# skylinemusiccds/Llama.github.io

Hardware: AMD Instinct MI355X
Metric: GBM train rows/sec (100 trees, depth 6) on HIGGS-11M at 1/2/4/8 MI355X (higher is better)
Workload: dtype fp32; 1 GPU; global_batch=11000000, parallelism=dp1 (row-sharded, hist all-reduce), rows=11000000, rows_per_rank=11000000, features=28, comm_bytes_per_tree=0

## Files before the change

llama_github_io_amd/csrc/tree_kernels.hip:

```cpp
#include <hip/hip_runtime.h>
#include <stdint.h>
#include <stdlib.h>
#include <string.h>

#include "abi.h"

#define NBIN 256
#define AMAX_SHARDS 64
#define NA_BIN 255
#define FTILE 32
#define BLK 1024
#define NW (BLK / 64)
#define TILE 2048
#define LEAFQ_STRIPES 16
#define LPR 8
#define RPI (BLK / LPR)

struct Node {
  int start, len, build, parent, sib ,
      dir , pad1, pad2;
};

#define NBW 32
#define GROUP_CAT 2
struct Dec {
  int feat;
  int bin;
  int na_left;
  int is_cat;
  unsigned bits[NBW];
  double gain;
  double wl, wr;
  float predl, predr;
};

#define TP_MAXL_DEV 64

struct Cand {
  double expl;
  double gain;
  double wl, wr;
  float predl, predr;
  int bin, na_left, valid, is_cat;
  unsigned bits[NBW];
};

struct SplitParams {
  double min_w;
  double min_split_improvement;
  double lambda, alpha, gamma;
  int mode;
  int random_split;
  unsigned long long seed;
  int hist_type;
  int fcut;
  const float* vrange;
  const double* hprev;
  const Dec* pdec;
  const Node* rnodes;
  const int* fgroup;
  const float* edges_all;
  int range_on, pad_r;
  const int* gcat;
  const double* rootw;
};

enum { HT_QUANTILES = 0, HT_UNIFORM = 1, HT_RANDOM = 2, HT_ROBUST = 3, HT_ROUND_ROBIN = 4 };

__device__ __forceinline__ unsigned long long splitmix64(unsigned long long x) {
  x += 0x9E3779B97F4A7C15ull;
  x = (x ^ (x >> 30)) * 0xBF58476D1CE4E5B9ull;
  x = (x ^ (x >> 27)) * 0x94D049BB133111EBull;
  return x ^ (x >> 31);
}

__device__ __forceinline__ bool dec_go_left(const Dec* d, int b) {
  if (b == NA_BIN) return d->na_left != 0;
  if (d->is_cat) return (d->bits[b >> 5] >> (b & 31)) & 1u;
  return b < d->bin;
}

__device__ __forceinline__ int group_level(unsigned word, unsigned pack) {
  if ((word & 0xFFu) == NA_BIN) return -1;
#pragma unroll
  for (int k = 0; k < 4; ++k) {
    const unsigned ek = (pack >> (8 * k)) & 0xFFu, b = (word >> (8 * k)) & 0xFFu;
    if (ek != 0u && b != ek) return 254 * k + (int)b;
  }
  return -1;
}

template <bool GRP = true>
__device__ __forceinline__ bool dec_go_left_key(const Dec* d, unsigned v) {
  if (GRP && d->is_cat == GROUP_CAT) {
    const int l = group_level(v, (unsigned)d->bin);
    return l < 0 ? d->na_left != 0 : ((d->bits[l >> 5] >> (l & 31)) & 1u) != 0u;
  }
  return dec_go_left(d, (int)v);
}

__device__ __forceinline__ int find_node(const int* __restrict__ tp, int n, int t) {
  int lo = 0, hi = n - 1;
  while (lo < hi) {
    int mid = (lo + hi + 1) >> 1;
    if (tp[mid] <= t) lo = mid; else hi = mid - 1;
  }
  return lo;
}

__device__ __forceinline__ double wave_sum_d(double v) {
  for (int o = 32; o > 0; o >>= 1) v += __shfl_xor(v, o, 64);
  return v;
}
__device__ __forceinline__ int wave_sum_i(int v) {
  for (int o = 32; o > 0; o >>= 1) v += __shfl_xor(v, o, 64);
  return v;
}

__device__ void block_sum4(double v[4], double* scratch ) {
  const int lane = threadIdx.x & 63, wid = threadIdx.x >> 6, nw = blockDim.x >> 6;
  for (int k = 0; k < 4; ++k) v[k] = wave_sum_d(v[k]);
  __syncthreads();
  if (lane == 0) for (int k = 0; k < 4; ++k) scratch[k * 16 + wid] = v[k];
  __syncthreads();
  if (threadIdx.x == 0) {
    for (int k = 0; k < 4; ++k) { double s = 0; for (int w = 0; w < nw; ++w) s += scratch[k * 16 + w]; v[k] = s; }
  }
  __syncthreads();
}

#define HPLANE (NBIN * FTILE + 16)
#define HIST_LDS_BYTES (2 * HPLANE * 8 + FTILE * 4)
#define WQCAP 192
#define HIST_LDS_TAIL (64 * 8 + (BLK / 64) * WQCAP * 4)
__device__ __forceinline__ int fslot(int fl) { return (fl & 16) | ((fl + ((fl >> 4) << 1)) & 15); }

__device__ __forceinline__ void lds_zero64(long long* h, int n) {
  for (int i = threadIdx.x; i < n; i += blockDim.x) h[i] = 0ll;
}

__device__ __forceinline__ long long q64(float v, float scale) {
  return (long long)(v * scale);
}

#define PACK_SHIFT 48
#define PACK_MAX 63488
__device__ __forceinline__ long long qpack(float w, float b, float scale_p, float sw, float shf) {
  if (shf < 40.f) return ((long long)__float2uint_rn(w * sw) << 32) + (long long)__float2int_rn(b * scale_p);
  return ((long long)__float2int_rz(w) << PACK_SHIFT) + (long long)__float2int_rz(b * scale_p);
}
__device__ __forceinline__ void unpack(long long v, long long& cnt, long long& val, int shift = PACK_SHIFT) {
  cnt = (long long)(((unsigned long long)v + (1ull << (shift - 1))) >> shift);
  val = (long long)((unsigned long long)v - ((unsigned long long)cnt << shift));
}

template <typename P>
__device__ __forceinline__ void put_partial(P* q, double d, bool acc) {
  *q = acc ? (P)((double)*q + d) : (P)d;
}
__device__ void flush_partial(const long long* h, const float* nayy, double node_wyy, int ftile, int F,
                              double* __restrict__ part, const double* __restrict__ qs, bool packed, bool acc,
                              bool f32, const int* srep, const int* snb, const int* sfine) {
  const int f0 = ftile * FTILE;
  const int nf = min(FTILE, F - f0);
  const double inv_a = qs[2], inv_b = qs[3], inv_p = qs[5];
  if (packed) {
    const int pshift = (int)qs[12];
    const double inv_w = qs[11];
    const int dbin = (int)blockDim.x / nf, drem = (int)blockDim.x - dbin * nf;
    int bin = (int)threadIdx.x / nf, fl = (int)threadIdx.x - bin * nf;
    for (int i = threadIdx.x; i < nf * NBIN; i += blockDim.x, bin += dbin, fl += drem) {
      if (fl >= nf) { fl -= nf; ++bin; }
      const int reps = srep[fl], nb = snb[fl];
      long long q = 0;
      if (sfine[fl]) {
        const int m = fl & ~3, k = fl & 3;
#pragma unroll
        for (int l = 0; l < 4; ++l) {
          const int bb = l <= k ? bin : bin - 1;
          if (bb >= 0) q += h[bb * FTILE + fslot(m + l)];
        }
      } else if (reps == 1) {
        q = h[bin * FTILE + fslot(fl)];
      } else if (bin < nb) {
        for (int c = 0; c < reps; ++c) q += h[(bin + c * nb) * FTILE + fslot(fl)];
      }
      long long c, v;
      unpack(q, c, v, pshift);
      const double dc = (double)c * inv_w, dv = (double)v * inv_p;
      const size_t e2 = (size_t)bin * 2 * F + 2 * (f0 + fl);
      if (f32) {
        float2* p2 = (float2*)((float*)part + e2);
        float2 o = make_float2((float)dc, (float)dv);
        if (acc) { const float2 a = *p2; o = make_float2((float)((double)a.x + dc), (float)((double)a.y + dv)); }
        *p2 = o;
      } else {
        double2* p2 = (double2*)(part + e2);
        double2 o = make_double2(dc, dv);
        if (acc) { const double2 a = *p2; o.x += a.x; o.y += a.y; }
        *p2 = o;
      }
    }
  } else {
  const int row2 = 2 * nf, dbin = (int)blockDim.x / row2, drem = (int)blockDim.x - dbin * row2;
  int bin = (int)threadIdx.x / row2, rem = (int)threadIdx.x - bin * row2;
  for (int i = threadIdx.x; i < nf * 2 * NBIN; i += blockDim.x, bin += dbin, rem += drem) {
    if (rem >= row2) { rem -= row2; ++bin; }
    const int fl = rem >> 1, r = rem & 1;
    const int reps = srep[fl], nb = snb[fl];
    long long q = 0;
    if (sfine[fl]) {
      const int m = fl & ~3, k = fl & 3;
      const int pl = r * HPLANE;
#pragma unroll
      for (int l = 0; l < 4; ++l) {
        const int bb = l <= k ? bin : bin - 1;
        if (bb >= 0) q += h[pl + bb * FTILE + fslot(m + l)];
      }
    } else if (reps == 1 || bin < nb) {
      for (int c = 0; c < reps; ++c) q += h[r * HPLANE + (bin + c * nb) * FTILE + fslot(fl)];
    }
    const double d = (double)q * (r ? inv_b : inv_a);
    const size_t e2 = (size_t)bin * 2 * F + 2 * (f0 + fl) + r;
    if (f32) put_partial((float*)part + e2, d, acc);
    else put_partial(part + e2, d, acc);
  }
  }
  for (int i = threadIdx.x; i < nf; i += blockDim.x) {
    const size_t e2 = (size_t)F * 2 * NBIN + f0 + i;
    if (f32) put_partial((float*)part + e2, (double)nayy[i], acc);
    else put_partial(part + e2, (double)nayy[i], acc);
  }
  if (threadIdx.x == 0 && ftile == 0) {
    const size_t e2 = (size_t)F * 2 * NBIN + F;
    if (f32) put_partial((float*)part + e2, node_wyy, acc);
    else put_partial(part + e2, node_wyy, acc);
  }
}

__device__ __forceinline__ float row_yy(float a, float b) {
  return a > 0.f ? b * b * __builtin_amdgcn_rcpf(a) : 0.f;
}

__device__ __forceinline__ size_t bin_off(long long row, int f, int stride, long long N, int planar) {
  return planar ? ((size_t)(f >> 5) * (size_t)N + (size_t)row) * 32 + (f & 31) : (size_t)row * stride + f;
}

struct RowFilter {
  const Dec* pd;
  const uint8_t* fptr;
  int fstride;
  int feat;
  int jw;
  int dir;
  int bin, na_left, is_cat;
  bool count;
  __device__ __forceinline__ bool left(unsigned v) const {
    if (is_cat == GROUP_CAT) {
      const int l = group_level(v, (unsigned)bin);
      return l < 0 ? na_left != 0 : ((pd->bits[l >> 5] >> (l & 31)) & 1u) != 0u;
    }
    const int b = (int)v;
    if (b == NA_BIN) return na_left != 0;
    if (is_cat) return (pd->bits[b >> 5] >> (b & 31)) & 1u;
    return b < bin;
  }
};


__device__ __forceinline__ void wave_sync_lds() {
  __builtin_amdgcn_fence(__ATOMIC_RELEASE, "wavefront");
  __builtin_amdgcn_wave_barrier();
  __builtin_amdgcn_fence(__ATOMIC_ACQUIRE, "wavefront");
}

#define FNP (TILE / BLK)
#define WROWS (TILE / NW)
__device__ __forceinline__ void filt_load(const RowFilter& flt, int r0, int r1, unsigned (&byt)[FNP]) {
  const int lane = threadIdx.x & 63, wv = threadIdx.x >> 6;
  if (flt.is_cat == GROUP_CAT) {
#pragma unroll
    for (int p = 0; p < FNP; ++p) {
      const int row = min(r0 + wv * WROWS + p * 64 + lane, r1 - 1);
      byt[p] = *reinterpret_cast<const unsigned*>(flt.fptr + (size_t)row * (size_t)flt.fstride);
    }
    return;
  }
#pragma unroll
  for (int p = 0; p < FNP; ++p) {
    const int row = min(r0 + wv * WROWS + p * 64 + lane, r1 - 1);
    byt[p] = flt.fptr[(size_t)row * (size_t)flt.fstride];
  }
}

__device__ __forceinline__ int filt_append(const RowFilter& flt, int r0, int r1, int* wq, int qn, int& lcnt,
                                           const unsigned (&byt)[FNP]) {
  const int lane = threadIdx.x & 63, wv = threadIdx.x >> 6;
  const unsigned long long below = (1ull << lane) - 1ull;
#pragma unroll
  for (int p = 0; p < FNP; ++p) {
    const int row = r0 + wv * WROWS + p * 64 + lane;
    bool sl = false;
    if (row < r1) {
      const bool gl = flt.left(byt[p]);
      if (flt.count) lcnt += gl ? 1 : 0;
      sl = (gl ? 0 : 1) == flt.dir;
    }
    const unsigned long long m = __ballot(sl);
    if (sl) wq[qn + __popcll(m & below)] = row;
    qn += __popcll(m);
  }
  return qn;
}

#ifndef H2O_UNR
#define H2O_UNR 8
#endif

struct HistSrc {
  const unsigned* bins32;
  const float* aw;
  const float* ay;
  __amdgpu_buffer_rsrc_t rb, ra, rw;
  int lgw;
};

__device__ __forceinline__ HistSrc make_src(const unsigned* bins32, const float* aw, const float* ay, long long N, int W,
                                            int lgw) {
  return HistSrc{bins32, aw, ay,
                 __builtin_amdgcn_make_buffer_rsrc((void*)bins32, 0, (int)(unsigned)((unsigned long long)N * W * 4),
                                                   0x00020000),
                 __builtin_amdgcn_make_buffer_rsrc((void*)ay, 0, (int)(unsigned)(N * 4), 0x00020000),
                 __builtin_amdgcn_make_buffer_rsrc((void*)(aw ? aw : ay), 0, (int)(unsigned)(N * 4), 0x00020000),
                 lgw};
}

template <bool FILT, bool PACKED, bool UNIT, bool NONA, bool BUF, bool FINE, int GR = RPI, int UNR = H2O_UNR>
__device__ __forceinline__ void hist_rows(long long* h, float* nayy, const HistSrc& src, int W, int wabs,
                                          int F, bool lead, int r0, int r1, int g, int j, float& wyy, float sa,
                                          float sb, float sp, const int* lst, const int* srep, const int* snb,
                                          const int* sfine) {
  const int rot = g & 1;
  unsigned offb[4], sh[4];
  unsigned vmask = 0u;
#pragma unroll
  for (int k = 0; k < 4; ++k) {
    const int kk = (k + rot) & 3;
    const int fl = j * 4 + kk;
    const int c = (g >> 1) & (srep[fl] - 1);
    offb[k] = (unsigned)fslot(fl) * 8u + ((unsigned)(c * snb[fl]) << 8);
    sh[k] = 8u * kk;
    if (wabs < W && wabs * 4 + kk < F) vmask |= 0xFFu << (8 * kk);
  }
  const bool live = vmask != 0u;
  const bool fine = FINE && live && sfine[j * 4] != 0;
  unsigned fsl[4];
#pragma unroll
  for (int l = 0; l < 4; ++l) fsl[l] = (unsigned)fslot(j * 4 + l) * 8u;
  const int wc = min(wabs, W - 1);
  const bool weighted = !UNIT && src.aw != nullptr;
  char* Hb = (char*)h;
  static_assert(FTILE * 8 == 256, "bin row of the LDS histogram is 256 bytes");
  auto ent = [&](unsigned w, int k) -> unsigned long long* {
    return (unsigned long long*)(Hb + ((__builtin_amdgcn_ubfe(w, sh[k], 8) << 8) + offb[k]));
  };
  for (int base = r0; base < r1; base += GR * UNR) {
    unsigned wd[UNR];
    float2 ab[UNR];
    const bool whole = base + GR * UNR <= r1;
    if (BUF && !FILT && whole) {
      const unsigned row0 = (unsigned)(base + g);
      const unsigned vb = (row0 << src.lgw) + (unsigned)wc * 4u, va = row0 * 4u;
#pragma unroll
      for (int u = 0; u < UNR; ++u) {
        wd[u] = __builtin_amdgcn_raw_buffer_load_b32(src.rb, vb, (unsigned)(u * GR) << src.lgw, 0);
        const float y = __uint_as_float(__builtin_amdgcn_raw_buffer_load_b32(src.ra, va, u * GR * 4, 0));
        const float w = weighted ? __uint_as_float(__builtin_amdgcn_raw_buffer_load_b32(src.rw, va, u * GR * 4, 0))
                                 : 1.f;
        ab[u] = make_float2(w, y);
      }
    } else {
#pragma unroll
      for (int u = 0; u < UNR; ++u) {
        const int idx = whole ? base + g + u * GR : min(base + g + u * GR, r1 - 1);
        const int row = FILT ? lst[idx] : idx;
        if (BUF) {
          const unsigned ro = (unsigned)row;
          wd[u] = __builtin_amdgcn_raw_buffer_load_b32(src.rb, (ro << src.lgw) + (unsigned)wc * 4u, 0, 0);
          const float y = __uint_as_float(__builtin_amdgcn_raw_buffer_load_b32(src.ra, ro * 4u, 0, 0));
          const float w = weighted ? __uint_as_float(__builtin_amdgcn_raw_buffer_load_b32(src.rw, ro * 4u, 0, 0)) : 1.f;
          ab[u] = make_float2(w, y);
        } else {
          ab[u] = make_float2(weighted ? src.aw[row] : 1.f, src.ay[row]);
          wd[u] = src.bins32[(size_t)row * W + wc];
        }
      }
    }
    auto row = [&](int u) {
      if (lead) wyy += UNIT ? ab[u].y * ab[u].y : row_yy(ab[u].x, ab[u].y);
      const long long qa = UNIT ? (1ll << PACK_SHIFT) + (long long)(int)(ab[u].y * sp)
                                : PACKED ? qpack(ab[u].x, ab[u].y, sp, sa, sb) : q64(ab[u].x, sa);
      const long long qb = PACKED ? 0ll : q64(ab[u].y, sb);
      const unsigned w = wd[u];
      if (FINE && fine) {
        const unsigned t = __builtin_amdgcn_sad_u8(w, 0u, 0u);
        const unsigned l = t & 3u;
        const unsigned so = (l & 2u) ? ((l & 1u) ? fsl[3] : fsl[2]) : ((l & 1u) ? fsl[1] : fsl[0]);
        unsigned long long* p = (unsigned long long*)(Hb + (((t >> 2) << 8) + so));
        atomicAdd(p, (unsigned long long)qa);
        if (!PACKED) atomicAdd(p + HPLANE, (unsigned long long)qb);
      } else if (live) {
#pragma unroll
        for (int k = 0; k < 4; ++k) {
          unsigned long long* p = ent(w, k);
          atomicAdd(p, (unsigned long long)qa);
          if (!PACKED) atomicAdd(p + HPLANE, (unsigned long long)qb);
        }
      }
      if (!NONA) {
        const unsigned x = ~w | ~vmask;
        if (((x - 0x01010101u) & ~x & 0x80808080u) != 0u) {
          const float yy = UNIT ? ab[u].y * ab[u].y : row_yy(ab[u].x, ab[u].y);
#pragma unroll
          for (int k = 0; k < 4; ++k)
            if (((vmask >> sh[k]) & 1u) && __builtin_amdgcn_ubfe(w, sh[k], 8) == NA_BIN)
              atomicAdd(nayy + j * 4 + (sh[k] >> 3), yy);
        }
      }
    };
    if (whole) {
#pragma unroll
      for (int u = 0; u < UNR; ++u) row(u);
    } else {
#pragma unroll
      for (int u = 0; u < UNR; ++u)
        if (base + g + u * GR < r1) row(u);
    }
  }
}

template <bool PACKED, bool UNIT, bool NONA, bool BUF, bool FINE>
__device__ __forceinline__ void hist_span(long long* h, float* nayy, const HistSrc& src, int W, int wabs, int F,
                                          bool lead, int r0, int r1, int g, int j, float& wyy, float sa, float sb,
                                          float sp, const int* srep, const int* snb, const int* sfine,
                                          bool no_atoms = false) {
  constexpr int GR = RPI, UNR = H2O_UNR;
  const int rot = g & 1;
  unsigned offb[4], sh[4];
  unsigned vmask = 0u;
#pragma unroll
  for (int k = 0; k < 4; ++k) {
    const int kk = (k + rot) & 3;
    const int fl = j * 4 + kk;
    const int c = (g >> 1) & (srep[fl] - 1);
    offb[k] = (unsigned)fslot(fl) * 8u + ((unsigned)(c * snb[fl]) << 8);
    sh[k] = 8u * kk;
    if (wabs < W && wabs * 4 + kk < F) vmask |= 0xFFu << (8 * kk);
  }
  const bool live = vmask != 0u && !no_atoms;
  const bool fine = FINE && live && sfine[j * 4] != 0;
  unsigned fsl[4];
#pragma unroll
  for (int l = 0; l < 4; ++l) fsl[l] = (unsigned)fslot(j * 4 + l) * 8u;
  const int wc = min(wabs, W - 1);
  const bool weighted = !UNIT && src.aw != nullptr;
  char* Hb = (char*)h;
  auto load = [&](int base, unsigned (&wd)[UNR], float2 (&ab)[UNR]) {
    if (BUF && base + GR * UNR <= r1) {
      const unsigned row0 = (unsigned)(base + g);
      const unsigned vb = (row0 << src.lgw) + (unsigned)wc * 4u, va = row0 * 4u;
#pragma unroll
      for (int u = 0; u < UNR; ++u) {
        wd[u] = __builtin_amdgcn_raw_buffer_load_b32(src.rb, vb, (unsigned)(u * GR) << src.lgw, 0);
        const float y = __uint_as_float(__builtin_amdgcn_raw_buffer_load_b32(src.ra, va, u * GR * 4, 0));
        const float w = weighted ? __uint_as_float(__builtin_amdgcn_raw_buffer_load_b32(src.rw, va, u * GR * 4, 0))
                                 : 1.f;
        ab[u] = make_float2(w, y);
      }
    } else {
#pragma unroll
      for (int u = 0; u < UNR; ++u) {
        const int row = min(base + g + u * GR, r1 - 1);
        if (BUF) {
          const unsigned ro = (unsigned)row;
          wd[u] = __builtin_amdgcn_raw_buffer_load_b32(src.rb, (ro << src.lgw) + (unsigned)wc * 4u, 0, 0);
          const float y = __uint_as_float(__builtin_amdgcn_raw_buffer_load_b32(src.ra, ro * 4u, 0, 0));
          const float w = weighted ? __uint_as_float(__builtin_amdgcn_raw_buffer_load_b32(src.rw, ro * 4u, 0, 0)) : 1.f;
          ab[u] = make_float2(w, y);
        } else {
          ab[u] = make_float2(weighted ? src.aw[row] : 1.f, src.ay[row]);
          wd[u] = src.bins32[(size_t)row * W + wc];
        }
      }
    }
  };
  unsigned wdn[UNR];
  float2 abn[UNR];
  if (r0 < r1) load(r0, wdn, abn);
  for (int base = r0; base < r1; base += GR * UNR) {
    unsigned wd[UNR];
    float2 ab[UNR];
#pragma unroll
    for (int u = 0; u < UNR; ++u) { wd[u] = wdn[u]; ab[u] = abn[u]; }
    if (base + GR * UNR < r1) load(base + GR * UNR, wdn, abn);
    auto atoms = [&](int u) {
      const long long qa = UNIT ? (1ll << PACK_SHIFT) + (long long)(int)(ab[u].y * sp)
                                : PACKED ? qpack(ab[u].x, ab[u].y, sp, sa, sb) : q64(ab[u].x, sa);
      const long long qb = PACKED ? 0ll : q64(ab[u].y, sb);
      const unsigned w = wd[u];
      if (FINE && fine) {
        const unsigned t = __builtin_amdgcn_sad_u8(w, 0u, 0u);
        const unsigned l = t & 3u;
        const unsigned so = (l & 2u) ? ((l & 1u) ? fsl[3] : fsl[2]) : ((l & 1u) ? fsl[1] : fsl[0]);
        unsigned long long* p = (unsigned long long*)(Hb + (((t >> 2) << 8) + so));
        atomicAdd(p, (unsigned long long)qa);
        if (!PACKED) atomicAdd(p + HPLANE, (unsigned long long)qb);
      } else {
#pragma unroll
        for (int k = 0; k < 4; ++k) {
          unsigned long long* p = (unsigned long long*)(Hb + ((__builtin_amdgcn_ubfe(w, sh[k], 8) << 8) + offb[k]));
          atomicAdd(p, (unsigned long long)qa);
          if (!PACKED) atomicAdd(p + HPLANE, (unsigned long long)qb);
        }
      }
    };
    auto row = [&](int u) {
      if (lead) wyy += UNIT ? ab[u].y * ab[u].y : row_yy(ab[u].x, ab[u].y);
      if (FINE && live) atoms(u);
      if (!NONA) {
        const unsigned w = wd[u];
        const unsigned x = ~w | ~vmask;
        if (((x - 0x01010101u) & ~x & 0x80808080u) != 0u) {
          const float yy = UNIT ? ab[u].y * ab[u].y : row_yy(ab[u].x, ab[u].y);
#pragma unroll
          for (int k = 0; k < 4; ++k)
            if (((vmask >> sh[k]) & 1u) && __builtin_amdgcn_ubfe(w, sh[k], 8) == NA_BIN)
              atomicAdd(nayy + j * 4 + (sh[k] >> 3), yy);
        }
      }
    };
    if (base + GR * UNR <= r1) {
#pragma unroll
      for (int u = 0; u < UNR; ++u) row(u);
      if (!FINE && live) {
#pragma unroll
        for (int u = 0; u < UNR; ++u) atoms(u);
      }
    } else {
#pragma unroll
      for (int u = 0; u < UNR; ++u)
        if (base + g + u * GR < r1) row(u);
      if (!FINE && live) {
#pragma unroll
        for (int u = 0; u < UNR; ++u)
          if (base + g + u * GR < r1) atoms(u);
      }
    }
  }
}

struct FiltLane {
  unsigned offb[4];
  unsigned vmask;
  int wc, rot;
  bool live, fine, weighted, lead;
};

template <bool PACKED, bool UNIT, bool FINE>
__device__ __forceinline__ FiltLane filt_lane(const HistSrc& src, int W, int wabs, int F, int g8, int j, bool lead,
                                              const int* srep, const int* snb, const int* sfine) {
  FiltLane L;
  L.rot = g8 & 1;
  L.vmask = 0u;
#pragma unroll
  for (int k = 0; k < 4; ++k) {
    const int kk = (k + L.rot) & 3;
    const int fl = j * 4 + kk;
    const int c = (g8 >> 1) & (srep[fl] - 1);
    L.offb[k] = (unsigned)fslot(fl) * 8u + ((unsigned)(c * snb[fl]) << 8);
    if (wabs < W && wabs * 4 + kk < F) L.vmask |= 0xFFu << (8 * kk);
  }
  L.live = L.vmask != 0u;
  L.fine = FINE && L.live && sfine[j * 4] != 0;
  L.wc = min(wabs, W - 1);
  L.weighted = !UNIT && src.aw != nullptr;
  L.lead = lead;
  return L;
}

template <bool UNIT, bool BUF>
__device__ __forceinline__ void filt_gather(const FiltLane& L, const HistSrc& src, int W, const int* wq, int n, int g8,
                                            unsigned (&wd)[8], float (&yv)[8], float (&wv)[8]) {
#pragma unroll
  for (int u = 0; u < 8; ++u) {
    const int row = wq[min(g8 + 8 * u, n - 1)];
    if (BUF) {
      const unsigned ro = (unsigned)row;
      wd[u] = __builtin_amdgcn_raw_buffer_load_b32(src.rb, (ro << src.lgw) + (unsigned)L.wc * 4u, 0, 0);
      yv[u] = __uint_as_float(__builtin_amdgcn_raw_buffer_load_b32(src.ra, ro * 4u, 0, 0));
      if (!UNIT) wv[u] = L.weighted ? __uint_as_float(__builtin_amdgcn_raw_buffer_load_b32(src.rw, ro * 4u, 0, 0)) : 1.f;
    } else {
      yv[u] = src.ay[row];
      if (!UNIT) wv[u] = L.weighted ? src.aw[row] : 1.f;
      wd[u] = src.bins32[(size_t)row * W + L.wc];
    }
  }
}

template <bool PACKED, bool UNIT, bool NONA, bool FINE>
__device__ __forceinline__ void filt_atoms(const FiltLane& L, long long* h, float* nayy, int n, int g8, int j,
                                           const unsigned (&wd)[8], const float (&yv)[8], const float (&wv)[8],
                                           float& wyy, float sa, float sb, float sp) {
  char* Hb = (char*)h;
#pragma unroll
  for (int u = 0; u < 8; ++u) {
    if (g8 + 8 * u >= n) continue;
    const float x = UNIT ? 1.f : wv[u];
    if (L.lead) wyy += UNIT ? yv[u] * yv[u] : row_yy(x, yv[u]);
    const long long qa = UNIT ? (1ll << PACK_SHIFT) + (long long)(int)(yv[u] * sp)
                              : PACKED ? qpack(x, yv[u], sp, sa, sb) : q64(x, sa);
    const long long qb = PACKED ? 0ll : q64(yv[u], sb);
    const unsigned w = wd[u];
    if (FINE && L.fine) {
      const unsigned t = __builtin_amdgcn_sad_u8(w, 0u, 0u);
      const unsigned l = t & 3u;
      unsigned long long* p = (unsigned long long*)(Hb + (((t >> 2) << 8) + (unsigned)fslot(j * 4 + (int)l) * 8u));
      atomicAdd(p, (unsigned long long)qa);
      if (!PACKED) atomicAdd(p + HPLANE, (unsigned long long)qb);
    } else if (L.live) {
      const unsigned wr = __builtin_amdgcn_alignbyte(w, w, L.rot);
#pragma unroll
      for (int k = 0; k < 4; ++k) {
        unsigned long long* p = (unsigned long long*)(Hb + ((__builtin_amdgcn_ubfe(wr, 8 * k, 8) << 8) + L.offb[k]));
        atomicAdd(p, (unsigned long long)qa);
        if (!PACKED) atomicAdd(p + HPLANE, (unsigned long long)qb);
      }
    }
    if (!NONA) {
      const unsigned xx = ~w | ~L.vmask;
      if (((xx - 0x01010101u) & ~xx & 0x80808080u) != 0u) {
        const float yy = UNIT ? yv[u] * yv[u] : row_yy(x, yv[u]);
#pragma unroll
        for (int k = 0; k < 4; ++k)
          if (((L.vmask >> (8 * k)) & 1u) && __builtin_amdgcn_ubfe(w, 8 * k, 8) == NA_BIN) atomicAdd(nayy + j * 4 + k, yy);
      }
    }
  }
}

template <bool FILT, bool PACKED, bool UNIT, bool NONA, bool BUF, bool FINE>
__global__ __launch_bounds__(BLK) void k_hist_build(
    const uint8_t* __restrict__ bins, int stride ,
    const float* __restrict__ aw , const float* __restrict__ ay ,
    const Node* __restrict__ nodes, const int* __restrict__ tile_prefix,
    const int* __restrict__ meta , int F, double* __restrict__ partials,
    int slot_doubles, const double* __restrict__ qs ,
    const Dec* __restrict__ pdec, int* __restrict__ nl_out, int f32, long long N, int planar, int lgw,
    const int* __restrict__ nbins_f ,
    const int* __restrict__ fine_f ,
    const uint8_t* __restrict__ fdir ,
    int dbg ) {
  constexpr bool packed = PACKED;
  extern __shared__ __attribute__((aligned(16))) long long smem64[];
  long long* h = smem64;
  float* nayy = (float*)(smem64 + (PACKED ? 1 : 2) * HPLANE);
  double* red = (double*)(nayy + FTILE);
  const int lane = threadIdx.x & 63;
  int* wq = (int*)(red + 64) + (threadIdx.x >> 6) * WQCAP;

  const int n_nodes = meta[0], n_tiles = meta[2];
  if (n_nodes <= 0 || n_tiles <= 0) return;
  const int per = (n_tiles + gridDim.x - 1) / gridDim.x;
  const int t0 = blockIdx.x * per, t1 = min(n_tiles, t0 + per);
  if (t0 >= t1) return;
  const int ftile = blockIdx.y;
  planar &= 1;
  const int W = planar ? LPR : stride >> 2;
  const int g = threadIdx.x / LPR, j = threadIdx.x % LPR;
  const int wabs = planar ? j : ftile * LPR + j;
  const int Fl = planar ? F - ftile * FTILE : F;
  const unsigned* bins32 = (const unsigned*)(planar ? bins + (size_t)ftile * (size_t)N * 32 : bins);
  const float sa = (float)qs[PACKED ? 10 : 0], sb = (float)qs[PACKED ? 12 : 1], sp = (float)qs[4];
  const HistSrc src = make_src(bins32, aw, ay, N, W, lgw);
  __shared__ int srep[FTILE], snb[FTILE], sfine[FTILE];
  if (threadIdx.x < FTILE) {
    const int fg = ftile * FTILE + threadIdx.x;
    const int fi = (fine_f && fg < F) ? fine_f[fg] : 0;
    const int nb = (NONA && nbins_f && fg < F && !fi) ? nbins_f[fg] : 0;
    srep[threadIdx.x] = (nb > 0 && nb * 4 <= NA_BIN) ? 4 : (nb > 0 && nb * 2 <= NA_BIN) ? 2 : 1;
    snb[threadIdx.x] = nb;
    sfine[threadIdx.x] = fi;
  }
  __syncthreads();

  __shared__ Dec spd;
  RowFilter flt{&spd, bins, stride, 0, -1, 0, 0, 0, 0, false};
  int lcnt = 0;
  int cur = -1, since = 0, cur_parent = -1;
  unsigned pre[FNP], pre2[FNP];
  int pre_t = -1, pre2_t = -1;
  int qn = 0;
  bool acc = false;
  double wyy = 0.0;
  const FiltLane FL = filt_lane<PACKED, UNIT, FINE>(src, W, wabs, Fl, lane >> 3, j, j == 0 && ftile == 0, srep, snb,
                                                    sfine);
  unsigned wdP[8];
  float yP[8], wP[8];
  int np = 0;
  auto drain = [&]() {
    if (!FILT) return;
    float wf2 = 0.f;
    if (qn > 0) {
      unsigned wdN[8];
      float yN[8], wN[8];
      wave_sync_lds();
      filt_gather<UNIT, BUF>(FL, src, W, wq, qn, lane >> 3, wdN, yN, wN);
      if (np > 0) filt_atoms<PACKED, UNIT, NONA, FINE>(FL, h, nayy, np, lane >> 3, j, wdP, yP, wP, wf2, sa, sb, sp);
      filt_atoms<PACKED, UNIT, NONA, FINE>(FL, h, nayy, qn, lane >> 3, j, wdN, yN, wN, wf2, sa, sb, sp);
      qn = 0;
      wave_sync_lds();
    } else if (np > 0) {
      filt_atoms<PACKED, UNIT, NONA, FINE>(FL, h, nayy, np, lane >> 3, j, wdP, yP, wP, wf2, sa, sb, sp);
    }
    np = 0;
    wyy += (double)wf2;
  };
  auto flush = [&]() {
    drain();
    if (dbg & 1) return;
    double v[4] = {wyy, (double)lcnt, 0, 0};
    block_sum4(v, red);
    __syncthreads();
    const size_t so = (size_t)(blockIdx.x + cur) * slot_doubles;
    flush_partial(h, nayy, v[0], ftile, F, f32 ? (double*)((float*)partials + so) : partials + so, qs, packed, acc,
                  f32 != 0, srep, snb, sfine);
    if (FILT && threadIdx.x == 0 && v[1] != 0.0) atomicAdd(nl_out + cur_parent, (int)v[1]);
    __syncthreads();
  };
  if (!FILT) {
    int t = t0;
    while (t < t1) {
      const int node = find_node(tile_prefix, n_nodes, t);
      const Node nd = nodes[node];
      const int tn0 = tile_prefix[node];
      const int te = max(t + 1, min(t1, tile_prefix[node + 1]));
      int rs = nd.start + (t - tn0) * TILE;
      const int re = min(nd.start + nd.len, nd.start + (te - tn0) * TILE);
      t = te;
      if (!nd.build) continue;
      while (rs < re) {
        if (node != cur || (packed && since >= PACK_MAX)) {
          if (cur >= 0) flush();
          acc = node == cur;
          lds_zero64(h, packed ? HPLANE : 2 * HPLANE);
          for (int i = threadIdx.x; i < FTILE; i += blockDim.x) nayy[i] = 0.f;
          wyy = 0.0;
          lcnt = 0;
          since = 0;
          cur = node;
          cur_parent = nd.parent;
          __syncthreads();
        }
        const int we = packed ? min(re, rs + (PACK_MAX - since)) : re;
        float wf = 0.f;
        hist_span<PACKED, UNIT, NONA, BUF, FINE>(h, nayy, src, W, wabs, Fl, j == 0 && ftile == 0, rs, we, g, j, wf, sa,
                                                 sb, sp, srep, snb, sfine, (dbg & 2) != 0);
        wyy += (double)wf;
        since += we - rs;
        rs = we;
      }
    }
  }
  for (int t = FILT ? t0 : t1; t < t1; ++t) {
    const int node = find_node(tile_prefix, n_nodes, t);
    const Node nd = nodes[node];
    if (!nd.build) continue;
    const int r0 = nd.start + (t - tile_prefix[node]) * TILE;
    const int r1 = min(r0 + TILE, nd.start + nd.len);
    if (node != cur || (packed && since + (r1 - r0) > PACK_MAX)) {
      if (cur >= 0) flush();
      acc = node == cur;
      lds_zero64(h, packed ? HPLANE : 2 * HPLANE);
      for (int i = threadIdx.x; i < FTILE; i += blockDim.x) nayy[i] = 0.f;
      if (FILT && threadIdx.x < (int)(sizeof(Dec) / 4))
        ((int*)&spd)[threadIdx.x] = ((const int*)(pdec + nd.parent))[threadIdx.x];
      wyy = 0.0;
      lcnt = 0;
      since = 0;
      cur = node;
      cur_parent = nd.parent;
      __syncthreads();
      if (FILT) {
        flt.feat = spd.feat;
        flt.fptr = bins + bin_off(0, spd.feat, stride, N, planar);
        flt.fstride = planar ? 32 : stride;
        if (fdir) { flt.fptr = fdir; flt.fstride = 1; }
        const int jw = (spd.feat >> 2) - ftile * LPR;
        flt.jw = (jw >= 0 && jw < LPR) ? jw : -1;
        flt.dir = nd.dir;
        flt.bin = spd.bin; flt.na_left = spd.na_left; flt.is_cat = spd.is_cat;
        if (fdir) { flt.bin = 1; flt.na_left = 0; flt.is_cat = 0; }
        flt.count = ftile == 0;
      }
    }
    since += r1 - r0;
    float wf = 0.f;
    if (FILT) {
      if (pre_t != t) filt_load(flt, r0, r1, pre);
      unsigned curb[FNP];
#pragma unroll
      for (int k = 0; k < FNP; ++k) curb[k] = pre[k];
      const int nend = nd.start + nd.len;
      const int rn1 = r0 + TILE, rn2 = r0 + 2 * TILE;
      if (pre2_t == t + 1) {
#pragma unroll
        for (int k = 0; k < FNP; ++k) pre[k] = pre2[k];
        pre_t = t + 1;
      } else if (t + 1 < t1 && rn1 < nend) {
        filt_load(flt, rn1, min(rn1 + TILE, nend), pre);
        pre_t = t + 1;
      } else {
        pre_t = -1;
      }
      if (t + 2 < t1 && rn2 < nend) {
        filt_load(flt, rn2, min(rn2 + TILE, nend), pre2);
        pre2_t = t + 2;
      } else {
        pre2_t = -1;
      }
      qn = filt_append(flt, r0, r1, wq, qn, lcnt, curb);
      while (qn >= 64) {
        unsigned wdN[8];
        float yN[8], wN[8];
        wave_sync_lds();
        filt_gather<UNIT, BUF>(FL, src, W, wq, 64, lane >> 3, wdN, yN, wN);
        const int rest = qn - 64;
        wave_sync_lds();
        const int v0 = lane < rest ? wq[64 + lane] : 0, v1 = lane + 64 < rest ? wq[128 + lane] : 0;
        if (lane < rest) wq[lane] = v0;
        if (lane + 64 < rest) wq[64 + lane] = v1;
        qn = rest;
        if (np > 0) filt_atoms<PACKED, UNIT, NONA, FINE>(FL, h, nayy, np, lane >> 3, j, wdP, yP, wP, wf, sa, sb, sp);
#pragma unroll
        for (int u = 0; u < 8; ++u) { wdP[u] = wdN[u]; yP[u] = yN[u]; wP[u] = wN[u]; }
        np = 64;
      }
    }
    wyy += (double)wf;
  }
  if (cur >= 0) flush();
}

#define RW 8
template <typename P, typename TO, bool COLS>
__global__ __launch_bounds__(RW * 64) void k_hist_reduce(
    const P* __restrict__ partials, int slot_doubles, int used, const Node* __restrict__ nodes,
    const int* __restrict__ bp, const int* __restrict__ meta, int G, TO* __restrict__ out, int ostride,
    double* __restrict__ hist_next, const double* __restrict__ hist_cur, int lo_F) {
  const int node = blockIdx.y;
  if (node >= meta[0]) return;
  const Node nd = nodes[node];
  if (!nd.build) return;
  __shared__ double red[RW][64];
  const int n_tiles = meta[2];
  const int per = n_tiles > 0 ? (n_tiles + G - 1) / G : 1;
  const int t0 = bp[node], t1 = bp[node + 1];
  const int b0 = t0 / per, b1 = t1 > t0 ? (t1 - 1) / per : b0 - 1;
  const int oslot = nd.parent >= 0 ? nd.parent : 0;
  const int lane = threadIdx.x & 63, w = threadIdx.x >> 6;
  int i = (COLS ? blockIdx.x * RW + w : blockIdx.x) * 64 + lane;
  if (lo_F > 0) {
    const int F = (used - 1) / (2 * NBIN + 1), lo2 = 2 * lo_F;
    const int vb = NBIN * lo2;
    if (i >= vb + F + 1) i = used;
    else i = i < vb ? (i / lo2) * 2 * F + i % lo2 : NBIN * 2 * F + (i - vb);
  }
  const int ic = min(i, used - 1);
  double a[8] = {0.0, 0.0, 0.0, 0.0, 0.0, 0.0, 0.0, 0.0};
  constexpr int ST = COLS ? 1 : RW;
  int b = b0 + (COLS ? 0 : w);
  for (; b + 7 * ST <= b1; b += 8 * ST) {
#pragma unroll
    for (int k = 0; k < 8; ++k) a[k] += (double)partials[(size_t)(b + k * ST + node) * slot_doubles + ic];
  }
  for (; b <= b1; b += ST) a[0] += (double)partials[(size_t)(b + node) * slot_doubles + ic];
  double acc = ((a[0] + a[1]) + (a[2] + a[3])) + ((a[4] + a[5]) + (a[6] + a[7]));
  if (!COLS) {
    red[w][lane] = acc;
    __syncthreads();
    if (w != 0) return;
    acc = red[0][lane];
#pragma unroll
    for (int k = 1; k < RW; ++k) acc += red[k][lane];
  }
  if (i >= used) return;
  if (out) out[(size_t)oslot * ostride + i] = (TO)acc;
  if (hist_next) {
    hist_next[(size_t)node * slot_doubles + i] = acc;
    if (nd.sib >= 0)
      hist_next[(size_t)nd.sib * slot_doubles + i] = hist_cur[(size_t)nd.parent * slot_doubles + i] - acc;
  }
}

struct Derive {
  const void* recv;
  int f32, E;
  const double* prev;
  const Node* nodes;
};

__device__ __forceinline__ double add_mul_rn(double a, double x, double y) {
#pragma clang fp contract(off)
  return a + x * y;
}

struct HistRead {
  const double* slot;
  const void* recv;
  const double* pv;
  size_t rb;
  int f32, build, derive;
  __device__ __forceinline__ double operator()(size_t i) const {
    if (!derive) return slot[i];
    const double r = f32 ? (double)((const float*)recv)[rb + i] : ((const double*)recv)[rb + i];
    return build ? r : pv[i] - r;
  }
};
#define GBINS 1024
__device__ void split_find_group(const HistRead& hv, int node, int f, int gg, int hs, int FL,
                                 const int* __restrict__ nbins_f, const int* __restrict__ mono_f, const SplitParams& p,
                                 int level, int f0, Cand* __restrict__ cand) {
  __shared__ double gk[GBINS], gw[GBINS], gy[GBINS];
  __shared__ int gi[GBINS];
  __shared__ double gwt[8];
  __shared__ double gbe[4];
  __shared__ int gbc[4];
  __shared__ unsigned gbits[NBW];
  __shared__ int s_lo, s_hi;
  const int t = threadIdx.x;
  int L = 0;
  for (int k = 0; k < gg; ++k) L = 254 * k + (nbins_f[f + k] - 1);
  for (int i = t; i < GBINS; i += 256) {
    const int k = i / 254, b = i - 254 * k;
    double w = 0.0, y = 0.0;
    bool in = false;
    if (k < gg && b < nbins_f[f + k] - 1) {
      in = true;
      w = hv((size_t)b * hs + 2 * (f + k));
      y = hv((size_t)b * hs + 2 * (f + k) + 1);
    }
    gw[i] = w; gy[i] = y;
    gk[i] = in ? (w > 0 ? y / w : -1.0e308) : 1.0e308;
    gi[i] = i;
  }
  if (t < NBW) gbits[t] = 0u;
  __syncthreads();
  for (int k = 2; k <= GBINS; k <<= 1) {
    for (int j = k >> 1; j > 0; j >>= 1) {
      for (int i = t; i < GBINS; i += 256) {
        const int ixj = i ^ j;
        if (ixj > i) {
          const bool up = (i & k) == 0;
          const double a = gk[i], b = gk[ixj];
          const int ia = gi[i], ib = gi[ixj];
          const bool gt = (a > b) || (a == b && ia > ib);
          if (gt == up) { gk[i] = b; gk[ixj] = a; gi[i] = ib; gi[ixj] = ia; }
        }
      }
      __syncthreads();
    }
  }
  double a[4], b[4];
#pragma unroll
  for (int j = 0; j < 4; ++j) { a[j] = gw[gi[4 * t + j]]; b[j] = gy[gi[4 * t + j]]; }
#pragma unroll
  for (int j = 1; j < 4; ++j) { a[j] += a[j - 1]; b[j] += b[j - 1]; }
  {
    const int lane = t & 63, wv = t >> 6;
    double sa = a[3], sb = b[3];
#pragma unroll
    for (int o = 1; o < 64; o <<= 1) {
      const double a2 = __shfl_up(sa, o, 64), b2 = __shfl_up(sb, o, 64);
      if (lane >= o) { sa += a2; sb += b2; }
    }
    if (lane == 63) { gwt[wv] = sa; gwt[4 + wv] = sb; }
    __syncthreads();
// ... 719 lines not shown
        next[li] = Node{nd.start, nd.len, 1, i, -1, 0, 0, 0};
      } else if (ri >= 0) {
        next[ri] = Node{nd.start, nd.len, 1, i, -1, 1, 0, 0};
      }
    }
  }
  const int nn = min(act_total, cap_next);
  if (i == 0) counters[0] = min(leaf_base0 + n_leaves_new, leaf_cap);
  if (odd) {
    if (i == 0) { next_meta[0] = nn; next_meta[1] = 0; next_meta[2] = 0; }
    return;
  }
  const int kt = (nd.len + TILE - 1) / TILE;
  const bool lb = li >= 0 && (ri < 0 || d.wl <= d.wr);
  const bool rb = ri >= 0 && !(li >= 0 && d.wl <= d.wr);
  int tot, totb;
  int off = wave_excl_scan((li >= 0 ? kt : 0) + (ri >= 0 ? kt : 0), &tot);
  int offb = wave_excl_scan((lb ? kt : 0) + (rb ? kt : 0), &totb);
  if (li >= 0) { next_tile_prefix[li] = off; next_build_prefix[li] = offb; off += kt; offb += lb ? kt : 0; }
  if (ri >= 0) { next_tile_prefix[ri] = off; next_build_prefix[ri] = offb; }
  if (i == 0) {
    next_tile_prefix[nn] = tot; next_build_prefix[nn] = totb;
    next_meta[0] = nn; next_meta[1] = tot; next_meta[2] = totb;
  }
}

__device__ void plan_body(
    const Node* __restrict__ nodes, const int* __restrict__ meta, Dec* __restrict__ dec,
    int* __restrict__ node_nl, const int* __restrict__ prev_nl, int4* __restrict__ curs,
    int* __restrict__ child_l, int* __restrict__ child_r,
    Node* __restrict__ next, int* __restrict__ next_tile_prefix, int* __restrict__ next_meta,
    int* __restrict__ next_build_prefix,
    int* __restrict__ counters, int* __restrict__ scratch ,
    int depth, int max_depth, double min_w, int cap_next, int leaf_cap, PlanReduce pr) {
  __shared__ int sh[17];
  const int n = meta[0];
  const int T = blockDim.x, tid = threadIdx.x;
  if (pr.cand) {
    for (int node = tid >> 6; node < n; node += T >> 6)
      reduce_node(pr.cand, node, pr.F, pr.feat_ok, pr.k_cols, pr.seed, depth, dec, pr.node_ok, pr.fgroup, tid & 63,
                  pr.cfs, pr.ccap);
    __syncthreads();
  }
  if (n <= 64 && !pr.no_wave) {
    if (tid < 64)
      plan_wave(nodes, n, dec, node_nl, prev_nl, curs, child_l, child_r, next, next_tile_prefix, next_meta,
                next_build_prefix, counters, depth, max_depth, min_w, cap_next, leaf_cap);
    return;
  }
  const bool odd = depth & 1;
  int total;
  const int perN = (n + T - 1) / T;
  const int na = min(n, tid * perN), nb2 = min(n, na + perN);
  for (int i = na; i < nb2; ++i) {
    const Node nd = nodes[i];
    if (!odd) {
      node_nl[i] = 0;
    } else {
      const int nl = nd.parent >= 0 ? prev_nl[nd.parent] : 0;
      const int cs = nd.start + (nd.dir ? nl : 0);
      const int ce = nd.dir ? nd.start + nd.len : nd.start + nl;
      curs[i] = make_int4(cs, ce, cs, ce);
    }
  }
  int act_cnt = 0;
  for (int i = na; i < nb2; ++i) {
    const DecLite d = dec_lite(dec + i);
    int a = 0;
    if (d.feat >= 0 && depth + 1 < max_depth) {
      a += (d.wl >= 2.0 * min_w) ? 1 : 0;
      a += (d.wr >= 2.0 * min_w) ? 1 : 0;
    }
    act_cnt += a;
  }
  int act_off = block_excl_scan(act_cnt, sh, &total);
  int leaf_cnt = 0;
  {
    int ao = act_off;
    for (int i = na; i < nb2; ++i) {
      const DecLite d = dec_lite(dec + i);
      int flags = 0, lv = 0;
      if (d.feat < 0) { lv = 1; }
      else {
        const bool la = depth + 1 < max_depth && d.wl >= 2.0 * min_w;
        const bool ra = depth + 1 < max_depth && d.wr >= 2.0 * min_w;
        if (la) { if (ao < cap_next) flags |= 1; ++ao; }
        if (ra) { if (ao < cap_next) flags |= 2; ++ao; }
        lv = 2 - ((flags & 1) + ((flags >> 1) & 1));
      }
      scratch[i] = flags;
      leaf_cnt += lv;
    }
  }
  const int leaf_base0 = counters[0];
  __syncthreads();
  int leaf_off = block_excl_scan(leaf_cnt, sh, &total);
  const int n_leaves_new = total;
  int ao = act_off;
  int lo = leaf_base0 + leaf_off;
  for (int i = na; i < nb2; ++i) {
    const DecLite d = dec_lite(dec + i);
    const Node nd = nodes[i];
    const int flags = scratch[i];
    if (d.feat < 0) {
      const int lid = min(lo++, leaf_cap - 1);
      child_l[i] = -1 - lid; child_r[i] = -1 - lid;
      continue;
    }
    const bool la = depth + 1 < max_depth && d.wl >= 2.0 * min_w;
    const bool ra = depth + 1 < max_depth && d.wr >= 2.0 * min_w;
    int li = -1, ri = -1;
    if (la) { if (flags & 1) li = ao; ++ao; }
    if (ra) { if (flags & 2) ri = ao; ++ao; }
    child_l[i] = (li >= 0) ? li : -1 - min(lo++, leaf_cap - 1);
    child_r[i] = (ri >= 0) ? ri : -1 - min(lo++, leaf_cap - 1);
    if (li >= 0 && ri >= 0) {
      const bool build_left = d.wl <= d.wr;
      next[li] = Node{nd.start, nd.len, build_left ? 1 : 0, i, ri, 0, 0, 0};
      next[ri] = Node{nd.start, nd.len, build_left ? 0 : 1, i, li, 1, 0, 0};
    } else if (li >= 0) {
      next[li] = Node{nd.start, nd.len, 1, i, -1, 0, 0, 0};
    } else if (ri >= 0) {
      next[ri] = Node{nd.start, nd.len, 1, i, -1, 1, 0, 0};
    }
  }
  __syncthreads();
  __shared__ int s_nnext;
  if (tid == T - 1) s_nnext = min(act_off + act_cnt, cap_next);
  __syncthreads();
  const int nn = s_nnext;
  if (tid == 0) counters[0] = min(leaf_base0 + n_leaves_new, leaf_cap);
  if (!odd) {
    level_tile_prefix(next, nn, next_tile_prefix, next_build_prefix, next_meta, sh);
  } else if (tid == 0) {
    next_meta[0] = nn; next_meta[1] = 0; next_meta[2] = 0;
  }
}

__global__ __launch_bounds__(1024) void k_plan(
    const Node* __restrict__ nodes, const int* __restrict__ meta, Dec* __restrict__ dec,
    int* __restrict__ node_nl, const int* __restrict__ prev_nl, int4* __restrict__ curs,
    int* __restrict__ child_l, int* __restrict__ child_r,
    Node* __restrict__ next, int* __restrict__ next_tile_prefix, int* __restrict__ next_meta,
    int* __restrict__ next_build_prefix, int* __restrict__ counters, int* __restrict__ scratch,
    int depth, int max_depth, double min_w, int cap_next, int leaf_cap, PlanReduce pr) {
  plan_body(nodes, meta, dec, node_nl, prev_nl, curs, child_l, child_r, next, next_tile_prefix, next_meta,
            next_build_prefix, counters, scratch, depth, max_depth, min_w, cap_next, leaf_cap, pr);
}

template <bool GRP>
__global__ __launch_bounds__(256) void k_split_find(
    double* __restrict__ hist, int slot_doubles, const int* __restrict__ meta, int F,
    const int* __restrict__ nbins_f, const int* __restrict__ iscat_f, const int* __restrict__ mono_f,
    SplitParams p, int level, Cand* __restrict__ cand, double* __restrict__ root_w,
    const float* __restrict__ edges, int adapt_nb, int f0, int FL, Derive dv) {
  split_find_body<GRP>(hist, slot_doubles, meta, F, nbins_f, iscat_f, mono_f, p, level, cand, root_w, edges, adapt_nb,
                       f0, FL, dv);
}

struct PlanArgs {
  const Node* nodes;
  const int* meta;
  Dec* dec;
  int* node_nl;
  const int* prev_nl;
  int4* curs;
  int* child_l;
  int* child_r;
  Node* next;
  int* next_tp;
  int* next_meta;
  int* next_bp;
  int* counters;
  int* scratch;
  int depth, max_depth, cap_next, leaf_cap;
  double min_w;
  PlanReduce pr;
  int* done;
};

__global__ __launch_bounds__(256) void k_split_find_plan(
    double* __restrict__ hist, int slot_doubles, const int* __restrict__ meta, int F,
    const int* __restrict__ nbins_f, const int* __restrict__ iscat_f, const int* __restrict__ mono_f,
    SplitParams p, int level, Cand* __restrict__ cand, double* __restrict__ root_w,
    const float* __restrict__ edges, int adapt_nb, int f0, int FL, Derive dv, PlanArgs pa) {
  split_find_body<false>(hist, slot_doubles, meta, F, nbins_f, iscat_f, mono_f, p, level, cand, root_w, edges,
                         adapt_nb, f0, FL, dv);
  __shared__ int s_last;
  __syncthreads();
  if (threadIdx.x == 0) {
    const int total = (int)(gridDim.x * gridDim.y);
    s_last = __hip_atomic_fetch_add(pa.done, 1, __ATOMIC_RELEASE, __HIP_MEMORY_SCOPE_AGENT) == total - 1;
  }
  __syncthreads();
  if (!s_last) return;
  __builtin_amdgcn_fence(__ATOMIC_ACQUIRE, "agent");
  plan_body(pa.nodes, pa.meta, pa.dec, pa.node_nl, pa.prev_nl, pa.curs, pa.child_l, pa.child_r, pa.next, pa.next_tp,
            pa.next_meta, pa.next_bp, pa.counters, pa.scratch, pa.depth, pa.max_depth, pa.min_w, pa.cap_next,
            pa.leaf_cap, pa.pr);
  if (threadIdx.x == 0) __hip_atomic_store(pa.done, 0, __ATOMIC_RELAXED, __HIP_MEMORY_SCOPE_AGENT);
}

__global__ __launch_bounds__(64) void k_ic_next(const Node* __restrict__ next, const int* __restrict__ next_meta,
                                                const Dec* __restrict__ dec, const unsigned char* __restrict__ ok_cur,
                                                const unsigned char* __restrict__ ic_map, int F,
                                                unsigned char* __restrict__ ok_next) {
  const int c = blockIdx.x;
  if (c >= next_meta[0]) return;
  const int par = next[c].parent;
  const int sf = dec[par].feat;
  for (int f = threadIdx.x; f < F; f += 64)
    ok_next[(size_t)c * F + f] = (sf >= 0 && ok_cur[(size_t)par * F + f] && ic_map[(size_t)sf * F + f]) ? 1 : 0;
}

__global__ __launch_bounds__(1024) void k_ranges(Node* __restrict__ next, const int4* __restrict__ curs,
                                                 int* __restrict__ tp, int* __restrict__ bp, int* __restrict__ meta) {
  __shared__ int sh[17];
  const int nn = meta[0];
  for (int i = threadIdx.x; i < nn; i += blockDim.x) {
    Node nd = next[i];
    const int4 c = curs[nd.parent];
    if (nd.dir == 0) { nd.start = c.z; nd.len = c.x - c.z; }
    else { nd.start = c.y; nd.len = c.w - c.y; }
    next[i] = nd;
  }
  __syncthreads();
  level_tile_prefix(next, nn, tp, bp, meta, sh);
}

__global__ void k_zero_hist(double* __restrict__ hbuild, const Node* __restrict__ next,
                            const int* __restrict__ meta, int slot_doubles) {
  const int node = blockIdx.y;
  if (node >= meta[0] || !next[node].build) return;
  double* s = hbuild + (size_t)next[node].parent * slot_doubles;
  for (int i = blockIdx.x * blockDim.x + threadIdx.x; i < slot_doubles; i += gridDim.x * blockDim.x) s[i] = 0.0;
}

template <typename TO>
__global__ void k_hist_pack(const double* __restrict__ src, int slot, int F, int Fs, int W, int n,
                            TO* __restrict__ dst) {
  const long long E = (long long)Fs * 2 * NBIN + Fs + 1;
  const long long total = (long long)W * n * E;
  for (long long i = blockIdx.x * (long long)blockDim.x + threadIdx.x; i < total;
       i += (long long)gridDim.x * blockDim.x) {
    const long long e = i % E;
    const long long rn = i / E;
    const int node = (int)(rn % n), r = (int)(rn / n);
    const double* sl = src + (size_t)node * slot;
    double v;
    if (e < (long long)Fs * 2 * NBIN) {
      const int bin = (int)(e / (2 * Fs)), rem = (int)(e % (2 * Fs));
      const int f = r * Fs + (rem >> 1);
      v = f < F ? sl[(size_t)bin * 2 * F + 2 * f + (rem & 1)] : 0.0;
    } else if (e < (long long)Fs * 2 * NBIN + Fs) {
      const int f = r * Fs + (int)(e - (long long)Fs * 2 * NBIN);
      v = f < F ? sl[(size_t)F * 2 * NBIN + f] : 0.0;
    } else {
      v = sl[(size_t)F * 2 * NBIN + F];
    }
    dst[i] = (TO)v;
  }
}

#define LW 8
#define LROWS (TILE / LW)
#define LU (LROWS / 64)
#define LMAXW 16

__device__ __forceinline__ unsigned pick_word(uint4 v, int wi) {
  unsigned r = v.x;
  r = wi == 1 ? v.y : r;
  r = wi == 2 ? v.z : r;
  r = wi == 3 ? v.w : r;
  return r;
}
__device__ __forceinline__ int row_byte(uint4 v0, uint4 v1, int f) {
  const int wi = f >> 2;
  const unsigned w = wi < 4 ? pick_word(v0, wi) : pick_word(v1, wi - 4);
  return (w >> (8 * (f & 3))) & 0xFF;
}
__device__ __forceinline__ int row_byte4(uint4 v0, uint4 v1, uint4 v2, uint4 v3, int f) {
  return f < 32 ? row_byte(v0, v1, f) : row_byte(v2, v3, f - 32);
}
__device__ __forceinline__ unsigned row_word(uint4 v0, uint4 v1, int f) {
  const int wi = f >> 2;
  return wi < 4 ? pick_word(v0, wi) : pick_word(v1, wi - 4);
}
__device__ __forceinline__ unsigned row_word4(uint4 v0, uint4 v1, uint4 v2, uint4 v3, int f) {
  return f < 32 ? row_word(v0, v1, f) : row_word(v2, v3, f - 32);
}
template <int NV, bool GRP>
__device__ __forceinline__ unsigned split_key(bool grp, int f, uint4 v0, uint4 v1, uint4 v2, uint4 v3,
                                              const uint8_t* __restrict__ bins, long long row, int stride, long long N,
                                              int planar) {
  if (GRP && grp) {
    if (NV > 0 && f < NV * 16) return NV > 2 ? row_word4(v0, v1, v2, v3, f) : row_word(v0, v1, f);
    return *reinterpret_cast<const unsigned*>(bins + bin_off(row, f, stride, N, planar));
  }
  return (NV > 0 && f >= NV * 16) ? bins[bin_off(row, f, stride, N, planar)]
         : NV > 2 ? (unsigned)row_byte4(v0, v1, v2, v3, f) : NV > 0 ? (unsigned)row_byte(v0, v1, f)
                  : bins[bin_off(row, f, stride, N, planar)];
}

template <int NV, bool GRP>
__device__ __forceinline__ void route_tile(
    const uint8_t* __restrict__ sbins, const float* __restrict__ say, const float* __restrict__ saw,
    uint8_t* __restrict__ dbins, float* __restrict__ day, float* __restrict__ daw, int stride,
    const Node* __restrict__ nodesA, const int* __restrict__ tpA, const int* __restrict__ metaA,
    const Dec* __restrict__ decA, const int* __restrict__ clA, const int* __restrict__ crA,
    const Dec* __restrict__ decB, const int* __restrict__ clB, const int* __restrict__ crB,
    int4* __restrict__ curs, long long N, int planar, uint8_t* __restrict__ lvl2,
    const uint8_t* __restrict__ fdir, int t) {
  const int n_nodes = metaA[0];
  __shared__ Dec sA, sB[2];
  __shared__ int sC[2], sG[4], sBase[4], sL[4];
  __shared__ int sCnt[LW][4];
  const int node = find_node(tpA, n_nodes, t);
  const Node nd = nodesA[node];
  const int tin = t - tpA[node];
  const int r0 = nd.start + tin * TILE;
  const int r1 = min(r0 + TILE, nd.start + nd.len);
  constexpr int NI = (int)(sizeof(Dec) / 4);
  if (threadIdx.x < NI) ((int*)&sA)[threadIdx.x] = ((const int*)(decA + node))[threadIdx.x];
  if (threadIdx.x < 2) sC[threadIdx.x] = threadIdx.x == 0 ? clA[node] : crA[node];
  __syncthreads();
  if (threadIdx.x < 4) {
    const int q = threadIdx.x, c = sC[q >> 1];
    sG[q] = c < 0 ? -1 : ((q & 1) ? crB[c] : clB[c]);
    const int g = c < 0 ? c : sG[q];
    sL[q] = g >= 0 ? g : 128 + (-1 - g);
  }
  for (int k = 0; k < 2; ++k) {
    const int c = sC[k];
    if (c >= 0 && threadIdx.x < NI) ((int*)&sB[k])[threadIdx.x] = ((const int*)(decB + c))[threadIdx.x];
  }
  __syncthreads();
  const int lane = threadIdx.x & 63, wid = threadIdx.x >> 6;
  const int featA = sA.feat;
  const bool grpA = sA.is_cat == GROUP_CAT;
  const int fB0 = sC[0] >= 0 ? sB[0].feat : -1, fB1 = sC[1] >= 0 ? sB[1].feat : -1;
  const bool grpB0 = sC[0] >= 0 && sB[0].is_cat == GROUP_CAT, grpB1 = sC[1] >= 0 && sB[1].is_cat == GROUP_CAT;
  const int wbase = r0 + wid * LROWS;
  const unsigned long long below = (lane == 0) ? 0ull : (~0ull >> (64 - lane));
  int q[LU], rank[LU];
  bool mv[LU];
  int cnt[4] = {0, 0, 0, 0};
  uint4 rv0[LU], rv1[LU], rv2[LU], rv3[LU];
  float ry[LU], rw[LU];
#pragma unroll
  for (int u = 0; u < LU; ++u) {
    const int row = min(wbase + u * 64 + lane, r1 - 1);
    if (NV > 0) {
      const uint4* s4 = (const uint4*)(sbins + (planar ? (size_t)row * 32 : (size_t)row * stride));
      const uint4* s4b = planar ? (const uint4*)(sbins + ((size_t)N + row) * 32) : s4 + 2;
      rv0[u] = s4[0];
      rv1[u] = NV > 1 ? s4[1] : make_uint4(0u, 0u, 0u, 0u);
      rv2[u] = NV > 2 ? s4b[0] : make_uint4(0u, 0u, 0u, 0u);
      rv3[u] = NV > 3 ? s4b[1] : make_uint4(0u, 0u, 0u, 0u);
    }
    ry[u] = say[row];
    rw[u] = saw ? saw[row] : 1.f;
  }
#pragma unroll
  for (int u = 0; u < LU; ++u) {
    const int row = wbase + u * 64 + lane;
    const bool valid = row < r1;
    int dA = 0, dB = 0;
    if (fdir) {
      dA = valid && featA >= 0 ? fdir[row] : 0;
    } else if (valid && featA >= 0)
      dA = dec_go_left_key<GRP>(&sA, split_key<NV, GRP>(grpA, featA, rv0[u], rv1[u], rv2[u], rv3[u], sbins, row, stride,
                                                        N, planar)) ? 0 : 1;
    if (valid && sC[dA] >= 0) {
      const Dec* b = &sB[dA];
      const int fb = dA ? fB1 : fB0;
      if (fb >= 0)
        dB = dec_go_left_key<GRP>(b, split_key<NV, GRP>(dA ? grpB1 : grpB0, fb, rv0[u], rv1[u], rv2[u], rv3[u], sbins,
                                                        row, stride, N, planar)) ? 0 : 1;
    }
    q[u] = 2 * dA + dB;
    mv[u] = valid && sG[q[u]] >= 0;
    if (lvl2 && valid) lvl2[row] = (uint8_t)sL[q[u]];
    rank[u] = 0;
#pragma unroll
    for (int k = 0; k < 4; ++k) {
      const bool mine = mv[u] && q[u] == k;
      const unsigned long long bm = __ballot(mine);
      if (mine) rank[u] = cnt[k] + __popcll(bm & below);
      cnt[k] += __popcll(bm);
    }
  }
  if (lane == 0) for (int k = 0; k < 4; ++k) sCnt[wid][k] = cnt[k];
  __syncthreads();
  if (threadIdx.x < 4) {
    const int k = threadIdx.x;
    int tot = 0;
    for (int w = 0; w < LW; ++w) tot += sCnt[w][k];
    int base = 0;
    if (tot > 0) {
      int4* cu = curs + sC[k >> 1];
      base = (k & 1) ? atomicSub(&cu->y, tot) - tot : atomicAdd(&cu->x, tot);
    }
    sBase[k] = base;
  }
  __syncthreads();
  int off[4];
#pragma unroll
  for (int k = 0; k < 4; ++k) {
    off[k] = sBase[k];
    for (int w = 0; w < wid; ++w) off[k] += sCnt[w][k];
  }
  const int W = stride >> 2;
  const unsigned* sb32 = (const unsigned*)sbins;
  unsigned* db32 = (unsigned*)dbins;
#pragma unroll
  for (int u = 0; u < LU; ++u) {
    if (!mv[u]) continue;
    const int row = wbase + u * 64 + lane;
    int pos = rank[u];
#pragma unroll
    for (int k = 0; k < 4; ++k) if (q[u] == k) pos += off[k];
    unsigned* dst = db32 + (size_t)pos * (planar ? 8 : W);
    if (NV > 0) {
      uint4* d4 = (uint4*)dst;
      uint4* d4b = planar ? (uint4*)(db32 + ((size_t)N + pos) * 8) : d4 + 2;
      d4[0] = rv0[u];
      if (NV > 1) d4[1] = rv1[u];
      if (NV > 2) d4b[0] = rv2[u];
      if (NV > 3) d4b[1] = rv3[u];
    } else if (planar) {
      for (int pl = 0; pl < (W >> 3); ++pl) {
        const unsigned* src = sb32 + ((size_t)pl * N + row) * 8;
        unsigned* d = db32 + ((size_t)pl * N + pos) * 8;
#pragma unroll
        for (int k = 0; k < 8; ++k) d[k] = src[k];
      }
    } else {
      const unsigned* src = sb32 + (size_t)row * W;
      if (W <= LMAXW) {
        unsigned v[LMAXW];
#pragma unroll
        for (int k = 0; k < LMAXW; ++k) if (k < W) v[k] = src[k];
#pragma unroll
        for (int k = 0; k < LMAXW; ++k) if (k < W) dst[k] = v[k];
      } else {
        for (int k = 0; k < W; ++k) dst[k] = src[k];
      }
    }
    day[pos] = ry[u];
    if (daw) daw[pos] = rw[u];
  }
}

struct RangesOut {
  Node* next;
  int* tp;
  int* bp;
  int* meta;
  int* done;
};
template <int NV, bool GRP>
__global__ __launch_bounds__(LW * 64) void k_route(
    const uint8_t* __restrict__ sbins, const float* __restrict__ say, const float* __restrict__ saw,
    uint8_t* __restrict__ dbins, float* __restrict__ day, float* __restrict__ daw, int stride,
    const Node* __restrict__ nodesA, const int* __restrict__ tpA, const int* __restrict__ metaA,
    const Dec* __restrict__ decA, const int* __restrict__ clA, const int* __restrict__ crA,
    const Dec* __restrict__ decB, const int* __restrict__ clB, const int* __restrict__ crB,
    int4* __restrict__ curs, long long N, int planar, uint8_t* __restrict__ lvl2,
    const uint8_t* __restrict__ fdir ,
    RangesOut ro) {
  const int t = blockIdx.x;
  if (t < metaA[1])
    route_tile<NV, GRP>(sbins, say, saw, dbins, day, daw, stride, nodesA, tpA, metaA, decA, clA, crA, decB, clB, crB,
                        curs, N, planar, lvl2, fdir, t);
  if (!ro.done) return;
  __shared__ int s_last;
  __shared__ int sh[17];
  __syncthreads();
  if (threadIdx.x == 0) s_last = atomicAdd(ro.done, 1) == (int)gridDim.x - 1;
  __syncthreads();
  if (!s_last) return;
  const int nn = ro.meta[0];
  for (int i = threadIdx.x; i < nn; i += blockDim.x) {
    Node nd = ro.next[i];
    int* cp = (int*)(curs + nd.parent);
    if (nd.dir == 0) {
      const int z = __hip_atomic_load(cp + 2, __ATOMIC_RELAXED, __HIP_MEMORY_SCOPE_AGENT);
      nd.start = z;
      nd.len = __hip_atomic_load(cp + 0, __ATOMIC_RELAXED, __HIP_MEMORY_SCOPE_AGENT) - z;
    } else {
      const int y = __hip_atomic_load(cp + 1, __ATOMIC_RELAXED, __HIP_MEMORY_SCOPE_AGENT);
      nd.start = y;
      nd.len = __hip_atomic_load(cp + 3, __ATOMIC_RELAXED, __HIP_MEMORY_SCOPE_AGENT) - y;
    }
    ro.next[i] = nd;
  }
  __syncthreads();
  level_tile_prefix(ro.next, nn, ro.tp, ro.bp, ro.meta, sh);
  if (threadIdx.x == 0) atomicExch(ro.done, 0);
}

__global__ __launch_bounds__(256) void k_row_dir(const uint8_t* __restrict__ bins, int stride, long long N, int planar,
                                                 const Dec* __restrict__ dec, uint8_t* __restrict__ out) {
  __shared__ Dec sd;
  if (threadIdx.x < (int)(sizeof(Dec) / 4)) ((int*)&sd)[threadIdx.x] = ((const int*)dec)[threadIdx.x];
  __syncthreads();
  const int f = sd.feat;
  for (long long row = (long long)blockIdx.x * blockDim.x + threadIdx.x; row < N; row += (long long)gridDim.x * blockDim.x)
    out[row] = (f >= 0 && !dec_go_left_key(&sd, sd.is_cat == GROUP_CAT
                                                   ? *reinterpret_cast<const unsigned*>(bins + bin_off(row, f, stride, N, planar))
                                                   : (unsigned)bins[bin_off(row, f, stride, N, planar)])) ? 1 : 0;
}

#define LEAF_LDS_MAX 2048
#define LEAF_TREE_MAX 2048
struct LevelPtrs { const Dec* dec; const int* cl; const int* cr; long long cap; };

template <int NV, bool GRP>
__device__ __forceinline__ void leaf_assign_body(
    const uint8_t* __restrict__ bins, int stride, long long N, const LevelPtrs* __restrict__ lv, int D,
    const float* __restrict__ an, const float* __restrict__ ad, const double* __restrict__ qs,
    int* __restrict__ leaf_of_row, unsigned long long* __restrict__ leafq, int leaf_cap, int n_nodes, int planar,
    const uint8_t* __restrict__ lvl2 ) {
  extern __shared__ __align__(16) unsigned char la_smem[];
  __shared__ int sbase[TP_MAXL_DEV + 1];
  const bool lds = leaf_cap <= LEAF_LDS_MAX;
  const bool tl = n_nodes <= LEAF_TREE_MAX;
  unsigned long long* sq = (unsigned long long*)la_smem;
  int4* st = (int4*)(la_smem + (lds ? (size_t)16 * leaf_cap : 0));
  if (threadIdx.x == 0) {
    int b = 0;
    for (int d = 0; d < D; ++d) { sbase[d] = b; b += (int)lv[d].cap; }
    sbase[D] = b;
  }
  if (lds)
    for (int i = threadIdx.x; i < 2 * leaf_cap; i += blockDim.x) sq[i] = 0ull;
  __syncthreads();
  if (tl) {
    for (int d = 0; d < D; ++d) {
      const int c = (int)lv[d].cap, b = sbase[d];
      for (int i = threadIdx.x; i < c; i += blockDim.x) {
        const Dec* dc = lv[d].dec + i;
        st[b + i] = make_int4(dc->feat, (dc->bin & 0xFFFF) | ((dc->na_left != 0) << 16) | ((dc->is_cat != 0) << 17) |
                                            ((dc->is_cat == GROUP_CAT) << 18),
                              lv[d].cl[i], lv[d].cr[i]);
      }
    }
  }
  __syncthreads();
  const float sn = (float)qs[6], sd = (float)qs[7];
  for (long long row = (long long)blockIdx.x * blockDim.x + threadIdx.x; row < N;
       row += (long long)gridDim.x * blockDim.x) {
    uint4 v0 = make_uint4(0u, 0u, 0u, 0u), v1 = v0, v2 = v0, v3 = v0;
    if (NV > 0) {
      const uint4* s4 = (const uint4*)(bins + (planar ? (size_t)row * 32 : (size_t)row * stride));
      const uint4* s4b = planar ? (const uint4*)(bins + ((size_t)N + row) * 32) : s4 + 2;
      v0 = s4[0];
      if (NV > 1) v1 = s4[1];
      if (NV > 2) v2 = s4b[0];
      if (NV > 3) v3 = s4b[1];
    }
    const float a_n = an[row], a_d = ad[row];
    int i = 0, leaf = 0, d0 = 0;
    if (lvl2) {
      const int code = lvl2[row];
      d0 = (code & 128) ? D : 2;
      if (code & 128) leaf = code & 127; else i = code;
    }
    for (int d = d0; d < D; ++d) {
      int c;
      if (tl) {
        const int4 e = st[sbase[d] + i];
        if (e.x < 0) {
          c = e.z;
        } else if (GRP && ((e.y >> 18) & 1)) {
          const Dec* dc = lv[d].dec + i;
          c = dec_go_left_key<GRP>(dc, split_key<NV, GRP>(true, e.x, v0, v1, v2, v3, bins, row, stride, N, planar))
                  ? e.z : e.w;
        } else {
          const int b = (NV > 0 && e.x >= NV * 16) ? bins[bin_off(row, e.x, stride, N, planar)]
                        : NV > 2 ? row_byte4(v0, v1, v2, v3, e.x) : NV > 0 ? row_byte(v0, v1, e.x)
                                 : bins[bin_off(row, e.x, stride, N, planar)];
          bool gl;
          if (b == NA_BIN) gl = (e.y >> 16) & 1;
          else if ((e.y >> 17) & 1) gl = (lv[d].dec[i].bits[b >> 5] >> (b & 31)) & 1u;
          else gl = b < (e.y & 0xFFFF);
          c = gl ? e.z : e.w;
        }
      } else {
        const Dec* dc = lv[d].dec + i;
        const int f = dc->feat;
        if (f < 0) {
          c = lv[d].cl[i];
        } else {
          c = dec_go_left_key<GRP>(dc, split_key<NV, GRP>(dc->is_cat == GROUP_CAT, f, v0, v1, v2, v3, bins, row, stride,
                                                          N, planar)) ? lv[d].cl[i] : lv[d].cr[i];
        }
      }
      if (c < 0) { leaf = -1 - c; break; }
      i = c;
    }
    leaf_of_row[row] = leaf;
    const long long qn = (long long)(a_n * sn), qd = (long long)(a_d * sd);
    if (lds) {
      if (qn) atomicAdd(sq + 2 * leaf, (unsigned long long)qn);
      if (qd) atomicAdd(sq + 2 * leaf + 1, (unsigned long long)qd);
    } else {
      unsigned long long* lq = leafq + (size_t)(blockIdx.x % LEAFQ_STRIPES) * 2 * leaf_cap;
      if (qn) atomicAdd(lq + 2 * leaf, (unsigned long long)qn);
      if (qd) atomicAdd(lq + 2 * leaf + 1, (unsigned long long)qd);
    }
  }
  if (lds) {
    __syncthreads();
    unsigned long long* lq = leafq + (size_t)(blockIdx.x % LEAFQ_STRIPES) * 2 * leaf_cap;
    for (int i = threadIdx.x; i < 2 * leaf_cap; i += blockDim.x)
      if (sq[i]) atomicAdd(lq + i, sq[i]);
  }
}

struct LeafVals {
  int log_link;
  double scale, kclamp, mx, lam, l1;
  float* out;
};

__device__ __forceinline__ float leaf_value(double num, double den, const LeafVals& v) {
  if (v.l1 > 0.0) num = num > v.l1 ? num - v.l1 : (num < -v.l1 ? num + v.l1 : 0.0);
  double g = den == 0.0 ? 0.0 : num / (den + v.lam);
  if (v.log_link) g = den == 0.0 ? 0.0 : log(fmax(g, 1e-300));
  double x = v.scale * g;
  if (x != x) x = 0.0;
  if (v.kclamp > 0.0) x = fmin(fmax(x, -v.kclamp), v.kclamp);
  if (isinf(x)) x = x > 0 ? 1e4 : -1e4;
  x = fmin(fmax(x, -v.mx), v.mx);
  return (float)x;
}

__device__ __forceinline__ void leafsum_one(unsigned long long* __restrict__ leafq, const double* __restrict__ qs,
                                            int n, double* __restrict__ leafsum, const LeafVals& lv, int i) {
  long long a = 0, b = 0;
  for (int k = 0; k < LEAFQ_STRIPES; ++k) {
    unsigned long long* q = leafq + (size_t)k * 2 * n;
    a += (long long)q[2 * i];
    b += (long long)q[2 * i + 1];
    q[2 * i] = 0ull;
    q[2 * i + 1] = 0ull;
  }
  leafsum[2 * i] = (double)a * qs[8];
  leafsum[2 * i + 1] = (double)b * qs[9];
  if (lv.out) lv.out[i] = leaf_value(leafsum[2 * i], leafsum[2 * i + 1], lv);
}

__global__ void k_leafsum_finish(unsigned long long* __restrict__ leafq, const double* __restrict__ qs, int n,
                                 double* __restrict__ leafsum, LeafVals lv) {
  const int i = blockIdx.x * blockDim.x + threadIdx.x;
  if (i < n) leafsum_one(leafq, qs, n, leafsum, lv, i);
}

template <int NV, bool FUSE, bool GRP>
__global__ __launch_bounds__(256) void k_leaf_assign(
    const uint8_t* __restrict__ bins, int stride, long long N, const LevelPtrs* __restrict__ lv, int D,
    const float* __restrict__ an, const float* __restrict__ ad, const double* __restrict__ qs,
    int* __restrict__ leaf_of_row, unsigned long long* __restrict__ leafq, int leaf_cap, int n_nodes, int planar,
    const uint8_t* __restrict__ lvl2, double* __restrict__ leafsum, LeafVals vals, int* __restrict__ done) {
  leaf_assign_body<NV, GRP>(bins, stride, N, lv, D, an, ad, qs, leaf_of_row, leafq, leaf_cap, n_nodes, planar, lvl2);
  if (!FUSE || !done) return;
  __shared__ int s_last;
  __syncthreads();
  if (threadIdx.x == 0)
    s_last = __hip_atomic_fetch_add(done, 1, __ATOMIC_RELEASE, __HIP_MEMORY_SCOPE_AGENT) == (int)gridDim.x - 1;
  __syncthreads();
  if (!s_last) return;
  __builtin_amdgcn_fence(__ATOMIC_ACQUIRE, "agent");
  for (int i = threadIdx.x; i < leaf_cap; i += blockDim.x) leafsum_one(leafq, qs, leaf_cap, leafsum, vals, i);
  if (threadIdx.x == 0) __hip_atomic_store(done, 0, __ATOMIC_RELAXED, __HIP_MEMORY_SCOPE_AGENT);
}

__global__ __launch_bounds__(256) void k_bin_assign(const float* __restrict__ X, long long N, int F, int stride,
                                                    const float* __restrict__ edges, int max_edges,
                                                    const int* __restrict__ nedges, const int* __restrict__ iscat,
                                                    uint8_t* __restrict__ bins, int planar,
                                                    const int* __restrict__ xmap ) {
  extern __shared__ float se[];
  __shared__ int sn[32], sc[32];
  const int f0 = blockIdx.y * 32;
  const int nf = min(32, stride - f0);
  const int nr = max(0, min(32, F - f0));
  for (int i = threadIdx.x; i < nr * max_edges; i += blockDim.x)
    se[i] = edges[(size_t)f0 * max_edges + i];
  if (threadIdx.x < 32) {
    sn[threadIdx.x] = threadIdx.x < nr ? nedges[f0 + threadIdx.x] : 0;
    sc[threadIdx.x] = threadIdx.x < nr ? iscat[f0 + threadIdx.x] : 0;
  }
  __syncthreads();
  for (long long row = (long long)blockIdx.x * blockDim.x + threadIdx.x; row < N;
       row += (long long)gridDim.x * blockDim.x) {
    uint32_t wd[8];
#pragma unroll
    for (int k = 0; k < 8; ++k) wd[k] = 0u;
#pragma unroll
    for (int fl = 0; fl < 32; ++fl) {
      if (fl < nr) {
        const int xr = xmap ? xmap[f0 + fl] : f0 + fl;
        const float x = X[(long long)xr * N + row];
        int b;
        if (x != x) b = NA_BIN;
        else if (sc[fl]) {
          const int code = (int)x;
          b = (code >= 0 && code <= sn[fl]) ? code : NA_BIN;
        } else {
          const float* e = se + fl * max_edges;
          int lo = 0, hi = sn[fl];
          while (lo < hi) { const int mid = (lo + hi) >> 1; if (e[mid] <= x) lo = mid + 1; else hi = mid; }
          b = lo;
        }
        wd[fl >> 2] |= (uint32_t)(b & 0xFF) << (8 * (fl & 3));
      }
    }
    if (planar) {
      uint4* dst = reinterpret_cast<uint4*>(bins + ((long long)blockIdx.y * N + row) * 32);
      dst[0] = make_uint4(wd[0], wd[1], wd[2], wd[3]);
      dst[1] = make_uint4(wd[4], wd[5], wd[6], wd[7]);
    } else {
      uint32_t* dst = reinterpret_cast<uint32_t*>(bins + row * stride + f0);
#pragma unroll
      for (int k = 0; k < 8; ++k)
        if (4 * k < nf) dst[k] = wd[k];
    }
  }
}

__global__ __launch_bounds__(256) void k_amax(const float* __restrict__ aux, long long N, unsigned* __restrict__ amax_bits) {
  float m[4] = {0.f, 0.f, 0.f, 0.f};
  for (long long i = (long long)blockIdx.x * blockDim.x + threadIdx.x; i < N; i += (long long)gridDim.x * blockDim.x) {
#pragma unroll
    for (int c = 0; c < 4; ++c) m[c] = fmaxf(m[c], fabsf(aux[(size_t)c * N + i]));
  }
#pragma unroll
  for (int c = 0; c < 4; ++c)
    for (int off = 32; off > 0; off >>= 1) m[c] = fmaxf(m[c], __shfl_xor(m[c], off, 64));
  __shared__ float sm[4][4];
  const int wv = threadIdx.x >> 6;
  if ((threadIdx.x & 63) == 0) for (int c = 0; c < 4; ++c) sm[c][wv] = m[c];
  __syncthreads();
  if (threadIdx.x < 4) {
    const int c = threadIdx.x;
    float v = sm[c][0];
    for (int k = 1; k < (int)(blockDim.x >> 6); ++k) v = fmaxf(v, sm[c][k]);
    atomicMax(amax_bits + 4 * (blockIdx.x & (AMAX_SHARDS - 1)) + c, __float_as_uint(v));
  }
}

__global__ __launch_bounds__(256) void k_qscale(unsigned* __restrict__ amax_bits, double* __restrict__ qs,
                                                int* __restrict__ counters, long long N, int fpack) {
  __shared__ unsigned sm[4];
  if (threadIdx.x < 4) {
    unsigned mbits = 0u;
    for (int k = 0; k < AMAX_SHARDS; ++k) mbits = max(mbits, amax_bits[4 * k + threadIdx.x]);
    sm[threadIdx.x] = mbits;
  }
  __syncthreads();
  if (threadIdx.x < 4) {
    const int c = threadIdx.x;
    const double m = (double)__uint_as_float(sm[c]);
    const bool ok = m > 0.0 && m == m && m < 1e300;
    if (c < 2) {
      const double sc = ok ? 1099511627776.0 / m : 1.0;
      qs[c] = sc;
      qs[2 + c] = 1.0 / sc;
      if (c == 1) {
        const double sp = !ok ? 1.0 : fpack ? 0.99 * 2147483648.0 / ((double)PACK_MAX * m) : 1073741824.0 / m;
        qs[4] = sp;
        qs[5] = 1.0 / sp;
      } else {
        const double sw = (fpack && ok) ? 0.99 * 4294967296.0 / ((double)PACK_MAX * m) : 1.0;
        qs[10] = sw;
        qs[11] = 1.0 / sw;
        qs[12] = fpack ? 32.0 : (double)PACK_SHIFT;
      }
    } else {
      int lb = 61;
      for (long long n = N; n > 0; n >>= 1) --lb;
      if (lb < 8) lb = 8;
      const double sc = ok ? ldexp(1.0, lb) / m : 1.0;
      qs[6 + (c - 2)] = sc;
      qs[8 + (c - 2)] = 1.0 / sc;
    }
  }
  for (int i = threadIdx.x; i < 4 * AMAX_SHARDS; i += blockDim.x) amax_bits[i] = 0u;
  if (counters && threadIdx.x < 4) counters[threadIdx.x] = 0;
}

__global__ void k_leaf_values(const double* __restrict__ leafsum, int n, int log_link, double scale, double kclamp,
                              double mx, double lam, double l1, float* __restrict__ out) {
  const int i = blockIdx.x * blockDim.x + threadIdx.x;
  if (i >= n) return;
  const LeafVals v{log_link, scale, kclamp, mx, lam, l1, out};
  out[i] = leaf_value(leafsum[2 * i], leafsum[2 * i + 1], v);
}

#define R16_NB 1024
#define R16_NA 1023
#define R16_FS 16
#define R16_LDS (R16_NB * R16_FS * 8 + R16_FS * 4 + 64 * 8)
template <bool UNIT>
__global__ __launch_bounds__(BLK) void k_hist_root16(
    const unsigned* __restrict__ fine32 , const float* __restrict__ aw,
    const float* __restrict__ ay, long long N, const int* __restrict__ meta, const int* __restrict__ fcol ,
    const int* __restrict__ fnc , int F,
    double* __restrict__ partials, int slot_doubles, const double* __restrict__ qs, int f32) {
  extern __shared__ __attribute__((aligned(16))) long long smem64[];
  long long* h = smem64;
  float* nayy = (float*)(smem64 + R16_NB * R16_FS);
  double* red = (double*)(nayy + R16_FS);
  const int n_tiles = meta[2];
  if (n_tiles <= 0) return;
  const int per = (n_tiles + gridDim.x - 1) / gridDim.x;
  const int t0 = blockIdx.x * per, t1 = min(n_tiles, t0 + per);
  if (t0 >= t1) return;
  const long long rb = (long long)t0 * TILE, re = min(N, (long long)t1 * TILE);
  const int ft = blockIdx.y;
  const unsigned* w32 = fine32 + (size_t)ft * (size_t)N * 8;
  const int g = threadIdx.x / LPR, j = threadIdx.x % LPR;
  const bool lead = j == 0 && ft == 0;
  const float sa = (float)qs[10], sb = (float)qs[12], sp = (float)qs[4];
  const int pshift = (int)qs[12];
  const double inv_w = qs[11], inv_p = qs[5];
  constexpr int UNR = 8;
  char* Hb = (char*)h;
  const unsigned slo = (unsigned)(2 * j) * 8u, shi = (unsigned)(2 * j + 1) * 8u;
  double wyy_blk = 0.0;
  bool acc = false;
  for (long long ws = rb; ws < re; ws += PACK_MAX) {
    const long long we = min(re, ws + PACK_MAX);
    for (int i = threadIdx.x; i < R16_NB * R16_FS; i += BLK) h[i] = 0ll;
    if (threadIdx.x < R16_FS) nayy[threadIdx.x] = 0.f;
    __syncthreads();
    float wyy = 0.f;
    for (long long base = ws; base < we; base += (long long)RPI * UNR) {
      unsigned wd[UNR];
      float yv[UNR], wv[UNR];
#pragma unroll
      for (int u = 0; u < UNR; ++u) {
        const long long row = min(base + g + (long long)u * RPI, we - 1);
        wd[u] = w32[(size_t)row * 8 + j];
        yv[u] = ay[row];
        wv[u] = UNIT ? 1.f : (aw ? aw[row] : 1.f);
      }
#pragma unroll
      for (int u = 0; u < UNR; ++u) {
        const long long row = base + g + (long long)u * RPI;
        if (row >= we) continue;
        const long long qa = UNIT ? (1ll << PACK_SHIFT) + (long long)(int)(yv[u] * sp) : qpack(wv[u], yv[u], sp, sa, sb);
        const unsigned w = wd[u];
        const unsigned tl = w & 0xFFFFu, th = w >> 16;
        const bool odd = (row & 1) != 0;
        const unsigned t_a = odd ? th : tl, t_b = odd ? tl : th;
        const unsigned s_a = odd ? shi : slo, s_b = odd ? slo : shi;
        atomicAdd((unsigned long long*)(Hb + ((t_a << 7) + s_a)), (unsigned long long)qa);
        atomicAdd((unsigned long long*)(Hb + ((t_b << 7) + s_b)), (unsigned long long)qa);
        const float yy = UNIT ? yv[u] * yv[u] : row_yy(wv[u], yv[u]);
        if (lead) wyy += yy;
        if (tl == R16_NA) atomicAdd(nayy + 2 * j, yy);
        if (th == R16_NA) atomicAdd(nayy + 2 * j + 1, yy);
      }
    }
    double v[4] = {(double)wyy, 0.0, 0.0, 0.0};
    block_sum4(v, red);
    __syncthreads();
    wyy_blk = v[0];
    double* part = partials + (size_t)blockIdx.x * slot_doubles;
    for (int i = threadIdx.x; i < R16_FS * 4 * NBIN; i += BLK) {
      const int bin = i >> 6, sl = (i >> 2) & 15, k = i & 3;
      const int slot = ft * R16_FS + sl;
      const int n = fnc[slot];
      if (k >= n) continue;
      const int col = fcol[slot * 4 + k];
      long long q = 0;
      if (bin == NA_BIN) {
        q = h[R16_NA * R16_FS + sl];
      } else {
        for (int m = 0; m < n; ++m) {
          const int t = n * bin + k - m;
          if (t >= 0 && t < R16_NA) q += h[t * R16_FS + sl];
        }
      }
      long long c, val;
      unpack(q, c, val, pshift);
      const double dc = (double)c * inv_w, dv = (double)val * inv_p;
      const size_t e2 = (size_t)bin * 2 * F + 2 * col;
      if (f32) {
        float2* p2 = (float2*)((float*)part + e2);
        float2 o = make_float2((float)dc, (float)dv);
        if (acc) { const float2 a = *p2; o = make_float2((float)((double)a.x + dc), (float)((double)a.y + dv)); }
        *p2 = o;
      } else {
        double2* p2 = (double2*)(part + e2);
        double2 o = make_double2(dc, dv);
        if (acc) { const double2 a = *p2; o.x += a.x; o.y += a.y; }
        *p2 = o;
      }
    }
    for (int i = threadIdx.x; i < R16_FS * 4; i += BLK) {
      const int sl = i >> 2, k = i & 3, slot = ft * R16_FS + sl;
      if (k >= fnc[slot]) continue;
      const size_t e2 = (size_t)F * 2 * NBIN + fcol[slot * 4 + k];
      if (f32) put_partial((float*)part + e2, (double)nayy[sl], acc);
      else put_partial(part + e2, (double)nayy[sl], acc);
    }
    if (threadIdx.x == 0 && ft == 0) {
      const size_t e2 = (size_t)F * 2 * NBIN + F;
      if (f32) put_partial((float*)part + e2, wyy_blk, acc);
      else put_partial(part + e2, wyy_blk, acc);
    }
    acc = true;
    __syncthreads();
  }
}

__global__ __launch_bounds__(256) void k_fine16_build(const uint8_t* __restrict__ master, int planes, long long N,
                                                      const int* __restrict__ cslot ,
                                                      int nslot, unsigned short* __restrict__ fine) {
  __shared__ unsigned short acc[64][256];
  const int tid = threadIdx.x;
  const long long row = (long long)blockIdx.x * 256 + tid;
  for (int k = 0; k < nslot; ++k) acc[k][tid] = 0;
  if (row >= N) return;
  for (int pl = 0; pl < planes; ++pl) {
    const uint4* src = (const uint4*)(master + ((size_t)pl * (size_t)N + (size_t)row) * 32);
    const uint4 v0 = src[0], v1 = src[1];
    const unsigned wd[8] = {v0.x, v0.y, v0.z, v0.w, v1.x, v1.y, v1.z, v1.w};
#pragma unroll
    for (int c = 0; c < 32; ++c) {
      const int sl = cslot[pl * 32 + c];
      if (sl < 0) continue;
      const unsigned b = (wd[c >> 2] >> (8 * (c & 3))) & 0xFFu;
      if (b == NA_BIN) acc[sl][tid] = 0x8000;
      else acc[sl][tid] = (unsigned short)(acc[sl][tid] + b);
    }
  }
  const int p16 = (nslot + 15) / 16;
  for (int q = 0; q < p16; ++q) {
    unsigned w[8];
#pragma unroll
    for (int i = 0; i < 8; ++i) {
      unsigned lo = 0, hi = 0;
      const int s0 = q * 16 + 2 * i, s1 = s0 + 1;
      if (s0 < nslot) { lo = acc[s0][tid]; lo = (lo & 0x8000u) ? 1023u : lo; }
      if (s1 < nslot) { hi = acc[s1][tid]; hi = (hi & 0x8000u) ? 1023u : hi; }
      w[i] = lo | (hi << 16);
    }
    uint4* dst = (uint4*)(fine + ((size_t)q * (size_t)N + (size_t)row) * 16);
    dst[0] = make_uint4(w[0], w[1], w[2], w[3]);
    dst[1] = make_uint4(w[4], w[5], w[6], w[7]);
  }
}

static int hist_dbg() {
  const char* e = getenv("H2O_HIST_DBG");
  return e ? atoi(e) : 0;
}

template <bool FILT, bool PACKED, bool UNIT, bool NONA, bool BUF>
static void launch_hist4(dim3 grid, size_t lds, hipStream_t s, const void* bins, int stride, const void* aw,
                         const void* ay, const void* nodes, const void* tile_prefix, const void* meta, int F,
                         void* partials, int slot_doubles, const void* qs, const void* pdec, void* nl_out, int f32,
                         long long N, int planar, int lgw, const void* nbins_f, const void* fine_f, const void* fdir) {
#define H2O_HB(FINE_)                                                                                              \
  hipLaunchKernelGGL((k_hist_build<FILT, PACKED, UNIT, NONA, BUF, FINE_>), grid, dim3(BLK), lds, s,               \
                     (const uint8_t*)bins, stride, (const float*)aw, (const float*)ay, (const Node*)nodes,         \
                     (const int*)tile_prefix, (const int*)meta, F, (double*)partials, slot_doubles, (const double*)qs, \
                     (const Dec*)pdec, (int*)nl_out, f32, N, planar, lgw, (const int*)nbins_f, (const int*)fine_f,  \
                     (const uint8_t*)fdir, hist_dbg())
  if (fine_f) H2O_HB(true); else H2O_HB(false);
#undef H2O_HB
}

template <bool PACKED, bool UNIT>
static void launch_hist(dim3 grid, size_t lds, hipStream_t s, const void* bins, int stride, const void* aw,
                        const void* ay, const void* nodes, const void* tile_prefix, const void* meta, int F,
                        void* partials, int slot_doubles, const void* qs, const void* pdec, void* nl_out, int f32,
                        long long N, int planar, const void* nbins_f, const void* fine_f, const void* fdir) {
  const bool nona = (planar >> 1) & 1;
  planar &= 1;
  const int rowb = planar ? 32 : stride;
  const unsigned long long bytes = (unsigned long long)N * (unsigned long long)rowb;
  int lgw = -1;
  for (int k = 0; k < 12; ++k) if (rowb == (1 << k)) lgw = k;
  const char* e_buf = getenv("H2O_HIST_BUF");
  const bool buf = lgw >= 0 && bytes < (1ull << 32) && (unsigned long long)N * 4ull < (1ull << 32) &&
                   !(e_buf && strcmp(e_buf, "0") == 0);
#define H2O_HIST_CASE(F_, N_, B_) \
  launch_hist4<F_, PACKED, UNIT, N_, B_>(grid, lds, s, bins, stride, aw, ay, nodes, tile_prefix, meta, F, partials, \
                                          slot_doubles, qs, pdec, nl_out, f32, N, planar, lgw, nbins_f, fine_f, fdir)
  const bool filt = pdec != nullptr;
  if (filt) {
    if (nona) { if (buf) H2O_HIST_CASE(true, true, true); else H2O_HIST_CASE(true, true, false); }
    else { if (buf) H2O_HIST_CASE(true, false, true); else H2O_HIST_CASE(true, false, false); }
  } else {
    if (nona) { if (buf) H2O_HIST_CASE(false, true, true); else H2O_HIST_CASE(false, true, false); }
    else { if (buf) H2O_HIST_CASE(false, false, true); else H2O_HIST_CASE(false, false, false); }
  }
#undef H2O_HIST_CASE
}

template <typename P, typename TO>
static void reduce_launch(const void* partials, int slot_doubles, int used, const void* nodes, const void* bp,
                          const void* meta, int cap, int grid, void* out, int ostride, void* hist_next,
                          const void* hist_cur, int lo_F, hipStream_t s) {
  const int F = (used - 1) / (2 * NBIN + 1);
  if (lo_F >= F) lo_F = 0;
  const int n = lo_F > 0 ? NBIN * 2 * lo_F + F + 1 : used;
  if (cap >= 16 && !getenv("H2O_REDUCE_SPLIT")) {
    const int gx = (n + 64 * RW - 1) / (64 * RW);
    hipLaunchKernelGGL((k_hist_reduce<P, TO, true>), dim3(gx, cap), dim3(RW * 64), 0, s, (const P*)partials,
                       slot_doubles, used, (const Node*)nodes, (const int*)bp, (const int*)meta, grid, (TO*)out,
                       ostride, (double*)hist_next, (const double*)hist_cur, lo_F);
    return;
  }
  const int gx = (n + 63) / 64;
  hipLaunchKernelGGL((k_hist_reduce<P, TO, false>), dim3(gx, cap), dim3(RW * 64), 0, s, (const P*)partials, slot_doubles,
                     used, (const Node*)nodes, (const int*)bp, (const int*)meta, grid, (TO*)out, ostride,
                     (double*)hist_next, (const double*)hist_cur, lo_F);
}

extern "C" {

int h2o_abi_version() { return H2O_ABI_VERSION; }

int h2o_tree_sizes(int* out) {
  out[7] = AMAX_SHARDS;
  out[8] = LEAFQ_STRIPES;
  out[0] = sizeof(Node); out[1] = sizeof(Dec); out[2] = sizeof(Cand); out[3] = TILE; out[4] = FTILE;
  out[5] = HIST_LDS_BYTES + HIST_LDS_TAIL;
  out[6] = BLK;
  return 0;
}

int h2o_hist_build(const void* bins, int stride, const void* aw, const void* ay, const void* nodes,
                   const void* tile_prefix, const void* meta, int F, void* partials, int slot_doubles, const void* qs,
                   int grid, int packed, const void* pdec, void* nl_out, int f32, long long N, int planar,
                   const void* nbins_f, const void* fine_f, int nft_lim, const void* fdir, hipStream_t s) {
  int nft = (F + FTILE - 1) / FTILE;
  if (nft_lim > 0 && nft_lim < nft) nft = nft_lim;
  const char* e_repl = getenv("H2O_HIST_REPL");
  const char* e_fine = getenv("H2O_HIST_FINE");
  const bool repl = !e_repl || strcmp(e_repl, "0") != 0;
  const bool fine = e_fine && strcmp(e_fine, "1") == 0;
  if (!repl) nbins_f = nullptr;
  if (!fine) fine_f = nullptr;
  const size_t lds = (packed ? HIST_LDS_BYTES - HPLANE * 8 : HIST_LDS_BYTES) + HIST_LDS_TAIL;
  const dim3 gr(grid, nft);
  if (packed && aw == nullptr)
    launch_hist<true, true>(gr, lds, s, bins, stride, aw, ay, nodes, tile_prefix, meta, F, partials, slot_doubles, qs, pdec, nl_out, f32, N, planar, nbins_f, fine_f, fdir);
  else if (packed) launch_hist<true, false>(gr, lds, s, bins, stride, aw, ay, nodes, tile_prefix, meta, F, partials, slot_doubles, qs, pdec, nl_out, f32, N, planar, nbins_f, fine_f, fdir);
  else launch_hist<false, false>(gr, lds, s, bins, stride, aw, ay, nodes, tile_prefix, meta, F, partials, slot_doubles, qs, pdec, nl_out, f32, N, planar, nbins_f, fine_f, fdir);
  return (int)hipGetLastError();
}


int h2o_fine16_build(const void* master, int planes, long long N, const void* cslot, int nslot, void* fine,
                     hipStream_t s) {
  if (nslot < 1 || nslot > 64 || planes < 1 || N <= 0) return (int)hipErrorInvalidValue;
  hipLaunchKernelGGL(k_fine16_build, dim3((unsigned)((N + 255) / 256)), dim3(256), 0, s, (const uint8_t*)master, planes,
                     N, (const int*)cslot, nslot, (unsigned short*)fine);
  return (int)hipGetLastError();
}

int h2o_hist_root16(const void* fine, int planes, const void* aw, const void* ay, long long N, const void* meta,
                    const void* fcol, const void* fnc, int F, void* partials, int slot_doubles, const void* qs, int grid,
                    int f32, hipStream_t s) {
  if (planes < 1 || grid < 1 || N <= 0) return (int)hipErrorInvalidValue;
  const dim3 gr(grid, planes);
  if (aw == nullptr)
    hipLaunchKernelGGL((k_hist_root16<true>), gr, dim3(BLK), R16_LDS, s, (const unsigned*)fine, (const float*)aw,
                       (const float*)ay, N, (const int*)meta, (const int*)fcol, (const int*)fnc, F, (double*)partials,
                       slot_doubles, (const double*)qs, f32);
  else
    hipLaunchKernelGGL((k_hist_root16<false>), gr, dim3(BLK), R16_LDS, s, (const unsigned*)fine, (const float*)aw,
                       (const float*)ay, N, (const int*)meta, (const int*)fcol, (const int*)fnc, F, (double*)partials,
                       slot_doubles, (const double*)qs, f32);
  return (int)hipGetLastError();
}

int h2o_hist_reduce(const void* partials, int slot_doubles, int used, const void* nodes, const void* bp,
                    const void* meta, int cap, int grid, void* out, void* hist_next, const void* hist_cur,
                    int f32, int out_f32, int ostride, int lo_F, hipStream_t s) {
  if (ostride <= 0) ostride = slot_doubles;
  if (f32 && out_f32)
    reduce_launch<float, float>(partials, slot_doubles, used, nodes, bp, meta, cap, grid, out, ostride, hist_next, hist_cur, lo_F, s);
  else if (f32)
    reduce_launch<float, double>(partials, slot_doubles, used, nodes, bp, meta, cap, grid, out, ostride, hist_next, hist_cur, lo_F, s);
  else if (out_f32)
    reduce_launch<double, float>(partials, slot_doubles, used, nodes, bp, meta, cap, grid, out, ostride, hist_next, hist_cur, lo_F, s);
  else
    reduce_launch<double, double>(partials, slot_doubles, used, nodes, bp, meta, cap, grid, out, ostride, hist_next, hist_cur, lo_F, s);
  return (int)hipGetLastError();
}

int h2o_leaf_values(const void* leafsum, int n, int log_link, double scale, double kclamp, double mx, double lam,
                    double l1, void* out,
                    hipStream_t s) {
  hipLaunchKernelGGL(k_leaf_values, dim3((n + 255) / 256), dim3(256), 0, s, (const double*)leafsum, n, log_link,
                     scale, kclamp, mx, lam, l1, (float*)out);
  return (int)hipGetLastError();
}

static int split_find_launch(void* hist, int slot_doubles, const void* meta, int cap, int F, const void* nbins_f,
                             const void* iscat_f, const void* mono_f, const SplitParams& p, int level, void* cand,
                             void* root_w, const void* edges, int adapt_nb, int f0, int FL, Derive dv, hipStream_t s) {
  if (F <= 0 || cap <= 0) return 0;
  if (FL < F) return (int)hipErrorInvalidValue;
  if (p.gcat)
    hipLaunchKernelGGL(k_split_find<true>, dim3(cap, F), dim3(256), 0, s, (double*)hist, slot_doubles,
                       (const int*)meta, F, (const int*)nbins_f, (const int*)iscat_f, (const int*)mono_f, p, level,
                       (Cand*)cand, (double*)root_w, (const float*)edges, adapt_nb, f0, FL, dv);
  else
    hipLaunchKernelGGL(k_split_find<false>, dim3(cap, F), dim3(256), 0, s, (double*)hist, slot_doubles,
                       (const int*)meta, F, (const int*)nbins_f, (const int*)iscat_f, (const int*)mono_f, p, level,
                       (Cand*)cand, (double*)root_w, (const float*)edges, adapt_nb, f0, FL, dv);
  return (int)hipGetLastError();
}

int h2o_split_find(const void* hist, int slot_doubles, const void* meta, int cap, int F, const void* nbins_f,
                   const void* iscat_f, const void* mono_f, double min_w, double msi, double lambda_, double alpha,
                   double gamma, int mode, int random_split, unsigned long long seed, int level, void* cand,
                   void* root_w, const void* edges, int adapt_nb, int hist_type, int f0, int FL, hipStream_t s) {
  SplitParams p;
  p.min_w = min_w; p.min_split_improvement = msi; p.lambda = lambda_; p.alpha = alpha; p.gamma = gamma;
  p.mode = mode; p.random_split = random_split; p.seed = seed; p.hist_type = hist_type; p.fcut = 0;
  p.vrange = nullptr; p.hprev = nullptr; p.pdec = nullptr; p.rnodes = nullptr; p.fgroup = nullptr; p.edges_all = nullptr;
  p.range_on = 0; p.pad_r = 0; p.gcat = nullptr; p.rootw = nullptr;
  return split_find_launch((void*)hist, slot_doubles, meta, cap, F, nbins_f, iscat_f, mono_f, p, level, cand, root_w,
                           edges, adapt_nb, f0, FL, Derive{nullptr, 0, 0, nullptr, nullptr}, s);
}

int h2o_split_reduce(const void* cand, const void* meta, int cap, int F, const void* feat_ok, int k_cols,
                     unsigned long long seed, int level, void* dec, const void* node_ok, const void* fgroup,
                     int cfs, hipStream_t s) {
  hipLaunchKernelGGL(k_split_reduce, dim3(cap), dim3(64), 0, s, (const Cand*)cand, (const int*)meta, F,
                     (const int*)feat_ok, k_cols, seed, level, (Dec*)dec, (const unsigned char*)node_ok,
                     (const int*)fgroup, cfs, cap);
  return (int)hipGetLastError();
}

int h2o_ic_next(const void* next, const void* next_meta, const void* dec, const void* ok_cur, const void* ic_map, int F,
                void* ok_next, int cap_next, hipStream_t s) {
  if (cap_next <= 0) return 0;
  hipLaunchKernelGGL(k_ic_next, dim3(cap_next), dim3(64), 0, s, (const Node*)next, (const int*)next_meta,
                     (const Dec*)dec, (const unsigned char*)ok_cur, (const unsigned char*)ic_map, F,
                     (unsigned char*)ok_next);
  return (int)hipGetLastError();
}

static int plan_wave_off() {
  static int v = -1;
  if (v < 0) { const char* e = getenv("H2O_PLAN_WAVE"); v = (e && e[0] == '0') ? 1 : 0; }
  return v;
}

static int plan_launch(const void* nodes, const void* meta, void* dec, void* node_nl, const void* prev_nl, void* curs,
                       void* child_l, void* child_r, void* next, void* next_tile_prefix, void* next_meta,
                       void* next_build_prefix, void* counters, void* scratch, int depth, int max_depth, double min_w,
                       int cap_next, int leaf_cap, PlanReduce pr, hipStream_t s) {
  pr.no_wave = plan_wave_off();
  hipLaunchKernelGGL(k_plan, dim3(1), dim3(1024), 0, s, (const Node*)nodes, (const int*)meta, (Dec*)dec,
                     (int*)node_nl, (const int*)prev_nl, (int4*)curs, (int*)child_l, (int*)child_r, (Node*)next,
                     (int*)next_tile_prefix, (int*)next_meta, (int*)next_build_prefix, (int*)counters, (int*)scratch,
                     depth, max_depth, min_w, cap_next, leaf_cap, pr);
  return (int)hipGetLastError();
}

int h2o_plan(const void* nodes, const void* meta, const void* dec, void* node_nl, const void* prev_nl, void* curs,
             void* child_l, void* child_r, void* next, void* next_tile_prefix, void* next_meta, void* next_build_prefix,
             void* counters, void* scratch, int depth, int max_depth, double min_w, int cap_next, int leaf_cap,
             hipStream_t s) {
  PlanReduce pr{nullptr, 0, nullptr, 0, 0ull, nullptr, nullptr, 0, 0};
  return plan_launch(nodes, meta, (void*)dec, node_nl, prev_nl, curs, child_l, child_r, next, next_tile_prefix,
                     next_meta, next_build_prefix, counters, scratch, depth, max_depth, min_w, cap_next, leaf_cap, pr, s);
}

int h2o_ranges(void* next, const void* curs, void* tp, void* bp, void* meta, hipStream_t s) {
  hipLaunchKernelGGL(k_ranges, dim3(1), dim3(1024), 0, s, (Node*)next, (const int4*)curs, (int*)tp, (int*)bp,
                     (int*)meta);
  return (int)hipGetLastError();
}

int h2o_zero_hist(void* hist, const void* next, const void* meta, int cap, int slot_doubles, hipStream_t s) {
  const int gx = (slot_doubles + 1023) / 1024;
  hipLaunchKernelGGL(k_zero_hist, dim3(gx < 64 ? gx : 64, cap), dim3(256), 0, s, (double*)hist,
                     (const Node*)next, (const int*)meta, slot_doubles);
  return (int)hipGetLastError();
}


int h2o_hist_pack(const void* src, int slot, int F, int Fs, int W, int n, void* dst, int out_f32, hipStream_t s) {
  if (n <= 0) return 0;
  const long long total = (long long)W * n * ((long long)Fs * 2 * NBIN + Fs + 1);
  long long g = (total + 255) / 256;
  const dim3 gr((unsigned)(g < 4096 ? g : 4096));
  if (out_f32)
    hipLaunchKernelGGL(k_hist_pack<float>, gr, dim3(256), 0, s, (const double*)src, slot, F, Fs, W, n, (float*)dst);
  else
    hipLaunchKernelGGL(k_hist_pack<double>, gr, dim3(256), 0, s, (const double*)src, slot, F, Fs, W, n, (double*)dst);
  return (int)hipGetLastError();
}

static bool route_generic() {
  static int v = -1;
  if (v < 0) { const char* e = getenv("H2O_ROUTE_GENERIC"); v = (e && e[0] == '1') ? 1 : 0; }
  return v == 1;
}

static int nv_of(int stride) {
  if (route_generic()) return 0;
  return stride == 64 ? 4 : stride == 48 ? 3 : stride == 32 ? 2 : stride == 16 ? 1 : 0;
}

static int route_launch(const void* sbins, const void* say, const void* saw, void* dbins, void* day, void* daw,
                        int stride, const void* nodesA, const void* tpA, const void* metaA, const void* decA,
                        const void* clA, const void* crA, const void* decB, const void* clB, const void* crB,
                        void* curs, int tiles_cap, long long N, int planar, int lp, void* lvl2, const void* fdir,
                        RangesOut ro, hipStream_t s, int grp = 0) {
  if (planar && (stride % 32 != 0 || stride < 64)) return (int)hipErrorInvalidValue;
  if (lp < 0 || lp > 2 || (lp > 0 && !planar)) return (int)hipErrorInvalidValue;
#define ROUTE_LAUNCH(NV) do { if (grp) ROUTE_LAUNCH2(NV, true); else ROUTE_LAUNCH2(NV, false); } while (0)
#define ROUTE_LAUNCH2(NV, G)                                                                                   \
  hipLaunchKernelGGL((k_route<NV, G>), dim3(tiles_cap), dim3(LW * 64), 0, s, (const uint8_t*)sbins,           \
                     (const float*)say, (const float*)saw, (uint8_t*)dbins, (float*)day, (float*)daw, stride,  \
                     (const Node*)nodesA, (const int*)tpA, (const int*)metaA, (const Dec*)decA, (const int*)clA, \
                     (const int*)crA, (const Dec*)decB, (const int*)clB, (const int*)crB, (int4*)curs, N, planar, \
                     (uint8_t*)lvl2, (const uint8_t*)fdir, ro)
  switch (lp == 1 ? 2 : lp == 2 ? 4 : nv_of(stride)) {
    case 4: ROUTE_LAUNCH(4); break;
    case 3: ROUTE_LAUNCH(3); break;
    case 2: ROUTE_LAUNCH(2); break;
    case 1: ROUTE_LAUNCH(1); break;
    default: ROUTE_LAUNCH(0);
  }
#undef ROUTE_LAUNCH
#undef ROUTE_LAUNCH2
  return (int)hipGetLastError();
}

int h2o_route(const void* sbins, const void* say, const void* saw, void* dbins, void* day, void* daw, int stride,
              const void* nodesA, const void* tpA, const void* metaA, const void* decA, const void* clA,
              const void* crA, const void* decB, const void* clB, const void* crB, void* curs, int tiles_cap,
              long long N, int planar, int lp, void* lvl2, const void* fdir, hipStream_t s) {
  return route_launch(sbins, say, saw, dbins, day, daw, stride, nodesA, tpA, metaA, decA, clA, crA, decB, clB, crB,
                      curs, tiles_cap, N, planar, lp, lvl2, fdir, RangesOut{nullptr, nullptr, nullptr, nullptr, nullptr},
                      s);
}

static int leaf_assign_launch(const void* master, int stride, long long N, const void* lvptrs, int D, const void* an,
                              const void* ad, const void* qs, void* leaf_of_row, void* leafq, int leaf_cap,
                              void* leafsum, int n_nodes, int planar, LeafVals lv, hipStream_t s,
                              const void* lvl2 = nullptr, int* done = nullptr, int grp = 0) {
  if (D > TP_MAXL_DEV) return (int)hipErrorInvalidValue;
  long long grid = (N + 255) / 256;
  if (grid > 2048) grid = 2048;
  if (grid < 1) grid = 1;
  const size_t lds = (leaf_cap <= LEAF_LDS_MAX ? (size_t)16 * leaf_cap : 0) +
                     (n_nodes <= LEAF_TREE_MAX ? (size_t)16 * n_nodes : 0);
#define LA(NV) do { if (done) { LA1(NV, true); } else { LA1(NV, false); } } while (0)
#define LA1(NV, FU) do { if (grp) { LA2(NV, FU, true); } else { LA2(NV, FU, false); } } while (0)
#define LA2(NV, FU, G) hipLaunchKernelGGL((k_leaf_assign<NV, FU, G>), dim3((unsigned)grid), dim3(256), lds, s, (const uint8_t*)master, \
                                  stride, N, (const LevelPtrs*)lvptrs, D, (const float*)an, (const float*)ad,          \
                                  (const double*)qs, (int*)leaf_of_row, (unsigned long long*)leafq, leaf_cap, n_nodes, planar, \
                                  (const uint8_t*)lvl2, (double*)leafsum, lv, done)
  switch ((planar && stride > 64 && !route_generic()) ? (lvl2 ? 2 : 4) : nv_of(stride)) {
    case 4: LA(4); break;
    case 3: LA(3); break;
    case 2: LA(2); break;
    case 1: LA(1); break;
    default: LA(0);
  }
#undef LA
#undef LA1
#undef LA2
  if (!done)
    hipLaunchKernelGGL(k_leafsum_finish, dim3((leaf_cap + 255) / 256), dim3(256), 0, s, (unsigned long long*)leafq,
                       (const double*)qs, leaf_cap, (double*)leafsum, lv);
  return (int)hipGetLastError();
}

int h2o_leaf_assign(const void* master, int stride, long long N, const void* lvptrs, int D, const void* an,
                    const void* ad, const void* qs, void* leaf_of_row, void* leafq, int leaf_cap, void* leafsum,
                    int n_nodes, int planar, hipStream_t s) {
  const LeafVals lv{0, 0.0, 0.0, 0.0, 0.0, 0.0, nullptr};
  return leaf_assign_launch(master, stride, N, lvptrs, D, an, ad, qs, leaf_of_row, leafq, leaf_cap, leafsum, n_nodes,
                            planar, lv, s);
}

int h2o_amax(const void* aux, long long N, void* amax_bits, hipStream_t s) {
  long long grid = (N + 255) / 256;
  if (grid > 2048) grid = 2048;
  if (grid < 1) grid = 1;
  hipLaunchKernelGGL(k_amax, dim3((unsigned)grid), dim3(256), 0, s, (const float*)aux, N, (unsigned*)amax_bits);
  return (int)hipGetLastError();
}

__global__ __launch_bounds__(256) void k_snap_copy(const uint4* __restrict__ src, uint4* __restrict__ dst, long long n16,
                                                   const unsigned char* __restrict__ srcb, unsigned char* __restrict__ dstb,
                                                   long long nbytes) {
  for (long long i = (long long)blockIdx.x * blockDim.x + threadIdx.x; i < n16; i += (long long)gridDim.x * blockDim.x)
    dst[i] = src[i];
  const long long t = n16 * 16 + (long long)blockIdx.x * blockDim.x + threadIdx.x;
  if (t < nbytes) dstb[t] = srcb[t];
}

int h2o_host_dev_ptr(void* host, unsigned long long* out) {
  void* d = nullptr;
  const hipError_t e = hipHostGetDevicePointer(&d, host, 0);
  *out = (unsigned long long)(uintptr_t)d;
  return (int)e;
}

int h2o_snap_copy(const void* src, void* dst, long long nbytes, hipStream_t s) {
  if (nbytes <= 0) return 0;
  if ((((uintptr_t)src) | ((uintptr_t)dst)) & 15) return (int)hipErrorInvalidValue;
  const long long n16 = nbytes / 16;
  long long grid = (n16 + 255) / 256;
  if (grid < 1) grid = 1;
  if (grid > 64) grid = 64;
  hipLaunchKernelGGL(k_snap_copy, dim3((unsigned)grid), dim3(256), 0, s, (const uint4*)src, (uint4*)dst, n16,
                     (const unsigned char*)src, (unsigned char*)dst, nbytes);
  return (int)hipGetLastError();
}

int h2o_qscale(void* amax_bits, void* qs, void* counters, long long N, int fpack, hipStream_t s) {
  hipLaunchKernelGGL(k_qscale, dim3(1), dim3(256), 0, s, (unsigned*)amax_bits, (double*)qs, (int*)counters, N, fpack);
  return (int)hipGetLastError();
}

int h2o_bin_assign(const void* X, long long N, int F, int stride, const void* edges, int max_edges,
                   const void* nedges, const void* iscat, void* bins, int planar, const void* xmap,
                   hipStream_t s) {
  if (planar && (stride % 32 != 0 || stride < 64)) return (int)hipErrorInvalidValue;
  if (stride % 4 != 0 || max_edges < 1 || (size_t)32 * max_edges * sizeof(float) > 96 * 1024)
    return (int)hipErrorInvalidValue;
  const int blk = 256;
  const int groups = (stride + 31) / 32;
  long long grid = (N + blk - 1) / blk;
  if (grid > 4096) grid = 4096;
  if (grid < 1) grid = 1;
  hipLaunchKernelGGL(k_bin_assign, dim3((unsigned)grid, (unsigned)groups), dim3(blk),
                     (size_t)32 * max_edges * sizeof(float), s, (const float*)X, N, F, stride,
                     (const float*)edges, max_edges, (const int*)nedges, (const int*)iscat, (uint8_t*)bins, planar,
                     (const int*)xmap);
  return (int)hipGetLastError();
}

#define TP_MAXL 65
struct TreePlan {
  long long N;
  int stride, F, D, slot, used, pf32, grid, leaf_cap, mode, random_split, unit;
  double min_w, msi, lam, alpha, gamma;
  void *master, *partials, *hist0, *hist1, *hbuild, *cand, *scratch, *nbins_f, *iscat_f, *mono_f;
  void *qs, *leafsum, *leaf_of_row, *counters, *rootw, *leafval, *leafq, *lvptrs;
  void *bb[2], *by[2], *bw[2];
  void *nodes[TP_MAXL], *meta[TP_MAXL], *tp[TP_MAXL], *bp[TP_MAXL], *dec[TP_MAXL], *cl[TP_MAXL], *cr[TP_MAXL],
      *nl[TP_MAXL], *cur[TP_MAXL];
  int caps[TP_MAXL], tiles_cap[TP_MAXL];
  void *aux, *amax_bits, *feat_ok;
  int compute_amax, k_cols, packed, leaf_native, log_link, hist_type;
  unsigned long long seed;
  double scale, kclamp, mx;
  int kc_level[TP_MAXL];
  int pad2;
  void* edges;
  int nb_level[TP_MAXL];
  int pad3;
  void* ic_map;
  void* ic[TP_MAXL];
  int sliced, fs0, fsn, sslot;
  void *cand_local, *hrecv;
  double leaf_lam, leaf_l1;
  int planar, no_na;
  void* fgroup;
  void* coll_fn;
  void* coll_ctx;
  int W, cf32;
  int cand_fs;
  int dist;
  void *hsend, *cand_all, *lsx;
  void* fine_f;
  int lo_F, lo_from, mid_F, mid_from;
  void* lvl2;
  void* fdir;
  int num_plane, pad4;
  void* fine16;
  void* f16col;
  void* f16n;
  int f16_planes, pad5;
  void* vrange;
  int range_on, pad6;
  void* gcat;
};

static inline void tp_node_range(const TreePlan* P, int d, const void* hprev, SplitParams& p) {
  p.range_on = (P->range_on && P->vrange && P->edges && P->nb_level[d] > 1) ? 1 : 0;
  p.vrange = (const float*)P->vrange;
  p.hprev = d > 0 ? (const double*)hprev : nullptr;
  p.pdec = d > 0 ? (const Dec*)P->dec[d - 1] : nullptr;
  p.rnodes = (const Node*)P->nodes[d];
  p.fgroup = (const int*)P->fgroup;
  p.edges_all = (const float*)P->edges;
  p.pad_r = 0;
  p.gcat = (const int*)P->gcat;
  p.rootw = d > 0 ? (const double*)P->rootw : nullptr;
}

enum { H2O_COLL_ALLREDUCE = 0, H2O_COLL_REDUCE_SCATTER = 1, H2O_COLL_ALLGATHER = 2 };
enum { H2O_DT_F32 = 0, H2O_DT_F64 = 1, H2O_DT_U8 = 2 };
typedef int (*h2o_coll_fn)(void* ctx, int op, const void* send, void* recv, long long count, int dtype,
                           hipStream_t s);

static inline const float* tp_aux(const TreePlan* P, int c) { return (const float*)P->aux + (size_t)c * P->N; }

static inline void tp_level_buf(const TreePlan* P, int e, const void*& b, const void*& y, const void*& w) {
  if (e == 0) { b = P->master; y = tp_aux(P, 1); w = P->unit ? nullptr : tp_aux(P, 0); return; }
  const int i = (e / 2 - 1) % 2;
  b = P->bb[i]; y = P->by[i]; w = P->unit ? nullptr : P->bw[i];
}

static inline int tp_fcut(const TreePlan* P, int d) {
  if (P->lo_F > 0 && d >= P->lo_from) return P->lo_F;
  if (P->mid_F > 0 && d >= P->mid_from) return P->mid_F;
  return 0;
}
static inline int tp_planes(int fc) { return fc > 0 ? (fc + FTILE - 1) / FTILE : 0; }
static inline void* tp_lvl2(const TreePlan* P) {
  return (P->lvl2 && P->planar && P->D > 2 && tp_fcut(P, 2) > 0 && tp_fcut(P, 2) <= FTILE) ? P->lvl2 : nullptr;
}

static bool route_fused_ranges() {
  static int v = -1;
  if (v < 0) { const char* e = getenv("H2O_ROUTE_RANGES"); v = (e && e[0] == '0') ? 0 : 1; }
  return v == 1;
}

static int tp_route(const TreePlan* P, int e, hipStream_t s, bool ranges) {
  const void *sb, *sy, *sw;
  tp_level_buf(P, e, sb, sy, sw);
  const int di = (e / 2) % 2;
  const int np = tp_planes(tp_fcut(P, e + 2));
  const int lp = (P->planar && np <= 2) ? np : 0;
  const RangesOut ro = ranges ? RangesOut{(Node*)P->nodes[e + 2], (int*)P->tp[e + 2], (int*)P->bp[e + 2],
                                          (int*)P->meta[e + 2], (int*)P->counters + 1}
                              : RangesOut{nullptr, nullptr, nullptr, nullptr, nullptr};
  return route_launch(sb, sy, sw, P->bb[di], P->by[di], P->unit ? nullptr : P->bw[di], P->stride, P->nodes[e], P->tp[e],
                      P->meta[e], P->dec[e], P->cl[e], P->cr[e], P->dec[e + 1], P->cl[e + 1], P->cr[e + 1],
                      P->cur[e + 1], P->tiles_cap[e], P->N, P->planar, lp, e == 0 ? tp_lvl2(P) : nullptr,
                      (e == 0 && tp_lvl2(P) && P->fdir) ? P->fdir : nullptr, ro, s, P->gcat != nullptr);
}

#define TP_CHECK(x) do { int rc_ = (x); if (rc_) return rc_; } while (0)

int h2o_tree_plan_size() { return (int)sizeof(TreePlan); }

int h2o_tree_root(const TreePlan* P, hipStream_t s) {
  if (P->D >= TP_MAXL - 1) return (int)hipErrorInvalidValue;
  if (P->compute_amax) TP_CHECK(h2o_amax(P->aux, P->N, P->amax_bits, s));
  TP_CHECK(h2o_qscale(P->amax_bits, P->qs, P->counters, P->N, P->packed == 2, s));
  const int g0 = P->tiles_cap[0] < P->grid ? P->tiles_cap[0] : P->grid;
  if (P->fine16 && P->packed && !P->sliced && tp_fcut(P, 0) == 0)
    TP_CHECK(h2o_hist_root16(P->fine16, P->f16_planes, P->unit ? nullptr : tp_aux(P, 0), tp_aux(P, 1), P->N, P->meta[0],
                             P->f16col, P->f16n, P->F, P->partials, P->slot, P->qs, g0, P->pf32, s));
  else
  TP_CHECK(h2o_hist_build(P->master, P->stride, P->unit ? nullptr : tp_aux(P, 0), tp_aux(P, 1), P->nodes[0], P->bp[0],
                          P->meta[0], P->F, P->partials, P->slot, P->qs, g0, P->packed, nullptr, nullptr, P->pf32, P->N,
                          P->planar | (P->no_na << 1), P->nbins_f, P->fine_f, tp_planes(tp_fcut(P, 0)), nullptr, s));
  if (P->dist && !P->sliced)
    return h2o_hist_reduce(P->partials, P->slot, P->used, P->nodes[0], P->bp[0], P->meta[0], 1, g0, P->hrecv, nullptr,
                           nullptr, P->pf32, P->cf32, P->sslot, tp_fcut(P, 0), s);
  return h2o_hist_reduce(P->partials, P->slot, P->used, P->nodes[0], P->bp[0], P->meta[0], 1, g0,
                         P->sliced ? P->hbuild : P->hist0, nullptr, nullptr, P->pf32, 0, 0,
                         tp_fcut(P, 0), s);
}

int h2o_tree_find(const TreePlan* P, int d, hipStream_t s) {
  void* hc = (d % 2) ? P->hist1 : P->hist0;
  const void* hp = (d % 2) ? P->hist0 : P->hist1;
  SplitParams p;
  p.min_w = P->min_w; p.min_split_improvement = P->msi; p.lambda = P->lam; p.alpha = P->alpha; p.gamma = P->gamma;
  p.mode = P->mode; p.random_split = P->random_split; p.seed = P->seed; p.hist_type = P->hist_type;
  p.fcut = tp_fcut(P, d);
  tp_node_range(P, d, hp, p);
  const int hs = P->sliced ? P->sslot : P->slot;
  const Derive dv = P->dist ? Derive{P->hrecv, P->cf32, P->sslot, (const double*)hp, (const Node*)P->nodes[d]}
                            : Derive{nullptr, 0, 0, nullptr, nullptr};
  if (!P->sliced)
    return split_find_launch(hc, hs, P->meta[d], P->caps[d], P->F, P->nbins_f, P->iscat_f, P->mono_f, p, d, P->cand,
                             d == 0 ? P->rootw : nullptr, P->edges, P->nb_level[d], 0, P->F, dv, s);
  const int f0 = P->fs0;
  return split_find_launch(hc, hs, P->meta[d], P->caps[d], P->fsn, (const int*)P->nbins_f + f0,
                           (const int*)P->iscat_f + f0, P->mono_f ? (const int*)P->mono_f + f0 : nullptr, p, d,
                           P->cand_local, d == 0 ? P->rootw : nullptr,
                           P->edges ? (const float*)P->edges + (size_t)f0 * 255 : nullptr, P->nb_level[d], f0,
                           (P->sslot - 1) / (2 * NBIN + 1), dv, s);
}

static int tree_grow(const TreePlan* P, int d, int dist, hipStream_t s, bool plan_done);
int h2o_tree_grow(const TreePlan* P, int d, int dist, hipStream_t s) { return tree_grow(P, d, dist, s, false); }

static bool plan_fused() {
  static int v = -1;
  if (v < 0) { const char* e = getenv("H2O_PLAN_FUSED"); v = (e && e[0] == '1') ? 1 : 0; }
  return v == 1;
}

static int tree_find_plan(const TreePlan* P, int d, hipStream_t s) {
  void* hc = (d % 2) ? P->hist1 : P->hist0;
  SplitParams p;
  p.min_w = P->min_w; p.min_split_improvement = P->msi; p.lambda = P->lam; p.alpha = P->alpha; p.gamma = P->gamma;
  p.mode = P->mode; p.random_split = P->random_split; p.seed = P->seed; p.hist_type = P->hist_type;
  p.fcut = tp_fcut(P, d);
  tp_node_range(P, d, (d % 2) ? P->hist0 : P->hist1, p);
  const int cap = P->caps[d];
  const int kc = P->kc_level[d] > 0 ? P->kc_level[d] : P->k_cols;
  const PlanReduce pr{(const Cand*)P->cand, P->F, (const int*)P->feat_ok, kc, P->seed,
                      P->ic_map ? (const unsigned char*)P->ic[d] : nullptr, (const int*)P->fgroup, 0, cap};
  const bool odd = d % 2 == 1;
  const PlanArgs pa{(const Node*)P->nodes[d], (const int*)P->meta[d], (Dec*)P->dec[d], (int*)P->nl[d],
                    odd ? (const int*)P->nl[d - 1] : nullptr, (int4*)P->cur[d], (int*)P->cl[d], (int*)P->cr[d],
                    (Node*)P->nodes[d + 1], (int*)P->tp[d + 1], (int*)P->meta[d + 1], (int*)P->bp[d + 1],
                    (int*)P->counters, (int*)P->scratch, d, P->D, P->caps[d + 1], P->leaf_cap, P->min_w, pr,
                    (int*)P->counters + 2};
  if (P->F <= 0 || cap <= 0) return (int)hipErrorInvalidValue;
  hipLaunchKernelGGL(k_split_find_plan, dim3(cap, P->F), dim3(256), 0, s, (double*)hc, P->slot, (const int*)P->meta[d],
                     P->F, (const int*)P->nbins_f, (const int*)P->iscat_f, (const int*)P->mono_f, p, d,
                     (Cand*)P->cand, d == 0 ? (double*)P->rootw : nullptr, (const float*)P->edges, P->nb_level[d], 0,
                     P->F, Derive{nullptr, 0, 0, nullptr, nullptr}, pa);
  return (int)hipGetLastError();
}

static int tree_grow(const TreePlan* P, int d, int dist, hipStream_t s, bool plan_done) {
  void* hc = (d % 2) ? P->hist1 : P->hist0;
  void* hn = (d % 2) ? P->hist0 : P->hist1;
  const int cap = P->caps[d];
  const bool odd = d % 2 == 1;
  int rc;
  const int kc = P->kc_level[d] > 0 ? P->kc_level[d] : P->k_cols;
  const void* cand = P->sliced ? P->cand_all : P->cand;
  const int cfs = P->sliced ? P->cand_fs : 0;
  PlanReduce pr{nullptr, P->F, (const int*)P->feat_ok, kc, P->seed,
                P->ic_map ? (const unsigned char*)P->ic[d] : nullptr, (const int*)P->fgroup, cfs, cap};
  if (!plan_done) {
    if (cap <= PLAN_REDUCE_MAX) {
      pr.cand = (const Cand*)cand;
    } else {
      rc = h2o_split_reduce(cand, P->meta[d], cap, P->F, P->feat_ok, kc, P->seed, d, P->dec[d],
                            P->ic_map ? P->ic[d] : nullptr, P->fgroup, cfs, s);
      if (rc) return -rc;
    }
    rc = plan_launch(P->nodes[d], P->meta[d], P->dec[d], P->nl[d], odd ? P->nl[d - 1] : nullptr, P->cur[d], P->cl[d],
                     P->cr[d], P->nodes[d + 1], P->tp[d + 1], P->meta[d + 1], P->bp[d + 1], P->counters, P->scratch,
                     d, P->D, P->min_w, P->caps[d + 1], P->leaf_cap, pr, s);
    if (rc) return -rc;
  }
  if (P->ic_map && d + 1 < P->D) {
    rc = h2o_ic_next(P->nodes[d + 1], P->meta[d + 1], P->dec[d], P->ic[d], P->ic_map, P->F, P->ic[d + 1],
                     P->caps[d + 1], s);
    if (rc) return -rc;
  }
  if (d + 1 == P->D) return 1;
  int gh;
  const void *sb, *sy, *sw;
  if (!odd) {
    gh = P->tiles_cap[d] < P->grid ? P->tiles_cap[d] : P->grid;
    tp_level_buf(P, d, sb, sy, sw);
    const void* fdir = nullptr;
    if (d == 0 && P->fdir && (tp_lvl2(P) || (P->planar && tp_planes(tp_fcut(P, 1) > 0 ? tp_fcut(P, 1) : P->F) >= 2))) {
      long long g = (P->N + 255) / 256;
      if (g > 4096) g = 4096;
      if (g < 1) g = 1;
      hipLaunchKernelGGL(k_row_dir, dim3((unsigned)g), dim3(256), 0, s, (const uint8_t*)P->master, P->stride, P->N,
                         P->planar, (const Dec*)P->dec[0], (uint8_t*)P->fdir);
      rc = (int)hipGetLastError();
      if (rc) return -rc;
      fdir = P->fdir;
    }
    rc = h2o_hist_build(sb, P->stride, sw, sy, P->nodes[d + 1], P->bp[d + 1], P->meta[d + 1], P->F, P->partials,
                        P->slot, P->qs, gh, P->packed, P->dec[d], P->nl[d], P->pf32, P->N, P->planar | (P->no_na << 1),
                        P->nbins_f, P->fine_f, tp_planes(tp_fcut(P, d + 1)), fdir, s);
  } else {
    const bool fused = route_fused_ranges() && P->tiles_cap[d - 1] > 0;
    rc = tp_route(P, d - 1, s, fused);
    if (rc) return -rc;
    if (!fused) {
      rc = h2o_ranges(P->nodes[d + 1], P->cur[d], P->tp[d + 1], P->bp[d + 1], P->meta[d + 1], s);
      if (rc) return -rc;
    }
    gh = P->tiles_cap[d + 1] < P->grid ? P->tiles_cap[d + 1] : P->grid;
    tp_level_buf(P, d + 1, sb, sy, sw);
    rc = h2o_hist_build(sb, P->stride, sw, sy, P->nodes[d + 1], P->bp[d + 1], P->meta[d + 1], P->F, P->partials,
                        P->slot, P->qs, gh, P->packed, nullptr, nullptr, P->pf32, P->N, P->planar | (P->no_na << 1),
                        P->nbins_f, P->fine_f, tp_planes(tp_fcut(P, d + 1)), nullptr, s);
  }
  if (rc) return -rc;
  const int lo = tp_fcut(P, d + 1);
  if (!dist)
    rc = h2o_hist_reduce(P->partials, P->slot, P->used, P->nodes[d + 1], P->bp[d + 1], P->meta[d + 1], P->caps[d + 1],
                         gh, nullptr, hn, hc, P->pf32, 0, 0, lo, s);
  else if (P->sliced)
    rc = h2o_hist_reduce(P->partials, P->slot, P->used, P->nodes[d + 1], P->bp[d + 1], P->meta[d + 1], P->caps[d + 1],
                         gh, P->hbuild, nullptr, nullptr, P->pf32, 0, 0, lo, s);
  else
    rc = h2o_hist_reduce(P->partials, P->slot, P->used, P->nodes[d + 1], P->bp[d + 1], P->meta[d + 1], P->caps[d + 1],
                         gh, P->hrecv, nullptr, nullptr, P->pf32, P->cf32, P->sslot, lo, s);
  return rc ? -rc : 0;
}

int h2o_tree_level(const TreePlan* P, int d, int dist, hipStream_t s) {
  const bool fuse = !dist && !P->dist && !P->sliced && P->caps[d] <= PLAN_REDUCE_MAX && plan_fused() && !P->gcat;
  const int rc = fuse ? tree_find_plan(P, d, s) : h2o_tree_find(P, d, s);
  if (rc) return -rc;
  return tree_grow(P, d, dist, s, fuse);
}


static int tree_leaves(const TreePlan* P, bool values, hipStream_t s) {
  int n_nodes = 0;
  for (int d = 0; d < P->D; ++d) n_nodes += P->caps[d];
  const LeafVals lv{P->log_link, P->scale, P->kclamp, P->mx, P->leaf_lam, P->leaf_l1,
                    values ? (float*)P->leafval : nullptr};
  static int fused = -1;
  if (fused < 0) { const char* e = getenv("H2O_LEAF_FUSED"); fused = (e && e[0] == '1') ? 1 : 0; }
  return leaf_assign_launch(P->master, P->stride, P->N, P->lvptrs, P->D, tp_aux(P, P->num_plane), tp_aux(P, 3), P->qs,
                            P->leaf_of_row, P->leafq, P->leaf_cap, P->leafsum, n_nodes, P->planar, lv, s, tp_lvl2(P),
                            fused ? (int*)P->counters + 3 : nullptr, P->gcat != nullptr);
}

int h2o_tree_leaves(const TreePlan* P, hipStream_t s) { return tree_leaves(P, false, s); }

static inline int coll(const TreePlan* P, int op, const void* snd, void* rcv, long long count, int dt, hipStream_t s) {
  return ((h2o_coll_fn)P->coll_fn)(P->coll_ctx, op, snd, rcv, count, dt, s);
}

static int exchange(const TreePlan* P, int n, hipStream_t s) {
  const int dt = P->cf32 ? H2O_DT_F32 : H2O_DT_F64;
  if (P->sliced) {
    TP_CHECK(h2o_hist_pack(P->hbuild, P->slot, P->F, P->cand_fs, P->W, n, P->hsend, P->cf32, s));
    return coll(P, H2O_COLL_REDUCE_SCATTER, P->hsend, P->hrecv, (long long)n * P->sslot, dt, s);
  }
  return coll(P, H2O_COLL_ALLREDUCE, P->hrecv, P->hrecv, (long long)n * P->sslot, dt, s);
}

int h2o_tree_dist(const TreePlan* P, hipStream_t s) {
  if (!P->coll_fn || P->W < 1) return (int)hipErrorInvalidValue;
  if (!P->dist) return (int)hipErrorInvalidValue;
  TP_CHECK(h2o_tree_root(P, s));
  const long long L2 = 2LL * P->leaf_cap;
  TP_CHECK(exchange(P, 1, s));
  for (int d = 0; d < P->D; ++d) {
    TP_CHECK(h2o_tree_find(P, d, s));
    if (P->sliced)
      TP_CHECK(coll(P, H2O_COLL_ALLGATHER, P->cand_local, P->cand_all,
                    (long long)P->caps[d] * P->cand_fs * (long long)sizeof(Cand), H2O_DT_U8, s));
    const int r = h2o_tree_grow(P, d, 1, s);
    if (r < 0) return -r;
    if (r == 1) break;
    TP_CHECK(exchange(P, P->caps[d], s));
  }
  TP_CHECK(h2o_tree_leaves(P, s));
  if (P->sliced) {
    double* lsx = (double*)P->lsx;
    TP_CHECK((int)hipMemcpyAsync(lsx, P->leafsum, (size_t)L2 * 8, hipMemcpyDeviceToDevice, s));
    if (P->fs0 == 0 && P->fsn > 0)
      TP_CHECK((int)hipMemcpyAsync(lsx + L2, P->rootw, 8, hipMemcpyDeviceToDevice, s));
    else
      TP_CHECK((int)hipMemsetAsync(lsx + L2, 0, 8, s));
    TP_CHECK(coll(P, H2O_COLL_ALLREDUCE, lsx, lsx, L2 + 1, H2O_DT_F64, s));
    TP_CHECK((int)hipMemcpyAsync(P->leafsum, lsx, (size_t)L2 * 8, hipMemcpyDeviceToDevice, s));
    TP_CHECK((int)hipMemcpyAsync(P->rootw, lsx + L2, 8, hipMemcpyDeviceToDevice, s));
  } else {
    TP_CHECK(coll(P, H2O_COLL_ALLREDUCE, P->leafsum, P->leafsum, L2, H2O_DT_F64, s));
  }
  if (P->leaf_native)
    TP_CHECK(h2o_leaf_values(P->leafsum, P->leaf_cap, P->log_link, P->scale, P->kclamp, P->mx, P->leaf_lam,
                             P->leaf_l1, P->leafval, s));
  return 0;
}

int h2o_tree_all(const TreePlan* P, hipStream_t s) {
  TP_CHECK(h2o_tree_root(P, s));
  for (int d = 0; d < P->D; ++d) {
    const int r = h2o_tree_level(P, d, 0, s);
    if (r < 0) return -r;
    if (r == 1) break;
  }
  return tree_leaves(P, P->leaf_native != 0, s);
}
#undef TP_CHECK

}
```

llama_github_io_amd/ops/tree.py:

```python
from __future__ import annotations

import ctypes
import math
import os
from dataclasses import dataclass, field

import numpy as np
import torch

from . import _native as nat
from ..parallel import collectives as coll

NBIN = 256
NA_BIN = 255
MAX_DATA_BINS = 255
FTILE = 32
AMAX_SHARDS = 64

NODE_DT = np.dtype([("start", "<i4"), ("len", "<i4"), ("build", "<i4"), ("parent", "<i4"), ("sib", "<i4"),
                    ("dir", "<i4"), ("p1", "<i4"), ("p2", "<i4")])
NBW = 32
DEC_DT = np.dtype([("feat", "<i4"), ("bin", "<i4"), ("na_left", "<i4"), ("is_cat", "<i4"), ("bits", "<u4", (NBW,)),
                   ("gain", "<f8"), ("wl", "<f8"), ("wr", "<f8"), ("predl", "<f4"), ("predr", "<f4")])
CAND_BYTES = 184
# ... 306 lines not shown
        for e, c in cands:
            if best_code < 0 or e > best_e or (e == best_e and c < best_code):
                best_e, best_code = e, c
        b, nal = (best_code >> 1, best_code & 1) if best_code > 0 else (0, 0)
        bits = np.zeros(NBW, dtype=np.uint32)
        if cat and best_code > 0:
            for t in range(nb):
                cidx = idx[t]
                empty = (sw[t] - (sw[t - 1] if t > 0 else 0.0)) == 0.0
                left = (nal != 0) if empty else (t < b)
                if left:
                    bits[cidx >> 5] |= np.uint32(1 << (cidx & 31))
        wl = wr = yl = yr = 0.0
        if best_code == 0:
            wl, yl, wr, yr = W, WY, wNA, wyNA
        elif best_code > 0:
            wl, yl = sw[b - 1], swy[b - 1]
            wr, yr = W - wl, WY - yl
            if nal:
                wl += wNA; yl += wyNA
            else:
                wr += wNA; yr += wyNA
        Epar = float(_E(p.mode, p, Wall, WYall))
        gain = best_e - Epar
        valid = False
        if best_code >= 0 and Wall >= 2.0 * p.min_w:
            if p.mode == MODE_SE:
                var = wyy * Wall - WYall * WYall
                seBefore = (wyy - Epar) if wNA >= p.min_w else ((wyy - nayy[f]) - float(_E(p.mode, p, W, WY)))
                seAfter = wyy - best_e
                pl, pr = np.float32(yl / wl) if wl else np.float32(np.nan), np.float32(yr / wr) if wr else np.float32(np.nan)
                valid = (np.float32(var) != 0) and (seAfter < seBefore * (1.0 - p.min_split_improvement)) and \
                    (pl != pr) and wl >= p.min_w and wr >= p.min_w
                if random_mode:
                    valid = wl > 0 and wr > 0
            elif p.mode == MODE_NEWTON:
                valid = (0.5 * gain - p.gamma) > 1e-6 and wl >= p.min_w and wr >= p.min_w
                gain = 0.5 * gain - p.gamma
            else:
                valid = wl > 0 and wr > 0
        if cat and best_code == 0:
            bits[:] = 0xFFFFFFFF
        cbin = NA_BIN if best_code == 0 else b
        if grp > 0:
            cbin = group_pack(nbins_f, f, grp)
        out.append(dict(expl=best_e, gain=gain, wl=wl, wr=wr, bin=cbin,
                        na_left=0 if best_code == 0 else nal, valid=bool(valid), is_cat=GROUP_CAT if grp else int(cat),
                        bits=bits, predl=_leafv(p.mode, p, wl, yl), predr=_leafv(p.mode, p, wr, yr)))
    return out


def split_reduce_ref(cands, feat_ok, k_cols, seed, level, node, node_ok=None, fgroup=None):
    F = len(cands)
    gid = list(range(F)) if fgroup is None else [int(g) for g in fgroup]
    lead = [gid[f] not in gid[:f] for f in range(F)] if fgroup is not None else [True] * F
    base = splitmix64((seed ^ ((level + 1) << 40) ^ node) & _M64)
    ok = [bool(feat_ok[f]) and (node_ok is None or bool(node_ok[f])) for f in range(F)]
    n_ok = sum(1 for f in range(F) if ok[f] and lead[f])
    sample = 0 < k_cols < n_ok
    allowed = ok[:]
    if sample:
        keys = [splitmix64((base + gid[f]) & _M64) for f in range(F)]
        for f in range(F):
            if not ok[f]:
                continue
            rank = sum(1 for g in range(F) if ok[g] and lead[g] and
                       (keys[g] < keys[f] or (keys[g] == keys[f] and gid[g] < gid[f])))
            allowed[f] = rank < k_cols
    be, bf = -1.0e300, -1
    for f in range(F):
        c = cands[f]
        if allowed[f] and c["valid"] and (bf < 0 or c["expl"] > be):
            be, bf = c["expl"], f
    d = np.zeros(1, dtype=DEC_DT)[0]
    d["feat"] = bf
    if bf >= 0:
        c = cands[bf]
        d["bin"], d["na_left"], d["is_cat"], d["bits"] = c["bin"], c["na_left"], c["is_cat"], c["bits"]
        d["gain"], d["wl"], d["wr"], d["predl"], d["predr"] = c["gain"], c["wl"], c["wr"], c["predl"], c["predr"]
    return d


def _level_k(k_cols, d: int) -> int:
    if isinstance(k_cols, (list, tuple)):
        return int(k_cols[min(d, len(k_cols) - 1)]) if k_cols else 0
    return int(k_cols)


def group_level_np(pack: int, b4: np.ndarray) -> np.ndarray:
    b4 = np.asarray(b4, dtype=np.int64)
    lvl = np.full(b4.shape[0], -1, dtype=np.int64)
    na = b4[:, 0] == NA_BIN
    for k in range(4):
        ek = ((int(pack) & 0xFFFFFFFF) >> (8 * k)) & 255
        if ek == 0:
            continue
        hit = (lvl < 0) & ~na & (b4[:, k] != ek)
        lvl[hit] = 254 * k + b4[hit, k]
    return lvl


def dec_go_left_np(d, b: np.ndarray) -> np.ndarray:
    if d["feat"] < 0:
        return np.ones(b.shape[0], dtype=bool)
    if int(d["is_cat"]) == GROUP_CAT:
        lvl = group_level_np(int(d["bin"]), b)
        bits = d["bits"]
        lc = np.maximum(lvl, 0)
        gl = ((bits[lc >> 5] >> (lc & 31).astype(np.uint32)) & 1).astype(bool)
        return np.where(lvl < 0, bool(d["na_left"]), gl)
    na = b == NA_BIN
    if d["is_cat"]:
        bits = d["bits"]
        gl = ((bits[b >> 5] >> (b & 31).astype(np.uint32)) & 1).astype(bool)
    else:
        gl = b < d["bin"]
    return np.where(na, bool(d["na_left"]), gl)


class RefTreeBuilder:

    def __init__(self, bins: torch.Tensor, F: int, nbins_f, iscat_f, mono_f, max_depth: int, params: SplitParams,
                 node_cap: int = 1 << 15):
        self.bins = bins.cpu().numpy() if isinstance(bins, torch.Tensor) else np.asarray(bins)
        self.F = F
        self.nbins_f = np.asarray(nbins_f)
        self.iscat_f = np.asarray(iscat_f)
        self.mono_f = None if mono_f is None else np.asarray(mono_f)
        self.D = max_depth
        self.p = params
        self.node_cap = node_cap
        self.N = self.bins.shape[0]
        self.ic_map = None
        self.n_low = self.n_mid = 0
        self.gcat = None

    def set_interaction_constraints(self, ic_map, root_ok):
        self.ic_map = np.asarray(ic_map, dtype=np.uint8)
        self.ic_root = np.asarray(root_ok, dtype=np.uint8)

    def set_feature_groups(self, fgroup, n_low: int = 0, n_mid: int = 0):
        self.fgroup = None if fgroup is None else np.asarray(fgroup, dtype=np.int64)
        self.n_low, self.n_mid = int(n_low), int(n_mid)

    def set_cat_groups(self, gcat):
        self.gcat = None if gcat is None else np.asarray(gcat, dtype=np.int32)

    def _split_bytes(self, d, rows):
        f = int(d["feat"])
        if int(d["is_cat"]) == GROUP_CAT:
            return self.bins[rows, f:f + 4].astype(np.int64)
        return self.bins[rows, f].astype(np.int64)

    def _hist(self, rows, aux):
        F = self.F
        h = np.zeros((F, 256, 2))
        a = aux[rows, 0].astype(np.float64); b = aux[rows, 1].astype(np.float64)
        a32 = aux[rows, 0]; b32 = aux[rows, 1]
        yy = np.where(a32 > 0, (b32 * b32 / np.where(a32 > 0, a32, 1)).astype(np.float32), 0).astype(np.float64)
        nayy = np.zeros(F)
        for f0 in range(0, F, 16):
            f1 = min(F, f0 + 16)
            bf = self.bins[rows, f0:f1].astype(np.int64)
            key = (bf + 256 * np.arange(f1 - f0)[None, :]).T.reshape(-1)
            n = 256 * (f1 - f0)
            h[f0:f1, :, 0] = np.bincount(key, weights=np.tile(a, f1 - f0), minlength=n).reshape(f1 - f0, 256)
            h[f0:f1, :, 1] = np.bincount(key, weights=np.tile(b, f1 - f0), minlength=n).reshape(f1 - f0, 256)
            for j in range(f1 - f0):
                nayy[f0 + j] = yy[bf[:, j] == NA_BIN].sum()
        return h, nayy, yy.sum()

    def _ranges_on(self) -> bool:
        p = self.p
        return (bool(p.parent_range) and bool(p.adapt_nbins) and p.edges is not None and p.vrange is not None
                and p.hist_type != HT_QUANTILES)

    def _occupied(self, h):
        F = self.F
        occ = np.full((F, 2), -1, dtype=np.int64)
        for f in range(F):
            nb = min(int(self.nbins_f[f]), NA_BIN)
            nz = np.nonzero(h[f, :nb, 0] > 0)[0]
            if nz.size:
                occ[f] = (nz[0], nz[-1])
        return occ

    def _value_ranges(self, occ, split=None, side=0):
        p, F = self.p, self.F
        vr = np.full((F, 2), np.nan)
        for f in range(F):
            if occ[f, 0] < 0 or self.iscat_f[f]:
                continue
            nb = int(self.nbins_f[f])
            vr[f] = (_bin_lo(p, f, int(occ[f, 0])), _bin_hi(p, f, int(occ[f, 1]), nb))
        if split is not None:
            sf, b = split
            v = float(np.float32(p.edges[sf][b - 1]))
            grp = getattr(self, "fgroup", None)
            for f in range(F):
                same = f == sf if grp is None else grp[f] == grp[sf]
                if same and not np.isnan(vr[f, 0]):
                    if side == 0:
                        vr[f, 1] = min(vr[f, 1], v)
                    else:
                        vr[f, 0] = max(vr[f, 0], v)
        return vr

    def build(self, aux_static: torch.Tensor, feat_ok=None, k_cols: int = 0, seed: int = 0, leaf_fn=None):
        aux = aux_static.detach().cpu().numpy().astype(np.float32)
        ranges = self._ranges_on()
        F, D, p = self.F, self.D, self.p
        feat_ok = np.ones(F, dtype=np.int32) if feat_ok is None else np.asarray(feat_ok)
        leaf_of_row = np.full(self.N, -1, dtype=np.int64)
        cut = narrow_cut(p, self.n_low, self.n_mid, F)
        leafsum = []
        level_rows = [np.arange(self.N)]
        level_ok = [None if self.ic_map is None else self.ic_root]
        level_vr = [None]
        decs, cls, crs = [], [], []
        n_leaves = 0
        for d in range(D):
            cap_next = min(1 << (d + 1), self.node_cap) if d + 1 < D else 1
            n = len(level_rows)
            dl = np.zeros(n, dtype=DEC_DT)
            level_occ = []
            for i, rows in enumerate(level_rows):
                h, nayy, wyy = self._hist(rows, aux)
                if coll.is_dist():
                    flat = torch.from_numpy(np.concatenate([h.ravel(), nayy, [wyy]]))
                    coll.all_reduce_(flat)
                    flat = flat.numpy()
                    h = flat[: h.size].reshape(h.shape)
                    nayy = flat[h.size: h.size + F]
                    wyy = float(flat[-1])
                vr = None
                if ranges:
                    level_occ.append(self._occupied(h))
                    vr = level_vr[i] if level_vr[i] is not None else self._value_ranges(level_occ[i])
                cands = split_find_ref(h, nayy, wyy, self.nbins_f, self.iscat_f, self.mono_f, p, d, i, seed, vr,
                                       self.gcat)
                fc = level_fcut(cut, self.n_low, self.n_mid, d)
                if fc:
                    for f in range(fc, F):
                        cands[f]["valid"] = False
                dl[i] = split_reduce_ref(cands, feat_ok, _level_k(k_cols, d), seed, d, i, level_ok[i],
                                         getattr(self, "fgroup", None))
            cl = np.zeros(n, dtype=np.int64); cr = np.zeros(n, dtype=np.int64)
            nxt, nxt_ok, nxt_vr = [], [], []
            act = 0
            for i, rows in enumerate(level_rows):
                dd = dl[i]
                if dd["feat"] < 0:
                    lid = n_leaves; n_leaves += 1
                    cl[i] = cr[i] = -1 - lid
                    leaf_of_row[rows] = lid
                    leafsum.append((aux[rows, 2].astype(np.float64).sum(), aux[rows, 3].astype(np.float64).sum()))
                    continue
                gl = dec_go_left_np(dd, self._split_bytes(dd, rows))
                lrows, rrows = rows[gl], rows[~gl]
                for side, crow, wside, arr in ((0, lrows, dd["wl"], cl), (1, rrows, dd["wr"], cr)):
                    active = d + 1 < D and wside >= 2.0 * p.min_w and act < cap_next
                    if d + 1 < D and wside >= 2.0 * p.min_w:
                        act += 1
                    if active:
                        arr[i] = len(nxt); nxt.append(crow)
                        nxt_ok.append(None if self.ic_map is None else level_ok[i] & self.ic_map[dd["feat"]])
                        if ranges:
                            num = not dd["is_cat"] and int(dd["bin"]) != NA_BIN
                            nxt_vr.append(self._value_ranges(level_occ[i], (int(dd["feat"]), int(dd["bin"]))
                                                             if num else None, side))
                    else:
                        lid = n_leaves; n_leaves += 1
                        arr[i] = -1 - lid
                        leaf_of_row[crow] = lid
                        leafsum.append((aux[crow, 2].astype(np.float64).sum(), aux[crow, 3].astype(np.float64).sum()))
            decs.append(dl); cls.append(cl); crs.append(cr)
            level_rows = nxt
            level_ok = nxt_ok
            level_vr = nxt_vr if ranges else [None] * len(nxt)
            if not nxt:
                break
        res = TreeLevels(decs, cls, crs, n_leaves)
        res.root_weight = float(aux[:, 0].astype(np.float64).sum())
        self.leafsum = torch.tensor(np.array(leafsum, dtype=np.float64).reshape(-1, 2))
        if coll.is_dist():
            coll.all_reduce_(self.leafsum)
            res.root_weight = coll.all_reduce_scalar(res.root_weight)
        self.leaf_of_row = torch.from_numpy(leaf_of_row.astype(np.int32))
        if leaf_fn is not None:
            res.leaf_values = leaf_fn(self.leafsum).to(torch.float32).cpu().numpy()
        if not hasattr(self, "history"):
            self.history = []
        self.history.append(res)
        return len(self.history) - 1

    def pop_levels(self, ready_only: bool = False) -> list:
        out = list(getattr(self, "history", []))
        self.history = []
        return out


_MAXL = 65
_SNAP_KERNEL = os.environ.get("H2O_SNAP_KERNEL", "1") != "0"
_vp, _ci, _cd = ctypes.c_void_p, ctypes.c_int, ctypes.c_double


class _TreePlan(ctypes.Structure):
    _fields_ = ([("N", ctypes.c_longlong)] +
                [(n, _ci) for n in ("stride", "F", "D", "slot", "used", "pf32", "grid", "leaf_cap", "mode",
                                    "random_split", "unit")] +
                [(n, _cd) for n in ("min_w", "msi", "lam", "alpha", "gamma")] +
                [(n, _vp) for n in ("master", "partials", "hist0", "hist1", "hbuild", "cand", "scratch", "nbins_f",
                                    "iscat_f", "mono_f", "qs", "leafsum", "leaf_of_row", "counters", "rootw",
                                    "leafval", "leafq", "lvptrs")] +
                [(n, _vp * 2) for n in ("bb", "by", "bw")] +
                [(n, _vp * _MAXL) for n in ("nodes", "meta", "tp", "bp", "dec", "cl", "cr", "nl", "cur")] +
                [("caps", _ci * _MAXL), ("tiles_cap", _ci * _MAXL)] +
                [(n, _vp) for n in ("aux", "amax_bits", "feat_ok")] +
                [(n, _ci) for n in ("compute_amax", "k_cols", "packed", "leaf_native", "log_link", "hist_type")] +
                [("seed", ctypes.c_ulonglong)] + [(n, _cd) for n in ("scale", "kclamp", "mx")] +
                [("kc_level", _ci * _MAXL), ("pad2", _ci)] +
                [("edges", _vp), ("nb_level", _ci * _MAXL), ("pad3", _ci)] +
                [("ic_map", _vp), ("ic", _vp * _MAXL)] +
                [(n, _ci) for n in ("sliced", "fs0", "fsn", "sslot")] + [("cand_local", _vp), ("hrecv", _vp)] +
                [("leaf_lam", _cd), ("leaf_l1", _cd)] + [("planar", _ci), ("no_na", _ci)] +
                [("fgroup", _vp)] + [("coll_fn", _vp), ("coll_ctx", _vp)] +
                [(n, _ci) for n in ("W", "cf32", "cand_fs", "dist")] + [(n, _vp) for n in ("hsend", "cand_all", "lsx")] +
                [("fine_f", _vp)] + [(n, _ci) for n in ("lo_F", "lo_from", "mid_F", "mid_from")] + [("lvl2", _vp), ("fdir", _vp)] +
                [("num_plane", _ci), ("pad4", _ci)] +
                [(n, _vp) for n in ("fine16", "f16col", "f16n")] + [("f16_planes", _ci), ("pad5", _ci)] +
                [("vrange", _vp), ("range_on", _ci), ("pad6", _ci)] + [("gcat", _vp)])


class _Arena:

    def __init__(self):
        self.off = 0
        self.items = []

    def add(self, name, nbytes):
        self.items.append((name, self.off, nbytes))
        self.off += (nbytes + 255) // 256 * 256
        return name


class GpuTreeBuilder:

    def __init__(self, bins: torch.Tensor, F: int, nbins_f, iscat_f, mono_f, max_depth: int, params: SplitParams,
                 node_cap: int = 1 << 14, grid: int = 256):
        assert bins.is_cuda and bins.dtype == torch.uint8 and bins.dim() in (2, 3)
        if bins.dim() == 2 and bins.shape[1] >= 64 and bins.shape[1] % 32 == 0 and \
                os.environ.get("H2O_BINS_ROWMAJOR") != "1":
            bins = bins.view(bins.shape[0], bins.shape[1] // 32, 32).permute(1, 0, 2).contiguous()
        self.planar = bins.dim() == 3
        if self.planar:
            assert bins.shape[2] == 32 and bins.shape[0] >= 2
        self.lib = nat.hip()
        sz = np.zeros(16, dtype=np.int32)
        self.lib.h2o_tree_sizes(sz.ctypes.data)
        assert sz[0] == NODE_DT.itemsize and sz[1] == DEC_DT.itemsize and sz[2] == CAND_BYTES, sz
        assert sz[7] == AMAX_SHARDS, sz
        self.TILE = int(sz[3])
        dev = bins.device
        self.dev = dev
        if self.planar:
            self.N, self.stride = bins.shape[1], bins.shape[0] * 32
        else:
            self.N, self.stride = bins.shape
        assert self.stride % 4 == 0
        self.F = F
        self.D = D = max(1, int(max_depth))
        if D >= _MAXL - 1:
            raise ValueError(f"max_depth {D} exceeds the native tree plan ({_MAXL - 2})")
        self.p = params
        self.grid = int(os.environ.get("H2O_HIST_GRID", grid))
        grid = self.grid
        self.pf32 = int(os.environ.get("H2O_PARTIAL_F32", "1" if self.N >= 1_000_000 else "0"))
        self.master = bins
        N, T = self.N, self.TILE
        self.caps = [min(1 << d, node_cap) for d in range(D)] + [1]
        capmax = max(self.caps)
        self.used = F * 2 * NBIN + F + 1
        self.slot = self.used + (self.used & 1)
        self.hist = [torch.empty(capmax * self.slot, dtype=torch.float64, device=dev) for _ in range(2)]
        self.hbuild = torch.empty(max(self.caps[:D]) * self.slot, dtype=torch.float64, device=dev)
        self.hist_bpc = int(os.environ.get("H2O_HIST_BPC", "1"))
        self.partials = torch.zeros((self.hist_bpc * grid + capmax) * self.slot, dtype=torch.float64, device=dev)
        self.tiles_cap = [(N + T - 1) // T + c for c in self.caps]
        self.cand = torch.empty(capmax * F * CAND_BYTES, dtype=torch.uint8, device=dev)
        self.scratch = torch.empty(2 * capmax + 16, dtype=torch.int32, device=dev)
        self.leaf_cap = min(N + 1, 2 * sum(self.caps) + 2)
        self.leafsum = torch.zeros(self.leaf_cap, 2, dtype=torch.float64, device=dev)
        self.leafq = torch.zeros(int(sz[8]) * self.leaf_cap * 2, dtype=torch.int64, device=dev)
        self.leaf_of_row = torch.empty(N, dtype=torch.int32, device=dev)
        self.nbins_f = torch.as_tensor(np.asarray(nbins_f, dtype=np.int32), device=dev)
        self.iscat_f = torch.as_tensor(np.asarray(iscat_f, dtype=np.int32), device=dev)
        self.iscat_np = np.asarray(iscat_f, dtype=np.int32)
        self.fine_f = None
        self.n_low = self.n_mid = 0
        self.mono_f = None if mono_f is None else torch.as_tensor(np.asarray(mono_f, dtype=np.int32), device=dev)
        self.feat_ok_all = torch.ones(F, dtype=torch.int32, device=dev)
        self.qs = torch.zeros(16, dtype=torch.float64, device=dev)
        self.amax_bits = torch.zeros(4 * AMAX_SHARDS, dtype=torch.int32, device=dev)
        self._soa = None
        self.bufs = [dict(bins=torch.empty(N * self.stride, dtype=torch.uint8, device=dev),
                          y=torch.empty(N, dtype=torch.float32, device=dev), w=None) for _ in range(2)]
        ar = _Arena()
        for d in range(D + 1):
            c = self.caps[d]
            ar.add(f"nodes{d}", c * NODE_DT.itemsize)
            ar.add(f"meta{d}", 16)
            ar.add(f"tp{d}", (c + 1) * 4)
            ar.add(f"bp{d}", (c + 1) * 4)
            ar.add(f"dec{d}", c * DEC_DT.itemsize)
            ar.add(f"cl{d}", c * 4)
            ar.add(f"cr{d}", c * 4)
            ar.add(f"nl{d}", c * 4)
            ar.add(f"cur{d}", c * 16)
        ar.add("counters", 16)
        ar.add("rootw", 8)
        ar.add("leafval", self.leaf_cap * 4)
        self.arena = torch.zeros(ar.off, dtype=torch.uint8, device=dev)
        self.av = {}
        self._off = {}
        for name, off, nb in ar.items:
            self.av[name] = self.arena[off:off + nb]
            self._off[name] = (off, nb)
        n_tiles0 = (N + T - 1) // T
        root = np.zeros(1, dtype=NODE_DT)
        root[0] = (0, N, 1, -1, -1, 0, 0, 0)
        self.av["nodes0"].copy_(torch.from_numpy(root.view(np.uint8)))
        self.av["meta0"].copy_(torch.from_numpy(np.array([1, n_tiles0, n_tiles0, 0], dtype=np.int32).view(np.uint8)))
        self.av["tp0"][:8].copy_(torch.from_numpy(np.array([0, n_tiles0], dtype=np.int32).view(np.uint8)))
        self.av["bp0"][:8].copy_(torch.from_numpy(np.array([0, n_tiles0], dtype=np.int32).view(np.uint8)))
        self.history = []
        npre = int(os.environ.get("H2O_TREE_SNAP_POOL", "8")) if dev.type == "cuda" else 0
        self._pinned_pool = [torch.empty(self.arena.numel(), dtype=torch.uint8, pin_memory=True) for _ in range(npre)]
        self._event_pool = [torch.cuda.Event() for _ in range(npre)]
        self._decoded = []
        self._snap_wait = npre > 0 and os.environ.get("H2O_TREE_SNAP_WAIT", "1") == "1"
        self._pt = {name: t.data_ptr() for name, t in self.av.items()}
        self.lvptrs = torch.tensor([[self._pt[f"dec{d}"], self._pt[f"cl{d}"], self._pt[f"cr{d}"], self.caps[d]]
                                    for d in range(D)],
                                   dtype=torch.int64).reshape(-1).to(dev)
        self.ic_map = None
        self._hp = [h.data_ptr() for h in self.hist]
        self._init_comm(capmax)

    def _init_comm(self, capmax: int):
        force = os.environ.get("H2O_TREE_COMM_FORCE", "")
        self.dist_mode = coll.is_dist() or force in ("rs", "ar")
        self.W = coll.world() if coll.is_dist() else 1
        mode = force if force in ("rs", "ar") else os.environ.get("H2O_TREE_COMM", "ar")
        self.sliced = self.dist_mode and mode == "rs"
        self.cf32 = int(self.dist_mode and os.environ.get("H2O_TREE_COMM_DTYPE", "f64") == "f32")
        self.fs = self.fs0 = self.fsn = 0
        self.sslot = self.slot
        self.transport = None
        if not self.dist_mode:
            return
        W, F, dev = self.W, self.F, self.dev
        wire = torch.float32 if self.cf32 else torch.float64
        self.hsend = self.cand_local = self.cand_all = self.lsx = None
        if self.sliced:
            self.fs = Fs = (F + W - 1) // W
            self.fs0 = min(F, coll.rank() * Fs)
            self.fsn = max(0, min(F, self.fs0 + Fs) - self.fs0)
            self.sslot = Fs * 2 * NBIN + Fs + 1
            self.hsend = torch.empty(W * capmax * self.sslot, dtype=wire, device=dev)
            self.cand_local = torch.zeros(capmax * Fs * CAND_BYTES, dtype=torch.uint8, device=dev)
            self.cand_all = torch.zeros(W * capmax * Fs * CAND_BYTES, dtype=torch.uint8, device=dev)
            self.lsx = torch.zeros(self.leaf_cap * 2 + 1, dtype=torch.float64, device=dev)
        else:
            self.sslot = self.used
        self.hrecv = torch.empty(capmax * self.sslot, dtype=wire, device=dev)
        from ..parallel import rccl
        comm = rccl.native_comm(force=bool(force))
        if comm is not None:
            self.transport = comm
        else:
            bufs = [self.hist[0], self.hbuild, self.leafsum, self.hsend, self.hrecv, self.cand_local,
                    self.cand_all, self.lsx]
            self.transport = rccl.HostTransport(bufs)

    def comm_per_tree(self) -> tuple:
        D, W = self.D, self.W
        if not self.dist_mode:
            return 0, 0
        es = 4 if self.cf32 else 8
        slots = [1] + self.caps[:D - 1]
        if self.sliced:
            rs = sum(W * n * self.sslot * es for n in slots)
            ag = sum(self.caps[d] * self.fs * CAND_BYTES for d in range(D))
            return len(slots) + D + 1, rs + ag + (self.leaf_cap * 2 + 1) * 8
        return len(slots) + 1, sum(n * self.sslot * es for n in slots) + self.leaf_cap * 2 * 8

    def _p(self, name):
        return self._pt[name]

    def set_interaction_constraints(self, ic_map, root_ok):
        F, dev = self.F, self.dev
        self.ic_map = torch.as_tensor(np.asarray(ic_map, dtype=np.uint8), device=dev).contiguous()
        self.ic_lv = [torch.zeros(self.caps[d] * F, dtype=torch.uint8, device=dev) for d in range(self.D + 1)]
        self.ic_lv[0][:F].copy_(torch.as_tensor(np.asarray(root_ok, dtype=np.uint8), device=dev))
        if getattr(self, "_plan", None) is not None:
            self._set_plan_ic(self._plan)

    def set_feature_groups(self, fgroup, n_low: int = 0, n_mid: int = 0):
        enc = encode_groups(fgroup)
        self.fgroup = None if enc is None else torch.as_tensor(enc, device=self.dev).contiguous()
        self._fgroup_np = None if fgroup is None else np.asarray(fgroup, dtype=np.int64)
        self._fine16 = None
        self.fine_f = fine_columns(fgroup, self.iscat_np, self.F)
        if self.fine_f is not None:
            self.fine_f = torch.as_tensor(self.fine_f, device=self.dev).contiguous()
        self.n_low, self.n_mid = int(n_low), int(n_mid)
        if getattr(self, "_plan", None) is not None:
            self._plan.fgroup = 0 if self.fgroup is None else self.fgroup.data_ptr()
            self._plan.fine_f = 0 if self.fine_f is None else self.fine_f.data_ptr()
            self._set_plan_narrow(self._plan)
            self._set_plan_fine16(self._plan)

    def set_cat_groups(self, gcat):
        if gcat is not None and self.sliced:
            raise ValueError("wide-categorical groups need the all-reduce histogram exchange (H2O_TREE_COMM=ar): a "
                             "feature slice could cut a group")
        self.gcat_np = None if gcat is None else np.asarray(gcat, dtype=np.int32)
        self.gcat = None if gcat is None else torch.as_tensor(self.gcat_np, device=self.dev).contiguous()
        if getattr(self, "_plan", None) is not None:
            self._plan.gcat = 0 if self.gcat is None else self.gcat.data_ptr()

    def _set_plan_narrow(self, P):
        mid, lo = narrow_cut(self.p, self.n_low, self.n_mid, self.F)
        P.lo_F, P.lo_from = (self.n_low, lo) if lo >= 0 else (0, 0)
        P.mid_F, P.mid_from = (self.n_mid, mid) if mid >= 0 else (0, 0)
        wide = self.planar and self.F > 32 and os.environ.get("H2O_ROW_DIR_PLANAR", "0") == "1"
        if (lo >= 0 and self.planar) or wide:
            if getattr(self, "_fdir", None) is None:
                self._fdir = torch.empty(self.N, dtype=torch.uint8, device=self.dev)
            if lo >= 0 and getattr(self, "_lvl2", None) is None:
                self._lvl2 = torch.empty(self.N, dtype=torch.uint8, device=self.dev)
        on = lo >= 0 and self.planar
        P.lvl2 = self._lvl2.data_ptr() if on else 0
        P.fdir = self._fdir.data_ptr() if (on or wide) else 0

    def _fine16_map(self):
        if os.environ.get("H2O_HIST_ROOT16", "1") == "0" or not self.planar or self.dev.type != "cuda":
            return None
        fg = getattr(self, "_fgroup_np", None)
        if fg is None or not (self.n_low or self.n_mid) or self.p.edges is None:
            return None
        F = self.F
        edges = np.asarray(self.p.edges, dtype=np.float32)
        order, cols = [], {}
        for c in range(F):
            g = int(fg[c])
            if g not in cols:
                cols[g] = []
                order.append(g)
            cols[g].append(c)
        nslot = len(order)
        if nslot > 64:
            return None
        ns = (nslot + 15) // 16 * 16
        cslot = np.full(self.master.shape[0] * 32, -1, dtype=np.int32)
        fcol = np.full((ns, 4), -1, dtype=np.int32)
        fn = np.zeros(ns, dtype=np.int32)
        for s_, g in enumerate(order):
            cs = cols[g]
            if len(cs) > 4 or (len(cs) > 1 and any(int(self.iscat_np[c]) for c in cs)):
                return None
            cs = sorted(cs, key=lambda c: float(edges[c, 0]))
            fcol[s_, :len(cs)] = cs
            fn[s_] = len(cs)
            cslot[cs] = s_
        return cslot, fcol, fn, nslot

    def _set_plan_fine16(self, P):
        P.fine16 = P.f16col = P.f16n = 0
        P.f16_planes = 0
        m = self._fine16_map()
        if m is None:
            return
        cslot, fcol, fn, nslot = m
        dev = self.dev
        if getattr(self, "_fine16", None) is None:
            planes16 = (nslot + 15) // 16
            self._f16_cslot = torch.as_tensor(cslot, device=dev)
            self._f16col = torch.as_tensor(fcol.reshape(-1), device=dev)
            self._f16n = torch.as_tensor(fn, device=dev)
            self._fine16 = torch.empty(planes16 * self.N * 16, dtype=torch.int16, device=dev)
            nat.call("h2o_fine16_build", self.master.data_ptr(), int(self.master.shape[0]), self.N,
                     self._f16_cslot.data_ptr(), nslot, self._fine16.data_ptr(), nat.stream_ptr(dev))
            self._f16_planes = planes16
        P.fine16, P.f16col, P.f16n = self._fine16.data_ptr(), self._f16col.data_ptr(), self._f16n.data_ptr()
        P.f16_planes = self._f16_planes

    def _set_plan_ic(self, P):
        if self.ic_map is None:
            P.ic_map = 0
            return
        P.ic_map = self.ic_map.data_ptr()
        for d in range(self.D + 1):
            P.ic[d] = self.ic_lv[d].data_ptr()

    def _make_plan(self):
        assert self.lib.h2o_tree_plan_size() == ctypes.sizeof(_TreePlan), "TreePlan layout mismatch"
        P = _TreePlan()
        p = self.p
        P.N, P.stride, P.F, P.D, P.slot, P.used, P.pf32 = self.N, self.stride, self.F, self.D, self.slot, self.used, self.pf32
        P.leaf_cap, P.mode, P.random_split = self.leaf_cap, int(p.mode), int(p.random_split)
        P.min_w, P.msi, P.lam, P.alpha, P.gamma = p.min_w, p.min_split_improvement, p.lam, p.alpha, p.gamma
        P.master, P.partials = self.master.data_ptr(), self.partials.data_ptr()
        P.hist0, P.hist1, P.hbuild = self._hp[0], self._hp[1], self.hbuild.data_ptr()
        P.cand, P.scratch = self.cand.data_ptr(), self.scratch.data_ptr()
        P.nbins_f, P.iscat_f = self.nbins_f.data_ptr(), self.iscat_f.data_ptr()
        P.mono_f = 0 if self.mono_f is None else self.mono_f.data_ptr()
        P.qs, P.leafsum, P.leaf_of_row = self.qs.data_ptr(), self.leafsum.data_ptr(), self.leaf_of_row.data_ptr()
        P.leafq, P.lvptrs = self.leafq.data_ptr(), self.lvptrs.data_ptr()
        P.counters, P.rootw, P.leafval = self._p("counters"), self._p("rootw"), self._p("leafval")
        for i in range(2):
            P.bb[i], P.by[i] = self.bufs[i]["bins"].data_ptr(), self.bufs[i]["y"].data_ptr()
            P.bw[i] = 0
        for d in range(self.D + 1):
            for n in ("nodes", "meta", "tp", "bp", "dec", "cl", "cr", "nl", "cur"):
                getattr(P, n)[d] = self._p(f"{n}{d}")
            P.caps[d], P.tiles_cap[d] = self.caps[d], self.tiles_cap[d]
        P.edges = self._edges_ptr()
        for d in range(_MAXL):
            P.nb_level[d] = p.adapt_nb(d) if P.edges else 0
        P.hist_type = int(p.hist_type)
        if P.edges and p.vrange is not None and p.parent_range and p.hist_type != HT_QUANTILES:
            self._vrange_dev = torch.as_tensor(np.asarray(p.vrange, dtype=np.float32).reshape(-1),
                                               device=self.dev).contiguous()
            P.vrange, P.range_on = self._vrange_dev.data_ptr(), 1
        else:
            P.vrange, P.range_on = 0, 0
        self._set_plan_ic(P)
        fg = getattr(self, "fgroup", None)
        P.fgroup = 0 if fg is None else fg.data_ptr()
        gc = getattr(self, "gcat", None)
        P.gcat = 0 if gc is None else gc.data_ptr()
        P.fine_f = 0 if self.fine_f is None else self.fine_f.data_ptr()
        self._set_plan_narrow(P)
        self._set_plan_fine16(P)
        P.sliced, P.fs0, P.fsn, P.sslot = int(self.sliced), self.fs0, self.fsn, self.sslot
        P.planar = int(self.planar)
        P.no_na = int(self._no_na())
        P.cand_local = self.cand_local.data_ptr() if self.sliced else 0
        P.hrecv = self.hrecv.data_ptr() if self.dist_mode else 0
        P.W, P.cf32, P.cand_fs, P.dist = self.W, self.cf32, self.fs, int(self.dist_mode)
        if self.sliced:
            P.hsend, P.cand_all, P.lsx = self.hsend.data_ptr(), self.cand_all.data_ptr(), self.lsx.data_ptr()
        if self.transport is not None:
            P.coll_fn, P.coll_ctx = self.transport.fn, self.transport.ctx
        return P

    def _no_na(self) -> bool:
        b, F = self.master, self.F
        if b.numel() == 0:
            return True
        hit = torch.zeros((), dtype=torch.bool, device=b.device)
        step = 1 << 24
        if self.planar:
            for pl in range(b.shape[0]):
                nf = min(32, F - 32 * pl)
                if nf <= 0:
                    break
                for r0 in range(0, b.shape[1], step):
                    hit |= (b[pl, r0:r0 + step, :nf] == NA_BIN).any()
        else:
            for r0 in range(0, b.shape[0], step):
                hit |= (b[r0:r0 + step, :F] == NA_BIN).any()
        return not bool(hit)

    def _edges_ptr(self):
        if self.p.edges is None or not self.p.adapt_nbins:
            return 0
        if getattr(self, "_edges_dev", None) is None:
            self._edges_dev = torch.as_tensor(np.asarray(self.p.edges, dtype=np.float32), device=self.master.device).contiguous()
        return self._edges_dev.data_ptr()

    def _planes(self, aux: torch.Tensor, soa: bool) -> torch.Tensor:
        if soa:
            assert aux.shape == (4, self.N) and aux.dtype == torch.float32 and aux.is_contiguous()
            return aux
        assert aux.shape == (self.N, 4) and aux.dtype == torch.float32
        if self._soa is None:
            self._soa = torch.empty(4, self.N, dtype=torch.float32, device=self.dev)
        self._soa.copy_(aux.t())
        return self._soa

    def build(self, aux_static: torch.Tensor, feat_ok: torch.Tensor | None = None, k_cols: int = 0, seed: int = 0,
              leaf_fn=None, amax_bits: torch.Tensor | None = None, packed: bool | int = False, leaf_native=None,
              soa: bool = False, unit: bool = False, num_plane: int = 2):
        if not hasattr(self, "_plan"):
            self._plan = self._make_plan()
        planes = self._planes(aux_static, soa)
        lib, P = self.lib, self._plan
        s = nat.stream_ptr(self.dev)
        P.aux = planes.data_ptr()
        P.unit = int(bool(unit))
        P.num_plane = int(num_plane) if soa else 2
        if not unit:
            for i in range(2):
                if self.bufs[i]["w"] is None:
                    self.bufs[i]["w"] = torch.empty(self.N, dtype=torch.float32, device=self.dev)
                P.bw[i] = self.bufs[i]["w"].data_ptr()
        P.compute_amax = int(amax_bits is None)
        P.amax_bits = (self.amax_bits if amax_bits is None else amax_bits).data_ptr()
        P.feat_ok = (self.feat_ok_all if feat_ok is None else feat_ok).data_ptr()
        P.k_cols, P.packed, P.seed = _level_k(k_cols, 0), (2 if packed == 2 else int(bool(packed))), int(seed) & _M64
        for d in range(_MAXL):
            P.kc_level[d] = _level_k(k_cols, d) if isinstance(k_cols, (list, tuple)) else 0
        P.grid = self.grid * (self.hist_bpc if packed else 1)
        P.leaf_native = int(leaf_native is not None)
        if leaf_native is not None:
            lg, scale, kclamp, mx = leaf_native[:4]
            lam, l1 = (tuple(leaf_native[4:6]) + (0.0, 0.0))[:2]
            P.log_link, P.scale, P.kclamp, P.mx = int(lg), float(scale), float(kclamp), float(mx)
            P.leaf_lam, P.leaf_l1 = float(lam), float(l1)
        ref = ctypes.byref(P)
        if not self.dist_mode:
            if self._graph_replay(P, k_cols):
                pass
            else:
                nat.check(lib.h2o_tree_all(ref, s), "tree_all")
        else:
            rc = lib.h2o_tree_dist(ref, s)
            err = getattr(self.transport, "error", None)
            if err is not None:
                self.transport.error = None
                raise RuntimeError(f"tree collective failed: {err}") from err
            nat.check(rc, "tree_dist")
            if isinstance(self.transport, _native_comm_cls()):
                coll.add_stats(*self.comm_per_tree())
        if leaf_native is None and leaf_fn is not None:
            vals = leaf_fn(self.leafsum)
            self.av["leafval"].view(torch.float32)[: vals.numel()].copy_(vals.to(torch.float32))
        return self._snapshot()

    def _seed_used(self, P, k_cols) -> bool:
        ht = int(self.p.hist_type)
        return (bool(P.k_cols) or any(int(v) for v in P.kc_level) or bool(P.random_split)
                or (bool(P.edges) and ht in (HT_RANDOM, HT_ROUND_ROBIN)))

    def _graph_replay(self, P, k_cols) -> bool:
        if self.dev.type != "cuda" or os.environ.get("H2O_TREE_GRAPH", "1") == "0" or self.__dict__.get("_graph_off"):
            return False
        seed = P.seed
        if not self._seed_used(P, k_cols):
            P.seed = 0
        sig = bytes(P)
        P.seed = seed
        cache = self.__dict__.setdefault("_graphs", {})
        g = cache.get(sig)
        if g is None:
            misses = self.__dict__.get("_graph_misses", 0) + 1
            self._graph_misses = misses
            if misses > _GRAPH_CACHE:
                self._graph_off = True
                cache.clear()
                return False
            g = torch.cuda.CUDAGraph()
            try:
                with torch.cuda.graph(g, capture_error_mode="thread_local"):
                    rc = self.lib.h2o_tree_all(ctypes.byref(P), nat.stream_ptr(self.dev))
            except Exception:
                self._graph_off = True
                cache.clear()
                return False
            nat.check(rc, "tree_all (capture)")
            if len(cache) >= _GRAPH_CACHE:
                cache.pop(next(iter(cache)))
            cache[sig] = g
        else:
            self._graph_misses = 0
        g.replay()
        return True

    def _snapshot(self):
        if not self._pinned_pool and self.history and self._snap_wait:
            self._decoded.extend(self._pop(1))
        host = self._pinned_pool.pop() if self._pinned_pool else torch.empty(self.arena.numel(), dtype=torch.uint8,
                                                                               pin_memory=True)
        dptr = self._snap_dev_ptr(host) if self.dev.type == "cuda" and _SNAP_KERNEL else 0
        if dptr:
            nat.call("h2o_snap_copy", self.arena.data_ptr(), dptr, self.arena.numel(), nat.stream_ptr(self.dev))
        else:
            host.copy_(self.arena, non_blocking=True)
        ev = self._event_pool.pop() if self._event_pool else torch.cuda.Event()
        ev.record()
        self.history.append((host, ev))
        return len(self.history) - 1

    def _snap_dev_ptr(self, host: torch.Tensor) -> int:
        cache = self.__dict__.setdefault("_dev_ptrs", {})
        hp = host.data_ptr()
        if hp not in cache:
            out = ctypes.c_ulonglong(0)
            rc = nat.hip().h2o_host_dev_ptr(ctypes.c_void_p(hp), ctypes.byref(out))
            cache[hp] = int(out.value) if rc == 0 and host.is_pinned() and out.value % 16 == 0 else 0
        return cache[hp]

    def leaf_values_view(self) -> torch.Tensor:
        return self.av["leafval"].view(torch.float32)

    def pop_levels(self, ready_only: bool = False) -> list:
        out, self._decoded = self._decoded, []
        return out + self._pop(None, ready_only)

    def _pop(self, limit, ready_only: bool = False) -> list:
        out = []
        while self.history and (limit is None or len(out) < limit):
            host, ev = self.history[0]
            if ready_only and not ev.query():
                break
            ev.synchronize()
            self.history.pop(0)
            hn = host.numpy()
            o = self._off["rootw"][0]
            out.append(self._decode(hn, float(hn[o:o + 8].view(np.float64)[0])))
            self._pinned_pool.append(host)
            self._event_pool.append(ev)
        return out

    def _decode(self, host: np.ndarray, root_weight: float) -> TreeLevels:
        off = self._off

        def arr(name, dt):
            o, nb = off[name]
            return host[o:o + nb].view(dt)
        decs, cls, crs = [], [], []
        for d in range(self.D):
            n = int(arr(f"meta{d}", np.int32)[0])
            if d == 0:
                n = 1
            if n <= 0:
                break
            decs.append(arr(f"dec{d}", DEC_DT)[:n].copy())
            cls.append(arr(f"cl{d}", np.int32)[:n].astype(np.int64))
            crs.append(arr(f"cr{d}", np.int32)[:n].astype(np.int64))
        n_leaves = int(arr("counters", np.int32)[0])
        vals = arr("leafval", np.float32)[:n_leaves].copy()
        return TreeLevels(decs, cls, crs, n_leaves, vals, root_weight)


def _native_comm_cls():
    from ..parallel.rccl import NativeComm
    return NativeComm


def make_builder(bins: torch.Tensor, F, nbins_f, iscat_f, mono_f, max_depth, params, node_cap=1 << 14):
    if bins.is_cuda:
        return GpuTreeBuilder(bins, F, nbins_f, iscat_f, mono_f, max_depth, params, node_cap=node_cap)
    return RefTreeBuilder(bins, F, nbins_f, iscat_f, mono_f, max_depth, params, node_cap=node_cap)


def best_first_prune(tl: TreeLevels, max_leaves: int, by_depth: bool = False):
    import heapq
    decs, cl, cr = tl.decs, tl.child_l, tl.child_r
    can = lambda d, i: d < len(decs) and int(decs[d]["feat"][i]) >= 0
    expanded = set()
    key = (lambda d, i: float(d)) if by_depth else (lambda d, i: -float(decs[d]["gain"][i]))
    heap = [(key(0, 0), 0, 0, 0)] if decs and can(0, 0) else []
    leaves, seq = 1, 1
    while heap and (max_leaves <= 0 or leaves < max_leaves):
        _, _, d, i = heapq.heappop(heap)
        expanded.add((d, i))
        leaves += 1
        for c in (int(cl[d][i]), int(cr[d][i])):
            if c >= 0 and can(d + 1, c):
                heapq.heappush(heap, (key(d + 1, c), seq, d + 1, c))
                seq += 1
    leaf_map = np.zeros(max(int(tl.n_leaves), 1), dtype=np.int64)

    def sub_leaves(d, i):
        out, stack = [], [(d, i)]
        while stack:
            a, b = stack.pop()
            for c in {int(cl[a][b]), int(cr[a][b])}:
                if c < 0:
                    out.append(-1 - c)
                else:
                    stack.append((a + 1, c))
        return out

    ndecs, ncl, ncr = [], [], []
    n_new = 0
    level = [0] if decs else []
    d = 0
    while level:
        dd = decs[d][level].copy()
        lcl = np.zeros(len(level), dtype=np.int64)
        lcr = np.zeros(len(level), dtype=np.int64)
        nxt = []
        for j, i in enumerate(level):
            if (d, i) in expanded:
                for c, arr in ((int(cl[d][i]), lcl), (int(cr[d][i]), lcr)):
                    if c >= 0:
                        arr[j] = len(nxt)
                        nxt.append(c)
                    else:
                        leaf_map[-1 - c] = n_new
                        arr[j] = -1 - n_new
                        n_new += 1
            else:
                for lf in sub_leaves(d, i):
                    leaf_map[lf] = n_new
                dd["feat"][j] = -1
                dd["gain"][j] = 0.0
                lcl[j] = lcr[j] = -1 - n_new
                n_new += 1
        ndecs.append(dd)
        ncl.append(lcl)
        ncr.append(lcr)
        level = nxt
        d += 1
    return TreeLevels(ndecs, ncl, ncr, max(n_new, 1), None, tl.root_weight), leaf_map


class BestFirstBuilder:

    def __init__(self, inner, max_leaves: int, by_depth: bool = False):
        self.inner, self.max_leaves, self.by_depth = inner, int(max_leaves), bool(by_depth)
        self.done = []
        self.leaf_of_row = None
        self.leafsum = None

    def __getattr__(self, name):
        return getattr(self.inner, name)

    def build(self, aux_static, feat_ok=None, k_cols=0, seed=0, leaf_fn=None, **kw):
        kw.pop("leaf_native", None)
        self.inner.build(aux_static, feat_ok, k_cols, seed=seed, leaf_fn=None, **kw)
        tl = self.inner.pop_levels()[-1]
        pruned, lmap = best_first_prune(tl, self.max_leaves, self.by_depth)
        dev = self.inner.leaf_of_row.device
        m = torch.from_numpy(lmap).to(dev)
        self.leaf_of_row = m[self.inner.leaf_of_row.long()].to(torch.int32)
        ls = self.inner.leafsum[: tl.n_leaves].to(dev)
        self.leafsum = torch.zeros(pruned.n_leaves, ls.shape[1], dtype=ls.dtype, device=dev).index_add_(0, m[: ls.shape[0]], ls)
        if leaf_fn is not None:
            pruned.leaf_values = leaf_fn(self.leafsum).to(torch.float32).cpu().numpy()
        self.done.append(pruned)
        return len(self.done) - 1

    def pop_levels(self, ready_only: bool = False) -> list:
        out, self.done = self.done, []
        return out
```

Baseline: 217.3 million rows/s.

## Pack routed target and weight into spare row words of partitioned bin buffers

When the row-major bin rows have spare 32-bit words past the feature bytes, the routing kernel now writes the target (and the weight, when not unit-weighted) into the last words of each destination row. It no longer scatters them into separate y/w arrays. Histogram kernels at deeper levels then read y/w from the same row they already fetch bins from, through the same buffer resource. This removes separate scattered stores and gathers and the separate y/w ping-pong buffers. The cost is extra template variants, a bit more addressing arithmetic, and a dependence on stride padding being available, which is enabled by default.

Result: slower. 213.9 million rows/s (-1.6%).

```diff
diff --git a/llama_github_io_amd/csrc/tree_kernels.hip b/llama_github_io_amd/csrc/tree_kernels.hip
--- a/llama_github_io_amd/csrc/tree_kernels.hip
+++ b/llama_github_io_amd/csrc/tree_kernels.hip
@@ -323,16 +323,21 @@
   const float* ay;
   __amdgpu_buffer_rsrc_t rb, ra, rw;
   int lgw;
+  int ys, ylg;
+  unsigned yo4, wo4;
 };
 
 __device__ __forceinline__ HistSrc make_src(const unsigned* bins32, const float* aw, const float* ay, long long N, int W,
-                                            int lgw) {
-  return HistSrc{bins32, aw, ay,
-                 __builtin_amdgcn_make_buffer_rsrc((void*)bins32, 0, (int)(unsigned)((unsigned long long)N * W * 4),
-                                                   0x00020000),
+                                            int lgw, int yrow) {
+  const __amdgpu_buffer_rsrc_t rb = __builtin_amdgcn_make_buffer_rsrc(
+      (void*)bins32, 0, (int)(unsigned)((unsigned long long)N * W * 4), 0x00020000);
+  if (yrow)
+    return HistSrc{bins32, yrow == 2 ? (const float*)bins32 : nullptr, (const float*)bins32, rb, rb, rb, lgw, W, lgw,
+                   (unsigned)(W - 1) * 4u, yrow == 2 ? (unsigned)(W - 2) * 4u : (unsigned)(W - 1) * 4u};
+  return HistSrc{bins32, aw, ay, rb,
                  __builtin_amdgcn_make_buffer_rsrc((void*)ay, 0, (int)(unsigned)(N * 4), 0x00020000),
                  __builtin_amdgcn_make_buffer_rsrc((void*)(aw ? aw : ay), 0, (int)(unsigned)(N * 4), 0x00020000),
-                 lgw};
+                 lgw, 1, 2, 0u, 0u};
 }
 
 template <bool FILT, bool PACKED, bool UNIT, bool NONA, bool BUF, bool FINE, int GR = RPI, int UNR = H2O_UNR>
@@ -370,12 +375,15 @@
     const bool whole = base + GR * UNR <= r1;
     if (BUF && !FILT && whole) {
       const unsigned row0 = (unsigned)(base + g);
-      const unsigned vb = (row0 << src.lgw) + (unsigned)wc * 4u, va = row0 * 4u;
+      const unsigned vb = (row0 << src.lgw) + (unsigned)wc * 4u;
+      const unsigned va = (row0 << src.ylg) + src.yo4, vw = (row0 << src.ylg) + src.wo4;
 #pragma unroll
       for (int u = 0; u < UNR; ++u) {
         wd[u] = __builtin_amdgcn_raw_buffer_load_b32(src.rb, vb, (unsigned)(u * GR) << src.lgw, 0);
-        const float y = __uint_as_float(__builtin_amdgcn_raw_buffer_load_b32(src.ra, va, u * GR * 4, 0));
-        const float w = weighted ? __uint_as_float(__builtin_amdgcn_raw_buffer_load_b32(src.rw, va, u * GR * 4, 0))
+        const float y =
+            __uint_as_float(__builtin_amdgcn_raw_buffer_load_b32(src.ra, va, (unsigned)(u * GR) << src.ylg, 0));
+        const float w = weighted ? __uint_as_float(__builtin_amdgcn_raw_buffer_load_b32(
+                                       src.rw, vw, (unsigned)(u * GR) << src.ylg, 0))
                                  : 1.f;
         ab[u] = make_float2(w, y);
       }
@@ -387,11 +395,15 @@
         if (BUF) {
           const unsigned ro = (unsigned)row;
           wd[u] = __builtin_amdgcn_raw_buffer_load_b32(src.rb, (ro << src.lgw) + (unsigned)wc * 4u, 0, 0);
-          const float y = __uint_as_float(__builtin_amdgcn_raw_buffer_load_b32(src.ra, ro * 4u, 0, 0));
-          const float w = weighted ? __uint_as_float(__builtin_amdgcn_raw_buffer_load_b32(src.rw, ro * 4u, 0, 0)) : 1.f;
+          const float y =
+              __uint_as_float(__builtin_amdgcn_raw_buffer_load_b32(src.ra, (ro << src.ylg) + src.yo4, 0, 0));
+          const float w = weighted ? __uint_as_float(__builtin_amdgcn_raw_buffer_load_b32(
+                                         src.rw, (ro << src.ylg) + src.wo4, 0, 0))
+                                   : 1.f;
           ab[u] = make_float2(w, y);
         } else {
-          ab[u] = make_float2(weighted ? src.aw[row] : 1.f, src.ay[row]);
+          const size_t ra = (size_t)row * src.ys;
+          ab[u] = make_float2(weighted ? src.aw[ra + (src.wo4 >> 2)] : 1.f, src.ay[ra + (src.yo4 >> 2)]);
           wd[u] = src.bins32[(size_t)row * W + wc];
         }
       }
@@ -468,12 +480,15 @@
   auto load = [&](int base, unsigned (&wd)[UNR], float2 (&ab)[UNR]) {
     if (BUF && base + GR * UNR <= r1) {
       const unsigned row0 = (unsigned)(base + g);
-      const unsigned vb = (row0 << src.lgw) + (unsigned)wc * 4u, va = row0 * 4u;
+      const unsigned vb = (row0 << src.lgw) + (unsigned)wc * 4u;
+      const unsigned va = (row0 << src.ylg) + src.yo4, vw = (row0 << src.ylg) + src.wo4;
 #pragma unroll
       for (int u = 0; u < UNR; ++u) {
         wd[u] = __builtin_amdgcn_raw_buffer_load_b32(src.rb, vb, (unsigned)(u * GR) << src.lgw, 0);
-        const float y = __uint_as_float(__builtin_amdgcn_raw_buffer_load_b32(src.ra, va, u * GR * 4, 0));
-        const float w = weighted ? __uint_as_float(__builtin_amdgcn_raw_buffer_load_b32(src.rw, va, u * GR * 4, 0))
+        const float y =
+            __uint_as_float(__builtin_amdgcn_raw_buffer_load_b32(src.ra, va, (unsigned)(u * GR) << src.ylg, 0));
+        const float w = weighted ? __uint_as_float(__builtin_amdgcn_raw_buffer_load_b32(
+                                       src.rw, vw, (unsigned)(u * GR) << src.ylg, 0))
                                  : 1.f;
         ab[u] = make_float2(w, y);
       }
@@ -484,11 +499,15 @@
         if (BUF) {
           const unsigned ro = (unsigned)row;
           wd[u] = __builtin_amdgcn_raw_buffer_load_b32(src.rb, (ro << src.lgw) + (unsigned)wc * 4u, 0, 0);
-          const float y = __uint_as_float(__builtin_amdgcn_raw_buffer_load_b32(src.ra, ro * 4u, 0, 0));
-          const float w = weighted ? __uint_as_float(__builtin_amdgcn_raw_buffer_load_b32(src.rw, ro * 4u, 0, 0)) : 1.f;
+          const float y =
+              __uint_as_float(__builtin_amdgcn_raw_buffer_load_b32(src.ra, (ro << src.ylg) + src.yo4, 0, 0));
+          const float w = weighted ? __uint_as_float(__builtin_amdgcn_raw_buffer_load_b32(
+                                         src.rw, (ro << src.ylg) + src.wo4, 0, 0))
+                                   : 1.f;
           ab[u] = make_float2(w, y);
         } else {
-          ab[u] = make_float2(weighted ? src.aw[row] : 1.f, src.ay[row]);
+          const size_t ra = (size_t)row * src.ys;
+          ab[u] = make_float2(weighted ? src.aw[ra + (src.wo4 >> 2)] : 1.f, src.ay[ra + (src.yo4 >> 2)]);
           wd[u] = src.bins32[(size_t)row * W + wc];
         }
       }
@@ -597,11 +616,15 @@
     if (BUF) {
       const unsigned ro = (unsigned)row;
       wd[u] = __builtin_amdgcn_raw_buffer_load_b32(src.rb, (ro << src.lgw) + (unsigned)L.wc * 4u, 0, 0);
-      yv[u] = __uint_as_float(__builtin_amdgcn_raw_buffer_load_b32(src.ra, ro * 4u, 0, 0));
-      if (!UNIT) wv[u] = L.weighted ? __uint_as_float(__builtin_amdgcn_raw_buffer_load_b32(src.rw, ro * 4u, 0, 0)) : 1.f;
+      yv[u] = __uint_as_float(__builtin_amdgcn_raw_buffer_load_b32(src.ra, (ro << src.ylg) + src.yo4, 0, 0));
+      if (!UNIT)
+        wv[u] = L.weighted
+                    ? __uint_as_float(__builtin_amdgcn_raw_buffer_load_b32(src.rw, (ro << src.ylg) + src.wo4, 0, 0))
+                    : 1.f;
     } else {
-      yv[u] = src.ay[row];
-      if (!UNIT) wv[u] = L.weighted ? src.aw[row] : 1.f;
+      const size_t ra = (size_t)row * src.ys;
+      yv[u] = src.ay[ra + (src.yo4 >> 2)];
+      if (!UNIT) wv[u] = L.weighted ? src.aw[ra + (src.wo4 >> 2)] : 1.f;
       wd[u] = src.bins32[(size_t)row * W + L.wc];
     }
   }
@@ -674,6 +697,7 @@
   const int t0 = blockIdx.x * per, t1 = min(n_tiles, t0 + per);
   if (t0 >= t1) return;
   const int ftile = blockIdx.y;
+  const int yrow = (planar >> 2) & 3;
   planar &= 1;
   const int W = planar ? LPR : stride >> 2;
   const int g = threadIdx.x / LPR, j = threadIdx.x % LPR;
@@ -681,7 +705,7 @@
   const int Fl = planar ? F - ftile * FTILE : F;
   const unsigned* bins32 = (const unsigned*)(planar ? bins + (size_t)ftile * (size_t)N * 32 : bins);
   const float sa = (float)qs[PACKED ? 10 : 0], sb = (float)qs[PACKED ? 12 : 1], sp = (float)qs[4];
-  const HistSrc src = make_src(bins32, aw, ay, N, W, lgw);
+  const HistSrc src = make_src(bins32, aw, ay, N, W, lgw, yrow);
   __shared__ int srep[FTILE], snb[FTILE], sfine[FTILE];
   if (threadIdx.x < FTILE) {
     const int fg = ftile * FTILE + threadIdx.x;
@@ -2007,10 +2031,10 @@
                   : bins[bin_off(row, f, stride, N, planar)];
 }
 
-template <int NV, bool GRP>
+template <int NV, bool GRP, int YR>
 __device__ __forceinline__ void route_tile(
     const uint8_t* __restrict__ sbins, const float* __restrict__ say, const float* __restrict__ saw,
-    uint8_t* __restrict__ dbins, float* __restrict__ day, float* __restrict__ daw, int stride,
+    uint8_t* __restrict__ dbins, float* __restrict__ day, float* __restrict__ daw, int stride, bool yw,
     const Node* __restrict__ nodesA, const int* __restrict__ tpA, const int* __restrict__ metaA,
     const Dec* __restrict__ decA, const int* __restrict__ clA, const int* __restrict__ crA,
     const Dec* __restrict__ decB, const int* __restrict__ clB, const int* __restrict__ crB,
@@ -2063,8 +2087,15 @@
       rv2[u] = NV > 2 ? s4b[0] : make_uint4(0u, 0u, 0u, 0u);
       rv3[u] = NV > 3 ? s4b[1] : make_uint4(0u, 0u, 0u, 0u);
     }
-    ry[u] = say[row];
-    rw[u] = saw ? saw[row] : 1.f;
+    if (YR != 2) {
+      ry[u] = say[row];
+      rw[u] = saw ? saw[row] : 1.f;
+    }
+    if (YR == 1 && NV > 0) {
+      uint4& lv = NV == 1 ? rv0[u] : NV == 2 ? rv1[u] : NV == 3 ? rv2[u] : rv3[u];
+      lv.w = __float_as_uint(ry[u]);
+      if (yw) lv.z = __float_as_uint(rw[u]);
+    }
   }
 #pragma unroll
   for (int u = 0; u < LU; ++u) {
@@ -2152,8 +2183,13 @@
         for (int k = 0; k < W; ++k) dst[k] = src[k];
       }
     }
-    day[pos] = ry[u];
-    if (daw) daw[pos] = rw[u];
+    if (YR == 0) {
+      day[pos] = ry[u];
+      if (daw) daw[pos] = rw[u];
+    } else if (YR == 1 && NV == 0) {
+      dst[W - 1] = __float_as_uint(ry[u]);
+      if (yw) dst[W - 2] = __float_as_uint(rw[u]);
+    }
   }
 }
 
@@ -2164,10 +2200,10 @@
   int* meta;
   int* done;
 };
-template <int NV, bool GRP>
+template <int NV, bool GRP, int YR>
 __global__ __launch_bounds__(LW * 64) void k_route(
     const uint8_t* __restrict__ sbins, const float* __restrict__ say, const float* __restrict__ saw,
-    uint8_t* __restrict__ dbins, float* __restrict__ day, float* __restrict__ daw, int stride,
+    uint8_t* __restrict__ dbins, float* __restrict__ day, float* __restrict__ daw, int stride, int yw,
     const Node* __restrict__ nodesA, const int* __restrict__ tpA, const int* __restrict__ metaA,
     const Dec* __restrict__ decA, const int* __restrict__ clA, const int* __restrict__ crA,
     const Dec* __restrict__ decB, const int* __restrict__ clB, const int* __restrict__ crB,
@@ -2176,8 +2212,8 @@
     RangesOut ro) {
   const int t = blockIdx.x;
   if (t < metaA[1])
-    route_tile<NV, GRP>(sbins, say, saw, dbins, day, daw, stride, nodesA, tpA, metaA, decA, clA, crA, decB, clB, crB,
-                        curs, N, planar, lvl2, fdir, t);
+    route_tile<NV, GRP, YR>(sbins, say, saw, dbins, day, daw, stride, yw != 0, nodesA, tpA, metaA, decA, clA, crA, decB,
+                            clB, crB, curs, N, planar, lvl2, fdir, t);
   if (!ro.done) return;
   __shared__ int s_last;
   __shared__ int sh[17];
@@ -2688,6 +2724,7 @@
                         void* partials, int slot_doubles, const void* qs, const void* pdec, void* nl_out, int f32,
                         long long N, int planar, const void* nbins_f, const void* fine_f, const void* fdir) {
   const bool nona = (planar >> 1) & 1;
+  const int yrow = (planar >> 2) & 3;
   planar &= 1;
   const int rowb = planar ? 32 : stride;
   const unsigned long long bytes = (unsigned long long)N * (unsigned long long)rowb;
@@ -2698,7 +2735,8 @@
                    !(e_buf && strcmp(e_buf, "0") == 0);
 #define H2O_HIST_CASE(F_, N_, B_) \
   launch_hist4<F_, PACKED, UNIT, N_, B_>(grid, lds, s, bins, stride, aw, ay, nodes, tile_prefix, meta, F, partials, \
-                                          slot_doubles, qs, pdec, nl_out, f32, N, planar, lgw, nbins_f, fine_f, fdir)
+                                          slot_doubles, qs, pdec, nl_out, f32, N, planar | (yrow << 2), lgw, nbins_f, \
+                                          fine_f, fdir)
   const bool filt = pdec != nullptr;
   if (filt) {
     if (nona) { if (buf) H2O_HIST_CASE(true, true, true); else H2O_HIST_CASE(true, true, false); }
@@ -2757,7 +2795,7 @@
   if (!fine) fine_f = nullptr;
   const size_t lds = (packed ? HIST_LDS_BYTES - HPLANE * 8 : HIST_LDS_BYTES) + HIST_LDS_TAIL;
   const dim3 gr(grid, nft);
-  if (packed && aw == nullptr)
+  if (packed && aw == nullptr && ((planar >> 2) & 3) != 2)
     launch_hist<true, true>(gr, lds, s, bins, stride, aw, ay, nodes, tile_prefix, meta, F, partials, slot_doubles, qs, pdec, nl_out, f32, N, planar, nbins_f, fine_f, fdir);
   else if (packed) launch_hist<true, false>(gr, lds, s, bins, stride, aw, ay, nodes, tile_prefix, meta, F, partials, slot_doubles, qs, pdec, nl_out, f32, N, planar, nbins_f, fine_f, fdir);
   else launch_hist<false, false>(gr, lds, s, bins, stride, aw, ay, nodes, tile_prefix, meta, F, partials, slot_doubles, qs, pdec, nl_out, f32, N, planar, nbins_f, fine_f, fdir);
@@ -2927,13 +2965,21 @@
                         int stride, const void* nodesA, const void* tpA, const void* metaA, const void* decA,
                         const void* clA, const void* crA, const void* decB, const void* clB, const void* crB,
                         void* curs, int tiles_cap, long long N, int planar, int lp, void* lvl2, const void* fdir,
-                        RangesOut ro, hipStream_t s, int grp = 0) {
+                        RangesOut ro, hipStream_t s, int grp = 0, int yrow = 0) {
   if (planar && (stride % 32 != 0 || stride < 64)) return (int)hipErrorInvalidValue;
   if (lp < 0 || lp > 2 || (lp > 0 && !planar)) return (int)hipErrorInvalidValue;
-#define ROUTE_LAUNCH(NV) do { if (grp) ROUTE_LAUNCH2(NV, true); else ROUTE_LAUNCH2(NV, false); } while (0)
-#define ROUTE_LAUNCH2(NV, G)                                                                                   \
-  hipLaunchKernelGGL((k_route<NV, G>), dim3(tiles_cap), dim3(LW * 64), 0, s, (const uint8_t*)sbins,           \
-                     (const float*)say, (const float*)saw, (uint8_t*)dbins, (float*)day, (float*)daw, stride,  \
+  if (yrow < 0 || yrow > 2) return (int)hipErrorInvalidValue;
+  if (yrow && (planar || day || daw || (say ? (saw != nullptr) != (yrow == 2) : saw != nullptr)))
+    return (int)hipErrorInvalidValue;
+  const int yw = yrow == 2;
+#define ROUTE_LAUNCH(NV) do { if (grp) ROUTE_LAUNCH1(NV, true); else ROUTE_LAUNCH1(NV, false); } while (0)
+#define ROUTE_LAUNCH1(NV, G)                                                                                   \
+  do {                                                                                                         \
+    if (!yrow) ROUTE_LAUNCH2(NV, G, 0); else if (say) ROUTE_LAUNCH2(NV, G, 1); else ROUTE_LAUNCH2(NV, G, 2);   \
+  } while (0)
+#define ROUTE_LAUNCH2(NV, G, Y)                                                                                \
+  hipLaunchKernelGGL((k_route<NV, G, Y>), dim3(tiles_cap), dim3(LW * 64), 0, s, (const uint8_t*)sbins,        \
+                     (const float*)say, (const float*)saw, (uint8_t*)dbins, (float*)day, (float*)daw, stride, yw, \
                      (const Node*)nodesA, (const int*)tpA, (const int*)metaA, (const Dec*)decA, (const int*)clA, \
                      (const int*)crA, (const Dec*)decB, (const int*)clB, (const int*)crB, (int4*)curs, N, planar, \
                      (uint8_t*)lvl2, (const uint8_t*)fdir, ro)
@@ -2945,6 +2991,7 @@
     default: ROUTE_LAUNCH(0);
   }
 #undef ROUTE_LAUNCH
+#undef ROUTE_LAUNCH1
 #undef ROUTE_LAUNCH2
   return (int)hipGetLastError();
 }
@@ -3102,7 +3149,14 @@
   void* vrange;
   int range_on, pad6;
   void* gcat;
+  int yrow, pad7;
 };
+
+static inline int tp_spare_words(const TreePlan* P) { return P->stride / 4 - (P->F + 3) / 4; }
+static inline bool tp_yrow_ok(const TreePlan* P) {
+  if (P->yrow == 0) return true;
+  return !P->planar && P->stride % 4 == 0 && P->yrow == (P->unit ? 1 : 2) && tp_spare_words(P) >= P->yrow;
+}
 
 static inline void tp_node_range(const TreePlan* P, int d, const void* hprev, SplitParams& p) {
   p.range_on = (P->range_on && P->vrange && P->edges && P->nb_level[d] > 1) ? 1 : 0;
@@ -3127,7 +3181,12 @@
 static inline void tp_level_buf(const TreePlan* P, int e, const void*& b, const void*& y, const void*& w) {
   if (e == 0) { b = P->master; y = tp_aux(P, 1); w = P->unit ? nullptr : tp_aux(P, 0); return; }
   const int i = (e / 2 - 1) % 2;
-  b = P->bb[i]; y = P->by[i]; w = P->unit ? nullptr : P->bw[i];
+  b = P->bb[i];
+  if (P->yrow) { y = w = nullptr; return; }
+  y = P->by[i]; w = P->unit ? nullptr : P->bw[i];
+}
+static inline int tp_hist_flags(const TreePlan* P, int e) {
+  return P->planar | (P->no_na << 1) | ((e > 0 ? P->yrow : 0) << 2);
 }
 
 static inline int tp_fcut(const TreePlan* P, int d) {
@@ -3155,10 +3214,12 @@
   const RangesOut ro = ranges ? RangesOut{(Node*)P->nodes[e + 2], (int*)P->tp[e + 2], (int*)P->bp[e + 2],
                                           (int*)P->meta[e + 2], (int*)P->counters + 1}
                               : RangesOut{nullptr, nullptr, nullptr, nullptr, nullptr};
-  return route_launch(sb, sy, sw, P->bb[di], P->by[di], P->unit ? nullptr : P->bw[di], P->stride, P->nodes[e], P->tp[e],
+  if (!tp_yrow_ok(P)) return (int)hipErrorInvalidValue;
+  return route_launch(sb, sy, sw, P->bb[di], P->yrow ? nullptr : P->by[di],
+                      (P->unit || P->yrow) ? nullptr : P->bw[di], P->stride, P->nodes[e], P->tp[e],
                       P->meta[e], P->dec[e], P->cl[e], P->cr[e], P->dec[e + 1], P->cl[e + 1], P->cr[e + 1],
                       P->cur[e + 1], P->tiles_cap[e], P->N, P->planar, lp, e == 0 ? tp_lvl2(P) : nullptr,
-                      (e == 0 && tp_lvl2(P) && P->fdir) ? P->fdir : nullptr, ro, s, P->gcat != nullptr);
+                      (e == 0 && tp_lvl2(P) && P->fdir) ? P->fdir : nullptr, ro, s, P->gcat != nullptr, P->yrow);
 }
 
 #define TP_CHECK(x) do { int rc_ = (x); if (rc_) return rc_; } while (0)
@@ -3288,7 +3349,7 @@
       fdir = P->fdir;
     }
     rc = h2o_hist_build(sb, P->stride, sw, sy, P->nodes[d + 1], P->bp[d + 1], P->meta[d + 1], P->F, P->partials,
-                        P->slot, P->qs, gh, P->packed, P->dec[d], P->nl[d], P->pf32, P->N, P->planar | (P->no_na << 1),
+                        P->slot, P->qs, gh, P->packed, P->dec[d], P->nl[d], P->pf32, P->N, tp_hist_flags(P, d),
                         P->nbins_f, P->fine_f, tp_planes(tp_fcut(P, d + 1)), fdir, s);
   } else {
     const bool fused = route_fused_ranges() && P->tiles_cap[d - 1] > 0;
@@ -3301,7 +3362,7 @@
     gh = P->tiles_cap[d + 1] < P->grid ? P->tiles_cap[d + 1] : P->grid;
     tp_level_buf(P, d + 1, sb, sy, sw);
     rc = h2o_hist_build(sb, P->stride, sw, sy, P->nodes[d + 1], P->bp[d + 1], P->meta[d + 1], P->F, P->partials,
-                        P->slot, P->qs, gh, P->packed, nullptr, nullptr, P->pf32, P->N, P->planar | (P->no_na << 1),
+                        P->slot, P->qs, gh, P->packed, nullptr, nullptr, P->pf32, P->N, tp_hist_flags(P, d + 1),
                         P->nbins_f, P->fine_f, tp_planes(tp_fcut(P, d + 1)), nullptr, s);
   }
   if (rc) return -rc;
diff --git a/llama_github_io_amd/ops/tree.py b/llama_github_io_amd/ops/tree.py
--- a/llama_github_io_amd/ops/tree.py
+++ b/llama_github_io_amd/ops/tree.py
@@ -632,6 +632,7 @@
 
 _MAXL = 65
 _SNAP_KERNEL = os.environ.get("H2O_SNAP_KERNEL", "1") != "0"
+_ROUTE_YROW_DEFAULT = "1"
 _vp, _ci, _cd = ctypes.c_void_p, ctypes.c_int, ctypes.c_double
 
 
@@ -659,7 +660,15 @@
                 [("fine_f", _vp)] + [(n, _ci) for n in ("lo_F", "lo_from", "mid_F", "mid_from")] + [("lvl2", _vp), ("fdir", _vp)] +
                 [("num_plane", _ci), ("pad4", _ci)] +
                 [(n, _vp) for n in ("fine16", "f16col", "f16n")] + [("f16_planes", _ci), ("pad5", _ci)] +
-                [("vrange", _vp), ("range_on", _ci), ("pad6", _ci)] + [("gcat", _vp)])
+                [("vrange", _vp), ("range_on", _ci), ("pad6", _ci)] + [("gcat", _vp)] +
+                [("yrow", _ci), ("pad7", _ci)])
+
+
+def route_yrow(stride: int, F: int, planar: bool, unit: bool) -> int:
+    if os.environ.get("H2O_ROUTE_YROW", _ROUTE_YROW_DEFAULT) == "0" or planar or stride % 4:
+        return 0
+    need = 1 if unit else 2
+    return need if stride // 4 - (F + 3) // 4 >= need else 0
 
 
 class _Arena:
@@ -733,8 +742,8 @@
         self.qs = torch.zeros(16, dtype=torch.float64, device=dev)
         self.amax_bits = torch.zeros(4 * AMAX_SHARDS, dtype=torch.int32, device=dev)
         self._soa = None
-        self.bufs = [dict(bins=torch.empty(N * self.stride, dtype=torch.uint8, device=dev),
-                          y=torch.empty(N, dtype=torch.float32, device=dev), w=None) for _ in range(2)]
+        self.bufs = [dict(bins=torch.empty(N * self.stride, dtype=torch.uint8, device=dev), y=None, w=None)
+                     for _ in range(2)]
         ar = _Arena()
         for d in range(D + 1):
             c = self.caps[d]
@@ -950,8 +959,7 @@
         P.leafq, P.lvptrs = self.leafq.data_ptr(), self.lvptrs.data_ptr()
         P.counters, P.rootw, P.leafval = self._p("counters"), self._p("rootw"), self._p("leafval")
         for i in range(2):
-            P.bb[i], P.by[i] = self.bufs[i]["bins"].data_ptr(), self.bufs[i]["y"].data_ptr()
-            P.bw[i] = 0
+            P.bb[i], P.by[i], P.bw[i] = self.bufs[i]["bins"].data_ptr(), 0, 0
         for d in range(self.D + 1):
             for n in ("nodes", "meta", "tp", "bp", "dec", "cl", "cr", "nl", "cur"):
                 getattr(P, n)[d] = self._p(f"{n}{d}")
@@ -1032,11 +1040,12 @@
         P.aux = planes.data_ptr()
         P.unit = int(bool(unit))
         P.num_plane = int(num_plane) if soa else 2
-        if not unit:
-            for i in range(2):
-                if self.bufs[i]["w"] is None:
-                    self.bufs[i]["w"] = torch.empty(self.N, dtype=torch.float32, device=self.dev)
-                P.bw[i] = self.bufs[i]["w"].data_ptr()
+        P.yrow = route_yrow(self.stride, self.F, self.planar, bool(unit))
+        for i in range(2):
+            for k, ptr, on in (("y", P.by, not P.yrow), ("w", P.bw, not P.yrow and not unit)):
+                if on and self.bufs[i][k] is None:
+                    self.bufs[i][k] = torch.empty(self.N, dtype=torch.float32, device=self.dev)
+                ptr[i] = self.bufs[i][k].data_ptr() if on else 0
         P.compute_amax = int(amax_bits is None)
         P.amax_bits = (self.amax_bits if amax_bits is None else amax_bits).data_ptr()
         P.feat_ok = (self.feat_ok_all if feat_ok is None else feat_ok).data_ptr()
```
